# pedro-morgado/spatialaudiogen

Measured on AMD Instinct MI355X. Metric: ambisonic seconds generated/sec (0.1 s windows, 224x448 video), higher is better.
Workload: dtype f32 (fp32 in / out / accumulate; products on the 16-bit matrix cores with fp32-equivalent operand splits: two fp16 planes (3 products per multiply) for the ResNet trunk's 3x3 convs, whose operand ranges batch-norm bounds, three bf16 planes (6 products) elsewhere - measured against the fp64 oracle as

## Files before the change

### spatialaudiogen_amd/build.py

```python
import os
import subprocess
import sys
from concurrent.futures import ThreadPoolExecutor

HERE = os.path.dirname(os.path.abspath(__file__))
CSRC = os.path.join(HERE, 'csrc')
OBJ = os.path.join(CSRC, 'build')
LIB = os.path.join(HERE, 'libsagen_hip.so')
SOURCES = ['conv3p.hip', 'conv3h.hip', 'conv3g.hip', 'p3.hip', 'igemm3dw.hip', 'igemm3s2.hip', 'stempool.hip', 'stem8.hip', 'igemm.hip', 'fcm.hip', 'igemm3.hip', 'elementwise.hip', 'fft.hip', 'eval.hip', 'evalx.hip', 'render.hip', 'overlay.hip', 'train.hip', 'wgrad.hip', 'wgrad3h.hip', 'backward.hip', 'model.hip', 'train_model.hip', 'api.hip']
HEADERS = sorted(os.path.join(CSRC, h) for h in os.listdir(CSRC) if h.endswith('.h')) + \
          [os.path.join(os.path.dirname(os.path.dirname(CSRC)), 'include', 'sagen.h')]
FLAGS = ['--offload-arch=gfx950', '-O3', '-std=c++17', '-fPIC', '-Wall', '-Wno-unused-function', '-fno-slp-vectorize', '-fno-vectorize']


def _hipcc():
    for cand in (os.environ.get('HIPCC'), '/opt/rocm/bin/hipcc', 'hipcc'):
        if cand and (os.path.isabs(cand) and os.path.exists(cand) or not os.path.isabs(cand)):
            return cand
    raise RuntimeError('hipcc not found')


def flags_digest():
    import hashlib
    h = hashlib.sha256(' '.join(FLAGS).encode())
    h.update(open(os.path.abspath(__file__), 'rb').read())
    return h.hexdigest()[:16]


def source_digest():
    import hashlib
    files = sorted(f for f in os.listdir(CSRC) if f.endswith(('.hip', '.h')))
    h = hashlib.sha256()
    for f in files:
        h.update(f.encode() + b'\0' + open(os.path.join(CSRC, f), 'rb').read() + b'\0')
    h.update(b'sagen.h\0' + open(HEADERS[-1], 'rb').read())
    return h.hexdigest()[:16]


def _stale(target, deps):
    if not os.path.exists(target):
        return True
    t = os.path.getmtime(target)
    return any(os.path.getmtime(d) > t for d in deps)


def build(force=False, verbose=True):
    os.makedirs(OBJ, exist_ok=True)
    hipcc = _hipcc()
    stamp = os.path.join(OBJ, 'flags.stamp')
    if not os.path.exists(stamp) or open(stamp).read().strip() != flags_digest():
        force = True
    jobs = []
    for src in SOURCES:
        s = os.path.join(CSRC, src)
        o = os.path.join(OBJ, src.replace('.hip', '.o'))
        if force or _stale(o, [s] + HEADERS):
            jobs.append((s, o))

    def compile_one(job):
        s, o = job
        cmd = [hipcc] + FLAGS + ['-DSAGEN_BUILD_FLAGS="%s"' % ' '.join(FLAGS), '-c', s, '-o', o]
        if verbose:
# ... 50 lines not shown
```

### spatialaudiogen_amd/csrc/conv3h.hip

```cpp
#include "igemm3_common.h"
#include "h2_planes.h"

namespace sagen {

typedef _Float16 f16x8 __attribute__((ext_vector_type(8)));

constexpr int conv3h_lds(int BM, int BN, int KC, int AR = 2) { return KC * (AR * BM * 64 + 2 * 3 * 2 * BN * 32); }
constexpr int conv3h_wgs_per_cu(int BM, int BN, int KC, int AR = 2) {
    return 160 * 1024 / conv3h_lds(BM, BN, KC, AR) >= 3 ? 3 : (160 * 1024 / conv3h_lds(BM, BN, KC, AR) >= 2 ? 2 : 1);
}

template <int BM, int BN, int WM, int WN, int KC, int AR>
__device__ __forceinline__ void conv3h_body(const IgemmDesc& d) {
    static_assert(AR == 2 || AR == 3, "activation ring of two or three stages");
    constexpr int MT = WM / 32, NT = WN / 32;
    constexpr int WAVES_N = BN / WN, WAVES_M = BM / WM;
    static_assert(WAVES_N * WAVES_M == 4, "4 waves per workgroup");
    constexpr int BME = BM - 2;
    constexpr int A_INST = BM / 16;
    constexpr int B_IPT = BN / 16;
    constexpr int B_INST = 3 * B_IPT;
    constexpr int A_PW = (A_INST + 3) / 4, B_PW = (B_INST + 3) / 4;
    constexpr int A_BYTES = A_INST * 1024, B_BYTES = B_INST * 1024;
    constexpr int ST_BYTES = KC * (A_BYTES + B_BYTES);
    constexpr int NM1 = 3 * MT * NT;
    constexpr int NMG = 3 * KC * NM1;
    constexpr int SPT = A_PW + B_PW;
    constexpr int CNT_MAX = KC * SPT;
    static_assert(CNT_MAX <= NMG, "one DMA slot per MFMA slot at most");
    constexpr int NF = 2 * (MT + NT);
    constexpr int SMEM_BYTES = KC * (AR * A_BYTES + 2 * B_BYTES);
    static_assert(SMEM_BYTES == conv3h_lds(BM, BN, KC, AR), "occupancy bound uses the same footprint");
    static_assert(AR == 2 || A_INST % 4 == 0, "counted vmcnt: every wave issues the same number of activation instructions");
    auto a_stage = [&](int sa) { return AR == 2 ? sa * ST_BYTES : sa * (KC * A_BYTES); };
    auto b_stage = [&](int sb) { return AR == 2 ? sb * ST_BYTES + KC * A_BYTES : AR * KC * A_BYTES + sb * (KC * B_BYTES); };
    __shared__ __attribute__((aligned(16))) char smem[SMEM_BYTES];

    const int tid = threadIdx.x;
#ifdef SAGEN_TRACE
    const size_t trc_wg = ((size_t)blockIdx.z * gridDim.y + blockIdx.y) * gridDim.x + blockIdx.x;
    unsigned long long* const trc = (d.trace && trc_wg < 8192) ? (unsigned long long*)d.trace + trc_wg * 8 : nullptr;
#define C3H_TRC(k) do { if (trc && tid == 0) trc[k] = __builtin_amdgcn_s_memtime(); } while (0)
    if (trc && tid == 0) {
        trc[4] = __builtin_amdgcn_s_getreg((31 << 11) | 4);
        trc[5] = __builtin_amdgcn_s_getreg((31 << 11) | 20);
        trc[6] = __builtin_amdgcn_s_memrealtime();
    }
    C3H_TRC(0);
    const int gsel = (blockIdx.y | blockIdx.z) ? -1 : ((int)blockIdx.x == 8 ? 0 : ((int)blockIdx.x == (int)gridDim.x - 64 ? 1 : -1));
    unsigned long long* const gtr = (d.trace && gsel >= 0) ? (unsigned long long*)d.trace + (size_t)8192 * 8 + (size_t)gsel * 64 * 8 : nullptr;
    int g_idx = 0;
#define C3H_GTRC(k) do { if (gtr && tid == 0 && g_idx < 64) gtr[g_idx * 8 + (k)] = __builtin_amdgcn_s_memtime(); } while (0)
#else
#define C3H_TRC(k) do { } while (0)
#define C3H_GTRC(k) do { } while (0)
#endif
    const int lane = tid & 63;
    const int wave = __builtin_amdgcn_readfirstlane(tid >> 6);
    const int wm = wave / WAVES_N, wn = wave % WAVES_N;
    const int W = d.Win, H = d.Hin, Wp = W + 1, NP = d.p3_np;
    const int nchunk = d.Cin >> 4;
    const bool dhs = d.splitk == 3;
    const int dh_z = dhs ? (int)blockIdx.y : 0;
    const int G = (dhs ? 1 : 3) * nchunk / KC;
    const int nM = (NP + BME - 1) / BME, nN = (d.N + BN - 1) / BN;

    const __amdgpu_buffer_rsrc_t x_rsrc = __builtin_amdgcn_make_buffer_rsrc((void*)d.xp3, 0, d.xp3_bytes, 0x00020000);
    const __amdgpu_buffer_rsrc_t w_rsrc = __builtin_amdgcn_make_buffer_rsrc((void*)d.wh2, 0, d.wh2_bytes, 0x00020000);

    const float osc = d.h2_a_inv[0] * d.h2_w_inv[0];

    const int xcd = (blockIdx.x + blockIdx.z) & 7;
    const int per = (nM + 7) >> 3;
    const int t_run = blockIdx.x >> 3;
    const int my_tiles = max(min((xcd + 1) * per, nM) - xcd * per, 0) * nN;
    if (t_run >= my_tiles) return;
    const int tq = t_run / nN;
    const int m0 = (xcd * per + tq) * BME;
    const int n0 = (t_run - tq * nN) * BN;

    unsigned a_v0[A_PW], a_v1[A_PW], a_v2[A_PW], a_cur[A_PW];
#pragma unroll
    for (int j = 0; j < A_PW; ++j) {
        const int inst = wave + 4 * j;
        const int U = inst * 64 + lane;
        const int slot = U >> 2, v = U & 3;
        const int u = v ^ ((slot >> 2) & 3);
        const int p = m0 - 1 + slot;
        unsigned bad = 7u;
        if (inst < A_INST && p >= 0 && p < NP) {
            const unsigned row = __umulhi((unsigned)p, d.p3_magic_wp);
            const int h = (int)(row - __umulhi(row, d.p3_magic_h) * (unsigned)H);
            bad = (h == 0 ? 1u : 0u) | (h == H - 1 ? 4u : 0u);
        }
        const int base = p * 64 + u * 16;
        a_v0[j] = (bad & 1u) ? OOB : (unsigned)(base - Wp * 64);
        a_v1[j] = (bad & 2u) ? OOB : (unsigned)base;
        a_v2[j] = (bad & 4u) ? OOB : (unsigned)(base + Wp * 64);
    }
    unsigned b_voff[B_PW];
    int b_tapoff[B_PW];
#pragma unroll
    for (int j = 0; j < B_PW; ++j) {
        const int inst = wave + 4 * j;
        b_tapoff[j] = __builtin_amdgcn_readfirstlane((inst / B_IPT) * nchunk * d.N * 64);
        const int r = inst % B_IPT;
        const int L = r * 64 + lane;
        const int pl = L / (2 * BN), n = (L >> 1) % BN, half = L & 1;
        b_voff[j] = (inst < B_INST && n0 + n < d.N) ? (unsigned)((pl * d.N + n0 + n) * 32 + 16 * (half ^ ((n >> 3) & 1))) : OOB;
    }

    int qa_dh = dh_z, qa_ch = 0, cur_dh = -1, qb_dh = dh_z, qb_ch = 0;
    unsigned i_asoff = 0, i_bsoff = 0;
    char* i_astage = smem;
    char* i_bstage = smem;
    auto begin_issue_a = [&](int sa) {
        i_astage = smem + a_stage(sa);
        if (qa_dh != cur_dh) {
            cur_dh = qa_dh;
#pragma unroll
            for (int j = 0; j < A_PW; ++j) a_cur[j] = qa_dh == 0 ? a_v0[j] : (qa_dh == 1 ? a_v1[j] : a_v2[j]);
        }
        i_asoff = (unsigned)qa_ch * d.xp3_cstride;
        qa_ch += KC;
        if (qa_ch == nchunk) { qa_ch = 0; ++qa_dh; }
    };
    auto begin_issue_b = [&](int sb) {
        i_bstage = smem + b_stage(sb);
        i_bsoff = (unsigned)((qb_dh * 3) * nchunk + qb_ch) * (unsigned)(d.N * 64);
        qb_ch += KC;
        if (qb_ch == nchunk) { qb_ch = 0; ++qb_dh; }
    };
    auto issue_a = [&](int kc, int s) {
        const int inst = wave + 4 * s;
        if (A_INST % 4 == 0 || inst < A_INST)
            dma16(x_rsrc, (float*)(i_astage + kc * A_BYTES + inst * 1024), a_cur[s], i_asoff + (unsigned)kc * d.xp3_cstride);
    };
    auto issue_b = [&](int kc, int j) {
        const int inst = wave + 4 * j;
        if (4 * (j + 1) <= B_INST || inst < B_INST)
            dma16(w_rsrc, (float*)(i_bstage + kc * B_BYTES + inst * 1024), b_voff[j], i_bsoff + (unsigned)b_tapoff[j] + (unsigned)(kc * d.N * 64));
    };
    auto issue_nth = [&](int n) {
        if (AR == 2) {
            const int sg = CNT_MAX - 1 - n;
            const int kc = sg / SPT, s = sg - kc * SPT;
            if (s < A_PW) issue_a(kc, s); else issue_b(kc, s - A_PW);
        } else if (n < KC * B_PW) {
            issue_b(n / B_PW, n % B_PW);
        } else {
            const int m = n - KC * B_PW;
            issue_a(m / A_PW, m % A_PW);
        }
    };

    f32x16 acc[MT][NT];
#pragma unroll
    for (int i = 0; i < MT; ++i)
#pragma unroll
        for (int j = 0; j < NT; ++j)
#pragma unroll
            for (int e = 0; e < 16; ++e) acc[i][j][e] = 0.f;

    const int li = lane & 31, kk = lane >> 5;
    int a_foff[3][MT];
#pragma unroll
    for (int i = 0; i < MT; ++i)
#pragma unroll
        for (int dwi = 0; dwi < 3; ++dwi) {
            const int sl = wm * WM + i * 32 + li + dwi;
            a_foff[dwi][i] = sl * 64 + 16 * (kk ^ ((sl >> 2) & 3));
        }
    const int b_foff = (wn * WN + li) * 32 + 16 * (kk ^ ((li >> 3) & 1));
    constexpr int TA[3] = {1, 0, 0}, TB[3] = {0, 1, 0};

    int sa = 0, sb = 0;
    begin_issue_a(0);
    begin_issue_b(0);
#pragma unroll
    for (int n = 0; n < CNT_MAX; ++n) issue_nth(n);
    if (AR == 3) {
        begin_issue_a(1);
#pragma unroll
        for (int n = KC * B_PW; n < CNT_MAX; ++n) issue_nth(n);
    }

    auto group = [&](auto issue_tag) {
        constexpr int ISSUE = decltype(issue_tag)::value;
        constexpr int NISSUE = ISSUE == 2 ? CNT_MAX : (ISSUE == 1 ? KC * B_PW : 0);
        const char* st_a = smem + a_stage(sa);
        const char* st_b = smem + b_stage(sb);
        f16x8 fq[2][NF];
        auto load_frag = [&](int buf, int t, int f) {
            const int kc = t / 3, dwi = t - 3 * kc;
            const int pl = f / (MT + NT), r = f - pl * (MT + NT);
            if (r < MT) fq[buf][f] = *reinterpret_cast<const f16x8*>(st_a + kc * A_BYTES + (a_foff[dwi][r] ^ (pl * 32)));
            else fq[buf][f] = *reinterpret_cast<const f16x8*>(st_b + b_foff + kc * B_BYTES + (dwi * 2 + pl) * (BN * 32) + (r - MT) * 32 * 32);
        };
#pragma unroll
        for (int f = 0; f < NF; ++f) load_frag(0, 0, f);
        C3H_GTRC(3);
#pragma unroll
        for (int t = 0; t < 3 * KC; ++t) {
            const int cb = t & 1;
#pragma unroll
            for (int tt = 0; tt < 3; ++tt)
#pragma unroll
                for (int i = 0; i < MT; ++i)
#pragma unroll
                    for (int j = 0; j < NT; ++j) {
                        const int k = (tt * MT + i) * NT + j;
                        const int idx = t * NM1 + k;
                        __builtin_amdgcn_sched_barrier(0);
                        acc[i][j] = __builtin_amdgcn_mfma_f32_32x32x16_f16(fq[cb][TA[tt] * (MT + NT) + i], fq[cb][TB[tt] * (MT + NT) + MT + j],
                                                                           acc[i][j], 0, 0, 0);
                        if (t + 1 < 3 * KC) {
#pragma unroll
                            for (int f = 0; f < NF; ++f)
                                if (f * NM1 / NF == k) load_frag(cb ^ 1, t + 1, f);
                        }
#pragma unroll
                        for (int n = 0; n < NISSUE; ++n)
                            if (idx == n) issue_nth(n);
                    }
        }
        __builtin_amdgcn_sched_barrier(0);
        C3H_GTRC(4);
#ifdef SAGEN_TRACE
        ++g_idx;
#endif
        sa = sa + 1 == AR ? 0 : sa + 1;
        sb ^= 1;
    };

    C3H_TRC(1);
    if (AR == 2) {
        for (int it = 0; it + 1 < G; ++it) {
            C3H_GTRC(0);
            asm volatile("s_waitcnt vmcnt(0)" ::: "memory");
            C3H_GTRC(1);
            lds_barrier();
            C3H_GTRC(2);
            begin_issue_a(sa ^ 1);
            begin_issue_b(sb ^ 1);
            group(std::integral_constant<int, 2>{});
        }
        asm volatile("s_waitcnt vmcnt(0)" ::: "memory");
        lds_barrier();
        group(std::integral_constant<int, 0>{});
    } else {
        for (int it = 0; it + 2 < G; ++it) {
            asm volatile("s_waitcnt vmcnt(%0)" ::"n"(KC * A_PW) : "memory");
            lds_barrier();
            begin_issue_b(sb ^ 1);
            begin_issue_a(sa == 0 ? 2 : sa - 1);
            group(std::integral_constant<int, 2>{});
        }
        asm volatile("s_waitcnt vmcnt(%0)" ::"n"(KC * A_PW) : "memory");
        lds_barrier();
        begin_issue_b(sb ^ 1);
        group(std::integral_constant<int, 1>{});
        asm volatile("s_waitcnt vmcnt(0)" ::: "memory");
        lds_barrier();
        group(std::integral_constant<int, 0>{});
    }

    C3H_TRC(2);
    const int colb = n0 + wn * WN + li;
    const bool plain = d.bias == nullptr && !d.relu_out;
    const __amdgpu_buffer_rsrc_t y_rsrc = __builtin_amdgcn_make_buffer_rsrc((void*)((char*)d.y + (size_t)dh_z * d.y_bytes), 0, d.y_bytes, 0x00020000);
    const unsigned ldy4 = (unsigned)d.ldy * 4u;
    const int plim = min(NP, m0 + BME);
    float bias_j[NT], cs[NT], cq[NT];
    unsigned col4[NT];
#pragma unroll
    for (int j = 0; j < NT; ++j) {
        const bool ok = colb + 32 * j < d.N;
        col4[j] = ok ? (unsigned)(colb + 32 * j) * 4u : OOB;
        bias_j[j] = (d.bias != nullptr && ok) ? d.bias[colb + 32 * j] : 0.f;
        cs[j] = 0.f; cq[j] = 0.f;
    }
    lds_barrier();
    unsigned* const s_roff = reinterpret_cast<unsigned*>(smem);
    for (int r = tid; r < BM; r += 256) {
        const int p = m0 + r;
        const unsigned row = __umulhi((unsigned)p, d.p3_magic_wp);
        s_roff[r] = (p < plim && (unsigned)p - row * (unsigned)Wp < (unsigned)W) ? ((unsigned)p - row) * ldy4 : OOB;
    }
    lds_barrier();
    auto epilogue = [&](auto fast_tag) {
        constexpr bool FAST = decltype(fast_tag)::value;
#pragma unroll
        for (int i = 0; i < MT; ++i)
#pragma unroll
            for (int q = 0; q < 4; ++q) {
                const uint4 ro = *reinterpret_cast<const uint4*>(s_roff + wm * WM + i * 32 + 8 * q + 4 * kk);
#pragma unroll
                for (int u = 0; u < 4; ++u) {
                    const int e = 4 * q + u;
                    const unsigned rraw = u == 0 ? ro.x : (u == 1 ? ro.y : (u == 2 ? ro.z : ro.w));
                    const float sc = (rraw & OOB) ? 0.f : osc;
                    const unsigned roff = FAST ? rraw + (unsigned)(colb * 4) : rraw;
#pragma unroll
                    for (int j = 0; j < NT; ++j) {
                        float v = acc[i][j][e] * sc;
                        if (i == MT - 1 && e >= 14 && (rraw & OOB)) v = 0.f;
                        if (FAST) {
                            cs[j] += v;
                            cq[j] = __builtin_fmaf(v, v, cq[j]);
                            __builtin_amdgcn_raw_buffer_store_b32(__builtin_bit_cast(unsigned, v), y_rsrc, roff, 128 * j, 0);
                        } else {
                            const unsigned off = ((roff | col4[j]) & OOB) ? OOB : roff + col4[j];
                            if (col4[j] & OOB) v = 0.f;
                            cs[j] += v;
                            cq[j] = __builtin_fmaf(v, v, cq[j]);
                            v += bias_j[j];
                            if (d.relu_out) v = fmaxf(v, 0.f);
                            __builtin_amdgcn_raw_buffer_store_b32(__builtin_bit_cast(unsigned, v), y_rsrc, off, 0, 0);
                        }
                    }
                }
            }
    };
    if (plain && n0 + BN <= d.N) epilogue(std::true_type{});
    else epilogue(std::false_type{});
    if (d.stats != nullptr) {
        float* const red = reinterpret_cast<float*>(smem + BM * 4);
        static_assert(BM * 4 + WAVES_M * 2 * 2 * BN * 4 <= SMEM_BYTES, "statistics staging must fit the ring");
#pragma unroll
        for (int j = 0; j < NT; ++j) {
            red[((wm * 2 + kk) * 2 + 0) * BN + wn * WN + j * 32 + li] = cs[j];
            red[((wm * 2 + kk) * 2 + 1) * BN + wn * WN + j * 32 + li] = cq[j];
        }
        lds_barrier();
        for (int t = tid; t < 2 * BN; t += 256) {
            const int which = t / BN, col = t - which * BN;
            if (n0 + col < d.N) {
                float sum = 0.f;
#pragma unroll
                for (int g = 0; g < WAVES_M * 2; ++g) sum += red[(g * 2 + which) * BN + col];
                atomicAdd(&d.stats[(long)which * d.N + n0 + col], (double)sum);
            }
        }
    }
    C3H_TRC(3);
#ifdef SAGEN_TRACE
    if (trc && tid == 0) trc[7] = __builtin_amdgcn_s_memrealtime();
#endif
#undef C3H_TRC
#undef C3H_GTRC
}

template <int BM, int BN, int WM, int WN, int KC>
__global__ __launch_bounds__(256, conv3h_wgs_per_cu(BM, BN, KC, 2)) void conv3h_kernel(const IgemmDesc d_in) {
    IgemmDesc d = d_in;
    if (d.grp.G > 1) igemm_relocate(d, (int)blockIdx.z);
    conv3h_body<BM, BN, WM, WN, KC, 2>(d);
}
template <int BM, int BN, int WM, int WN, int KC>
__global__ __launch_bounds__(256, conv3h_wgs_per_cu(BM, BN, KC, 3)) void conv3hr_kernel(const IgemmDesc d_in) {
    IgemmDesc d = d_in;
    if (d.grp.G > 1) igemm_relocate(d, (int)blockIdx.z);
    conv3h_body<BM, BN, WM, WN, KC, 3>(d);
}

template <int BM, int BN, int WM, int WN, int KC, int AR = 2>
static int launch_conv3h(const IgemmDesc& d, hipStream_t s) {
    if ((d.Cin / 16) % KC) return fail(SAGEN_ERR_UNSUPPORTED, "conv3h: %d channel chunks are not a multiple of %d per group", d.Cin / 16, KC);
    const int per = (cdiv(d.p3_np, BM - 2) + 7) / 8;
    const int grid = 8 * per * cdiv(d.N, BN);
    if constexpr (AR == 3) {
        if (d.splitk != 1) return fail(SAGEN_ERR_UNSUPPORTED, "conv3hr: no dh-split (the three-deep ring needs three groups)");
        hipLaunchKernelGGL((conv3hr_kernel<BM, BN, WM, WN, KC>), dim3(grid, 1, d.grp.G), dim3(256), 0, s, d);
    } else hipLaunchKernelGGL((conv3h_kernel<BM, BN, WM, WN, KC>), dim3(grid, d.splitk, d.grp.G), dim3(256), 0, s, d);
    SAGEN_LAUNCH_CHECK();
    return SAGEN_OK;
}

#ifdef SAGEN_TRACE
static void* g_trace_buf = nullptr;
static int g_trace_nth = -1;
extern "C" void sagen_debug_trace_conv3h(void* buf, int nth) { g_trace_buf = buf; g_trace_nth = nth; }
#endif

int conv3h_dispatch(const IgemmDesc& d_in, IgemmTile tile, hipStream_t s) {
    IgemmDesc d = d_in;
#ifdef SAGEN_TRACE
    if (g_trace_nth >= 0 && g_trace_nth-- == 0) d.trace = g_trace_buf;
#endif
    if (!d.xp3 || d.p3_np <= 0 || d.xp3_fmt != 1) return fail(SAGEN_ERR_NULL, "conv3h: the fp16x2 activation planes are missing");
    if (!d.wh2 || !d.h2_a_inv || !d.h2_w_inv) return fail(SAGEN_ERR_NULL, "conv3h: the fp16x2 filter planes / scales are missing");
    if (d.splitk != 1 && d.splitk != 3) return fail(SAGEN_ERR_UNSUPPORTED, "conv3h: split-K only as the dh-split (3), got %d", d.splitk);
    if (d.splitk == 3) {
        if (!d.splitk_ws || d.bias || d.relu_out || d.stats) return fail(SAGEN_ERR_UNSUPPORTED, "conv3h: the dh-split writes raw partials (no bias / ReLU / statistics)");
        d.y = d.splitk_ws;
        d.ldy = d.N;
    }
    if ((long)(d.p3_np + 512) * (d.Win + 1) >= (1L << 32) || ((long)(d.p3_np + 512) / (d.Win + 1) + 1) * d.Hin >= (1L << 32))
        return fail(SAGEN_ERR_UNSUPPORTED, "conv3h: too many pixels for 32-bit index arithmetic");
    if ((long)d.p3_np * 64 >= (1L << 31) || (long)d.xp3_cstride * (d.Cin / 16) >= (1L << 31) || d.xp3_bytes == 0)
        return fail(SAGEN_ERR_UNSUPPORTED, "conv3h: the activation planes exceed 2 GiB buffer addressing (use a smaller batch)");
    const long y_bytes = ((long)(d.M - 1) * d.ldy + d.N) * 4;
    if (y_bytes >= (1L << 31)) return fail(SAGEN_ERR_UNSUPPORTED, "conv3h: the output exceeds 2 GiB buffer addressing (use a smaller batch)");
    d.y_bytes = (unsigned)y_bytes;
// ... 133 lines not shown
```

### spatialaudiogen_amd/csrc/igemm.hip

```cpp
#include "igemm_common.h"
#include <cstdlib>

namespace sagen {


template <int BM, int BN, int WM, int WN, int STG, int BK>
__global__ __launch_bounds__(256, (WM * WN >= 4096 ? 2 : (WM * WN >= 2048 ? (BK == 32 ? 2 : 3) : (BK == 32 ? 3 : 4)))) void igemm_kernel(const IgemmDesc d_in) {
    static_assert(BK == 16 || BK == 32, "K tile of 16 or 32");
    IgemmDesc d = d_in;
    int z = blockIdx.z;
    if (d.grp.G > 1) {
        const int g = d.splitk == 1 ? z : z / d.splitk;
        z -= g * d.splitk;
        igemm_relocate(d, g);
    }
    constexpr int CPR = BK / 4;
    constexpr int RPI = 64 / CPR;
    constexpr int RPBR = 64 / BK;
    constexpr int MT = WM / 32, NT = WN / 32;
    constexpr int WAVES_N = BN / WN;
    constexpr int WAVES_M = BM / WM;
    static_assert(WAVES_N * WAVES_M == 4, "4 waves per workgroup");
    constexpr int A_DMA = BM / RPI, B_DMA = BN / RPI;
    constexpr int A_PW = (A_DMA + 3) / 4, B_PW = (B_DMA + 3) / 4;
// ... 176 lines not shown
                        v.x = ok ? fmaxf(fmaf(v.x, sc.x, sh.x), 0.f) : 0.f;
                        v.y = ok ? fmaxf(fmaf(v.y, sc.y, sh.y), 0.f) : 0.f;
                        v.z = ok ? fmaxf(fmaf(v.z, sc.z, sh.z), 0.f) : 0.f;
                        v.w = ok ? fmaxf(fmaf(v.w, sc.w, sh.w), 0.f) : 0.f;
                        af[u][i] = v;
                    }
                }
            }
            if (hf == 0) TRC(1);
#pragma unroll
            for (int u = 0; u < 2; ++u)
#pragma unroll
                for (int r = 0; r < 4; ++r)
#pragma unroll
                    for (int i = 0; i < MT; ++i)
#pragma unroll
                        for (int j = 0; j < NT; ++j) {
                            const float a = r == 0 ? af[u][i].x : r == 1 ? af[u][i].y : r == 2 ? af[u][i].z : af[u][i].w;
                            const float b = r == 0 ? bf[u][j].x : r == 1 ? bf[u][j].y : r == 2 ? bf[u][j].z : bf[u][j].w;
#ifndef SAGEN_ABLATE_MFMA
                            acc[i][j] = __builtin_amdgcn_mfma_f32_32x32x2f32(a, b, acc[i][j], 0, 0, 0);
#else
                            asm volatile("" ::"v"(a), "v"(b));
#endif
                            const int idx = (((hf * 2 + u) * 4 + r) * MT + i) * NT + j;
#pragma unroll
                            for (int g = 0; g < PER; ++g)
                                if (idx == (g + 1) * NMFMA / (PER + 1) - 1 && more) issue_one(g);
                        }
        }
        TRC(2);
        if (uni) {
            p_c0 += BK;
            if (d.ntaps > 1 && p_c0 == d.Cin) { p_c0 = 0; ++p_tap; }
        }
        if (STAGES == 3 && more) wait_vmcnt<EVEN ? PER : 0>(); else wait_vmcnt<0>();
        TRC(3);
        lds_barrier();
        TRC(4);
        stage = stage + 1 == STAGES ? 0 : stage + 1;
    }

    igemm_epilogue<BM, BN, WM, WN>(d, acc, s_row, smem, m0, n0, z, tid);
}

template <int BM, int BN, int WM, int WN, int STG, int BK>
static int launch_cfg(const IgemmDesc& d, hipStream_t s) {
    dim3 grid(cdiv(d.M, BM), cdiv(d.N, BN), d.splitk * d.grp.G);
    hipLaunchKernelGGL((igemm_kernel<BM, BN, WM, WN, STG, BK>), grid, dim3(256), 0, s, d);
    SAGEN_LAUNCH_CHECK();
    return SAGEN_OK;
}

struct TileCfg { int bm, bn, bk; const char* name; bool split = false; bool dw3 = false; bool s2 = false; bool p3 = false; bool g = false; bool h = false; };
static const TileCfg kTiles[TILE_AUTO] = {
    {128, 128, 16, "igemm_kernel<128,128,64,64,3,16>"}, {128, 64, 16, "igemm_kernel<128,64,64,32,3,16>"},
    {256, 64, 16, "igemm_kernel<256,64,64,64,3,16>"},   {64, 64, 16, "igemm_kernel<64,64,32,32,3,16>"},
    {128, 32, 16, "igemm_kernel<128,32,32,32,2,16>"},   {32, 128, 16, "igemm_kernel<32,128,32,32,2,16>"},
    {128, 128, 16, "igemm_kernel<128,128,64,64,2,16>"}, {128, 64, 16, "igemm_kernel<128,64,64,32,2,16>"},
    {256, 64, 16, "igemm_kernel<256,64,64,64,2,16>"},   {64, 64, 16, "igemm_kernel<64,64,32,32,2,16>"},
    {64, 128, 16, "igemm_kernel<64,128,32,64,3,16>"},   {64, 128, 16, "igemm_kernel<64,128,32,64,2,16>"},
    {64, 256, 16, "igemm_kernel<64,256,64,64,3,16>"},   {64, 256, 16, "igemm_kernel<64,256,64,64,2,16>"},
    {256, 32, 16, "igemm_kernel<256,32,64,32,2,16>"},
    {64, 64, 32, "igemm_kernel<64,64,32,32,2,32>"},     {64, 128, 32, "igemm_kernel<64,128,32,64,2,32>"},
    {128, 64, 32, "igemm_kernel<128,64,64,32,2,32>"},   {128, 128, 32, "igemm_kernel<128,128,64,64,2,32>"},
    {32, 128, 32, "igemm_kernel<32,128,32,32,2,32>"},   {128, 32, 32, "igemm_kernel<128,32,32,32,2,32>"},
    {128, 128, 16, "igemm3_kernel<128,128,64,64,1>", true}, {128, 64, 16, "igemm3_kernel<128,64,64,32,1>", true},
    {256, 64, 16, "igemm3_kernel<256,64,64,64,1>", true},   {64, 64, 16, "igemm3_kernel<64,64,32,32,1>", true},
    {64, 128, 16, "igemm3_kernel<64,128,32,64,1>", true},   {64, 256, 16, "igemm3_kernel<64,256,64,64,1>", true},
    {32, 128, 16, "igemm3_kernel<32,128,32,32,1>", true},   {128, 32, 16, "igemm3_kernel<128,32,32,32,1>", true},
    {128, 64, 16, "igemm3_kernel<128,64,64,32,2>", true},   {64, 64, 16, "igemm3_kernel<64,64,32,32,2>", true},
    {64, 128, 16, "igemm3_kernel<64,128,32,64,2>", true},   {32, 128, 16, "igemm3_kernel<32,128,32,32,2>", true},
    {128, 32, 16, "igemm3_kernel<128,32,32,32,2>", true},
    {128, 128, 16, "igemm3dw_kernel<128,128,64,64,false>", true, true}, {128, 64, 16, "igemm3dw_kernel<128,64,64,32,false>", true, true},
    {256, 64, 16, "igemm3dw_kernel<256,64,64,64,false>", true, true},   {64, 128, 16, "igemm3dw_kernel<64,128,32,64,false>", true, true},
    {64, 64, 16, "igemm3dw_kernel<64,64,32,32,false>", true, true},     {64, 256, 16, "igemm3dw_kernel<64,256,64,64,false>", true, true},
    {128, 64, 16, "igemm3dw_kernel<128,64,64,32,true>", true, true},    {256, 64, 16, "igemm3dw_kernel<256,64,64,64,true>", true, true},
    {64, 64, 16, "igemm3dw_kernel<64,64,32,32,true>", true, true},      {64, 128, 16, "igemm3dw_kernel<64,128,32,64,true>", true, true},
    {256, 64, 16, "igemm3s2_kernel<256,64,64,64>", true, false, true},  {128, 64, 16, "igemm3s2_kernel<128,64,64,32>", true, false, true},
    {128, 64, 16, "conv3p_kernel<128,64,64,32>", true, true, false, true},   {128, 128, 16, "conv3p_kernel<128,128,64,64>", true, true, false, true},
    {64, 64, 16, "conv3p_kernel<64,64,32,32>", true, true, false, true},
    {128, 64, 16, "conv3pp_kernel<0>", true, true, false, true},          {128, 64, 16, "conv3pp_kernel<1>", true, true, false, true},
    {128, 64, 16, "conv3g_kernel<128,64,64,32,2,false>", true, false, false, true, true}, {64, 64, 16, "conv3g_kernel<64,64,32,32,2,false>", true, false, false, true, true},
    {64, 128, 16, "conv3g_kernel<64,128,32,64,2,false>", true, false, false, true, true}, {128, 128, 16, "conv3g_kernel<128,128,64,64,1,false>", true, false, false, true, true},
    {128, 64, 16, "conv3h_kernel<128,64,64,32,1>", true, true, false, true, false, true},   {128, 128, 16, "conv3h_kernel<128,128,64,64,1>", true, true, false, true, false, true},
    {64, 64, 16, "conv3h_kernel<64,64,32,32,1>", true, true, false, true, false, true},      {256, 64, 16, "conv3h_kernel<256,64,64,64,1>", true, true, false, true, false, true},
    {128, 64, 16, "conv3g_kernel<128,64,64,32,3,true>", true, false, false, true, true, true},   {64, 64, 16, "conv3g_kernel<64,64,32,32,4,true>", true, false, false, true, true, true},
    {128, 128, 16, "conv3g_kernel<128,128,64,64,2,true>", true, false, false, true, true, true}, {64, 128, 16, "conv3g_kernel<64,128,32,64,3,true>", true, false, false, true, true, true},
    {128, 64, 32, "conv3h_kernel<128,64,64,32,2>", true, true, false, true, false, true}, {64, 64, 32, "conv3h_kernel<64,64,32,32,2>", true, true, false, true, false, true},
    {64, 64, 64, "conv3h_kernel<64,64,32,32,4>", true, true, false, true, false, true},
    {64, 128, 16, "conv3g_kernel<64,128,32,64,2,true,1>", true, false, false, true, true, true}, {64, 128, 16, "conv3g_kernel<64,128,32,64,4,true,1>", true, false, false, true, true, true},
    {128, 128, 16, "conv3g_kernel<128,128,64,64,2,true,1>", true, false, false, true, true, true}, {128, 256, 16, "conv3g_kernel<128,256,64,128,2,true,1>", true, false, false, true, true, true},
    {256, 64, 16, "conv3hr_kernel<256,64,64,64,1>", true, true, false, true, false, true}, {128, 64, 16, "conv3hr_kernel<128,64,64,32,1>", true, true, false, true, false, true},
    {64, 64, 32, "conv3hr_kernel<64,64,32,32,2>", true, true, false, true, false, true},
    {128, 128, 16, "conv3hr_kernel<128,128,64,64,1>", true, true, false, true, false, true},
};
static bool s2_ok(const IgemmDesc& d) {
    return d.Cin == 4 && d.ldx == 4 && d.ntaps == 56 && d.TW == 8 && d.in_sh == 2 && d.in_sw == 2 && d.tap_sh == 1 && d.tap_sw == 1 &&
           d.tap_h0 == 0 && d.tap_w0 == 0 && d.dsh * d.dsw == 1 && d.g_h0 == 0 && d.g_w0 == 0 && d.K == 224 && d.Kpad == 224 &&
           d.in_scale == nullptr && d.bn_in.acc == nullptr && d.x_bstride == (long)d.Hin * d.Win * 4 && d.Wg >= 64 &&
           (d.Wg - 1) * 2 + 8 <= d.Win && (d.Hg - 1) * 2 + 7 <= d.Hin;
}
static bool dw3_ok(const IgemmDesc& d) {
    return d.ntaps == 9 && d.TW == 3 && d.tap_sh == 1 && d.tap_sw == 1 && d.tap_h0 == -1 && d.tap_w0 == -1 && d.in_sh == 1 &&
           d.in_sw == 1 && d.dsh * d.dsw == 1 && d.Hin == d.Hg && d.Win == d.Wg && d.g_h0 == 0 && d.g_w0 == 0 && d.Cin % 16 == 0 &&
           d.K == 9 * d.Cin && d.Kpad == d.K && d.x_bstride == (long)d.Hin * d.Win * d.ldx && d.Hin >= 2 && d.Win >= 8;
}
bool igemm_tile_split(IgemmTile t) { return t >= 0 && t < TILE_AUTO && kTiles[t].split; }
bool igemm_tile_p3(IgemmTile t) { return t >= 0 && t < TILE_AUTO && kTiles[t].p3; }
bool igemm_tile_dh_split(IgemmTile t) {
    return t >= 0 && t < TILE_AUTO && kTiles[t].p3 && kTiles[t].h && !kTiles[t].g && t != TILE_P3HR_256x64 && t != TILE_P3HR_128x64 && t != TILE_P3HR_64x64_C2 && t != TILE_P3HR_128x128;
}
bool igemm_p3_eligible(const IgemmDesc& d) { return dw3_ok(d) && d.w_split && d.dsh * d.dsw == 1 && d.Cin <= MAX_BN_C; }
static int tile_bm(IgemmTile t) { return (t >= 0 && t < TILE_AUTO) ? kTiles[t].bm : 0; }
static int tile_bn(IgemmTile t) { return (t >= 0 && t < TILE_AUTO) ? kTiles[t].bn : 0; }
int igemm_tile_bm(IgemmTile t) { return tile_bm(t); }
int igemm_tile_bn(IgemmTile t) { return tile_bn(t); }
int igemm_tile_bk(IgemmTile t) { return (t >= 0 && t < TILE_AUTO) ? kTiles[t].bk : 0; }
const char* igemm_tile_name(IgemmTile t) { return (t >= 0 && t < TILE_AUTO) ? kTiles[t].name : "igemm_kernel<?>"; }

static bool uniform_taps_for(const IgemmDesc& d, int bk) {
    return (d.ntaps > 1 ? (d.Cin % bk == 0) : true) && (d.K % bk == 0);
}
bool igemm_tile_grouped(IgemmTile t) {
    if (t < 0 || t >= TILE_AUTO) return false;
    const TileCfg& k = kTiles[t];
    if (k.s2 || (k.dw3 && !k.p3)) return false;
    if (k.p3 && !k.h && !k.g) return false;
    return true;
}
bool igemm_tile_ok(const IgemmDesc& d, IgemmTile t) {
    if (t < 0 || t >= TILE_AUTO) return false;
    if (cur_group().G > 1 && !igemm_tile_grouped(t)) return false;
    const int bk = kTiles[t].bk;
    if (d.Kpad % bk) return false;
    if (kTiles[t].split && !d.w_split) return false;
    const bool mm_tile = t == TILE_P3GH_MM_64x128_K2 || t == TILE_P3GH_MM_64x128_K4 || t == TILE_P3GH_MM_128x128_K2 || t == TILE_P3GH_MM_128x256_K2;
    if (mm_tile != (d.mm_out != nullptr && kTiles[t].g)) return false;
    if (mm_tile && (d.Wg % kTiles[t].bm || (d.dsw * d.Cout) % kTiles[t].bn)) return false;
    if (d.mm_out != nullptr && !mm_tile) {
        const bool b3 = kTiles[t].split && !kTiles[t].dw3 && !kTiles[t].s2 && !kTiles[t].p3;
        if (!b3 || kTiles[t].bm > 128 || kTiles[t].bn > 128 || d.Cout != 32 || d.dsh * d.dsw <= 1 || d.Wg % kTiles[t].bm ||
            (d.dsw * d.Cout) % kTiles[t].bn || d.splitk != 1 || d.in_scale || d.bn_in.acc || !d.mm_coeffs)
            return false;
    }
    if (kTiles[t].dw3 && !dw3_ok(d)) return false;
    if (kTiles[t].p3 && (d.xp3 == nullptr || (d.splitk != 1 && !(d.splitk == 3 && igemm_tile_dh_split(t))))) return false;
    if (kTiles[t].p3 && (kTiles[t].h ? (d.xp3_fmt != 1 || d.wh2 == nullptr) : d.xp3_fmt != 0)) return false;
    if (!kTiles[t].p3 && d.xp3 != nullptr && d.x == nullptr) return false;
    if (kTiles[t].g) return conv3g_ok(d);
    if (kTiles[t].p3) return true;
    if (kTiles[t].s2 && !s2_ok(d)) return false;
    if ((d.in_scale || d.bn_in.acc) && !uniform_taps_for(d, bk)) return false;
    return true;
}

IgemmTile igemm_pick_tile(const IgemmDesc& d) {
    static const char* force = getenv("SAGEN_FORCE_TILE");
    if (force && d.M > 128 && d.N >= 64 && igemm_tile_ok(d, (IgemmTile)atoi(force))) return (IgemmTile)atoi(force);
    static const bool fp32_only = getenv("SAGEN_FP32_ONLY") != nullptr;
    if (d.mm_out != nullptr) return (d.xp3 != nullptr && d.xp3_fmt == 1 && d.wh2 != nullptr && conv3g_ok(d)) ? TILE_P3GH_MM_64x128_K2 : TILE_B3_64x128;
    auto blocks = [&](IgemmTile t) { return (long)cdiv(d.M, tile_bm(t)) * cdiv(d.N, tile_bn(t)) * d.splitk; };
    const long want = 2 * 256;
    if (d.w_split && !fp32_only) {
        const bool pro = d.in_scale != nullptr || d.bn_in.acc != nullptr;
        if (s2_ok(d)) return TILE_B3S2_128x64;
        if (d.xp3 != nullptr && d.xp3_fmt == 1 && dw3_ok(d) && d.splitk == 1) {
            const long np = d.p3_np;
            if ((long)cdiv(np, 126) * cdiv(d.N, 64) >= 3 * 256) return TILE_P3H_128x64;
            return TILE_P3H_64x64;
        }
        if (d.xp3 != nullptr && dw3_ok(d) && d.splitk == 1) {
            const long np = d.p3_np;
            if (d.N <= 64) return cdiv(np, 128) >= want ? TILE_P3_128x64 : TILE_P3_64x64;
            if ((long)cdiv(np, 128) * cdiv(d.N, 64) >= want) return TILE_P3_128x64;
            return TILE_P3_64x64;
        }
        if (d.xp3 != nullptr && !dw3_ok(d) && d.splitk == 1 && conv3g_ok(d)) {
            if (d.xp3_fmt == 1) return blocks(TILE_P3GH_128x64_K3) >= 256 + 128 ? TILE_P3GH_128x64_K3 : TILE_P3GH_64x64_K4;
            return blocks(TILE_P3G_128x64_K2) >= 256 + 128 ? TILE_P3G_128x64_K2 : TILE_P3G_64x64_K2;
        }
        if (dw3_ok(d) && (!pro || uniform_taps_for(d, 16))) {
            if (d.N <= 64) return blocks(TILE_B3DW_128x64) >= want ? TILE_B3DW_128x64 : TILE_B3DWM_64x64;
            if (blocks(TILE_B3DW_128x128) >= 256 + 128) return TILE_B3DW_128x128;
            return blocks(TILE_B3DWM_128x64) >= 256 + 128 ? TILE_B3DWM_128x64 : TILE_B3DWM_64x64;
        }
        if (d.M <= 32) return TILE_B3_32x128;
        if (d.N <= 32) return TILE_B3_128x32;
        if (d.N <= 64) return blocks(TILE_B3_128x64) >= want ? TILE_B3_128x64 : TILE_B3_64x64;
        if (blocks(TILE_B3_128x128) >= 256 + 128) return TILE_B3_128x128;
        if (blocks(TILE_B3_64x128) >= want) return TILE_B3_64x128_K2;
        return TILE_B3_64x64_K2;
    }
    if (d.M <= 32) return TILE_32x128;
    if (d.N <= 32) return TILE_128x32;
    if (d.N <= 64) {
        if (blocks(TILE_256x64) >= want) return TILE_256x64;
        if (blocks(TILE_128x64) >= want) return TILE_128x64;
        return TILE_64x64;
    }
    if (blocks(TILE_128x128) >= want) return TILE_128x128;
    if (blocks(TILE_128x64) >= want) return TILE_128x64;
    return TILE_64x64;
}

int igemm_grid_m(const IgemmDesc& d, IgemmTile tile) {
    if (tile == TILE_AUTO) tile = igemm_pick_tile(d);
    return cdiv(d.M, tile_bm(tile));
}

int igemm_launch(const IgemmDesc& d_in, IgemmTile tile, hipStream_t s) {
    IgemmDesc d = d_in;
    if ((!d.x && !d.xp3) || !d.w || (!d.y && !d.splitk_ws)) return fail(SAGEN_ERR_NULL, "igemm: null operand");
    if (d.M <= 0 || d.N <= 0 || d.K <= 0) return fail(SAGEN_ERR_SHAPE, "igemm: empty problem M=%d N=%d K=%d", d.M, d.N, d.K);
    if (d.Kpad % 16 || d.Kpad < d.K) return fail(SAGEN_ERR_SHAPE, "igemm: Kpad=%d must be a multiple of 16 >= K=%d", d.Kpad, d.K);
    if (d.K % 4 || d.Cin % 4) return fail(SAGEN_ERR_UNSUPPORTED, "igemm: Cin=%d / K=%d must be multiples of 4", d.Cin, d.K);
    if (d.ntaps > 1 && (d.log2Cin < 2 || (1 << d.log2Cin) != d.Cin))
        return fail(SAGEN_ERR_UNSUPPORTED, "igemm: multi-tap conv needs power-of-two Cin (got %d)", d.Cin);
    if (d.K != d.ntaps * d.Cin) return fail(SAGEN_ERR_SHAPE, "igemm: K=%d != ntaps*Cin=%d", d.K, d.ntaps * d.Cin);
    if (d.splitk > 1 && !d.splitk_ws) return fail(SAGEN_ERR_UNSUPPORTED, "igemm: split-K needs a workspace");
    if (d.splitk_ws && (d.stats || d.dsh * d.dsw != 1))
        return fail(SAGEN_ERR_UNSUPPORTED, "igemm: partial-sum output needs a plain epilogue");
    if (d.N != d.dsh * d.dsw * d.Cout) return fail(SAGEN_ERR_SHAPE, "igemm: N=%d != dsh*dsw*Cout", d.N);
    {
        const int nb = d.M / (d.Hg * d.Wg) + (d.M % (d.Hg * d.Wg) ? 1 : 0);
        const long xb = (long)nb * d.x_bstride * 4, wb = (long)d.N * d.Kpad * 4;
        if (xb >= (1L << 31) || wb >= (1L << 31) || (d.w_split && wb / 2 * 3 >= (1L << 31)))
            return fail(SAGEN_ERR_UNSUPPORTED, "igemm: operand of %ld bytes exceeds 2 GiB buffer addressing (use a smaller batch)", xb > wb ? xb : wb);
        d.x_bytes = (unsigned)xb;
        d.w_bytes = (unsigned)wb;
        bool inside = true;
        for (int t = 0; t < d.ntaps && inside; ++t) {
            const int th = t / d.TW, dh = th * d.tap_sh + d.tap_h0, dw = (t - th * d.TW) * d.tap_sw + d.tap_w0;
            const long h_lo = (long)d.g_h0 * d.in_sh + dh, h_hi = (long)(d.g_h0 + d.Hg - 1) * d.in_sh + dh;
            const long w_lo = (long)d.g_w0 * d.in_sw + dw, w_hi = (long)(d.g_w0 + d.Wg - 1) * d.in_sw + dw;
            inside = h_lo >= 0 && h_hi < d.Hin && w_lo >= 0 && w_hi < d.Win;
        }
        d.no_bounds = inside ? 1 : 0;
        if ((d.in_scale || d.bn_in.acc) && (d.Cin % 16 || d.K % 16 || d.ntaps == 1 || d.Cin > MAX_BN_C))
            return fail(SAGEN_ERR_UNSUPPORTED, "igemm: input batch-norm needs a multi-tap conv with Cin %% 16 == 0 and Cin <= %d", MAX_BN_C);
        if (!inside && d.ntaps > 64) return fail(SAGEN_ERR_UNSUPPORTED, "igemm: padded conv with %d taps (max 64)", d.ntaps);
    }
    if (tile == TILE_AUTO) tile = igemm_pick_tile(d);
    d.grp = cur_group();
    if (d.grp.G > 1 && !igemm_tile_grouped(tile)) return fail(SAGEN_ERR_UNSUPPORTED, "igemm: %s has no grouped launch", igemm_tile_name(tile));
    if (!igemm_tile_ok(d, tile)) return fail(SAGEN_ERR_UNSUPPORTED, "igemm: %s cannot run this problem (Kpad=%d Cin=%d)", igemm_tile_name(tile), d.Kpad, d.Cin);
    d.uniform_taps = uniform_taps_for(d, kTiles[tile].bk) ? 1 : 0;
    if (d.ntaps > MAX_TAPS) return fail(SAGEN_ERR_UNSUPPORTED, "igemm: %d taps (max %d)", d.ntaps, MAX_TAPS);
    if (kTiles[tile].g) return conv3g_dispatch(d, tile, s);
    if (kTiles[tile].h) return conv3h_dispatch(d, tile, s);
    if (kTiles[tile].p3) return conv3p_dispatch(d, tile, s);
    if (kTiles[tile].s2) return igemm3s2_dispatch(d, tile, s);
    if (kTiles[tile].split) return igemm3_dispatch(d, tile, s);
    switch (tile) {
        case TILE_128x128: return launch_cfg<128, 128, 64, 64, 3, 16>(d, s);
        case TILE_128x64: return launch_cfg<128, 64, 64, 32, 3, 16>(d, s);
        case TILE_256x64: return launch_cfg<256, 64, 64, 64, 3, 16>(d, s);
        case TILE_64x64: return launch_cfg<64, 64, 32, 32, 3, 16>(d, s);
        case TILE_128x32: return launch_cfg<128, 32, 32, 32, 2, 16>(d, s);
        case TILE_32x128: return launch_cfg<32, 128, 32, 32, 2, 16>(d, s);
        case TILE_128x128_S2: return launch_cfg<128, 128, 64, 64, 2, 16>(d, s);
        case TILE_128x64_S2: return launch_cfg<128, 64, 64, 32, 2, 16>(d, s);
        case TILE_256x64_S2: return launch_cfg<256, 64, 64, 64, 2, 16>(d, s);
        case TILE_64x64_S2: return launch_cfg<64, 64, 32, 32, 2, 16>(d, s);
        case TILE_64x128: return launch_cfg<64, 128, 32, 64, 3, 16>(d, s);
        case TILE_64x128_S2: return launch_cfg<64, 128, 32, 64, 2, 16>(d, s);
        case TILE_64x256: return launch_cfg<64, 256, 64, 64, 3, 16>(d, s);
        case TILE_64x256_S2: return launch_cfg<64, 256, 64, 64, 2, 16>(d, s);
        case TILE_256x32: return launch_cfg<256, 32, 64, 32, 2, 16>(d, s);
        case TILE_64x64_K32: return launch_cfg<64, 64, 32, 32, 2, 32>(d, s);
        case TILE_64x128_K32: return launch_cfg<64, 128, 32, 64, 2, 32>(d, s);
        case TILE_128x64_K32: return launch_cfg<128, 64, 64, 32, 2, 32>(d, s);
        case TILE_128x128_K32: return launch_cfg<128, 128, 64, 64, 2, 32>(d, s);
        case TILE_32x128_K32: return launch_cfg<32, 128, 32, 32, 2, 32>(d, s);
        case TILE_128x32_K32: return launch_cfg<128, 32, 32, 32, 2, 32>(d, s);
        default: return fail(SAGEN_ERR_UNSUPPORTED, "igemm: bad tile id %d", (int)tile);
    }
}

template <int V>
__global__ __launch_bounds__(256) void splitk_reduce_kernel(const float* __restrict__ ws_, int splitk, int M, int N,
                                                            const float* __restrict__ bias, int relu,
                                                            float* __restrict__ y_, int ldy, int rep, float* __restrict__ amax_out_, const GroupInfo gi) {
    const float* __restrict__ ws = SAGEN_GRP(ws_);
    float* __restrict__ y = SAGEN_GRP(y_);
    float* __restrict__ amax_out = SAGEN_GRP(amax_out_);
    const int NV = N / V;
    const long idx = (long)blockIdx.x * 256 + threadIdx.x;
    const bool ok = idx < (long)M * NV;
    const int m = ok ? (int)(idx / NV) : 0, n = ok ? (int)(idx - (long)m * NV) * V : 0;
    float v[V];
#pragma unroll
    for (int i = 0; i < V; ++i) v[i] = 0.f;
    if (ok) {
        const long MN = (long)M * N;
        const float* p = ws + (long)m * N + n;
        int zz = 0;
        if (V == 4)
            for (; zz + 4 <= splitk; zz += 4, p += 4 * MN) {
                const float4 t0 = *reinterpret_cast<const float4*>(p), t1 = *reinterpret_cast<const float4*>(p + MN);
                const float4 t2 = *reinterpret_cast<const float4*>(p + 2 * MN), t3 = *reinterpret_cast<const float4*>(p + 3 * MN);
// ... 410 lines not shown
```

### spatialaudiogen_amd/csrc/kernels.h

```cpp
#pragma once
#include "common.h"
#include "wave_reduce.h"

namespace sagen {

struct BnRef {
    const double* acc = nullptr;
    const float* gamma = nullptr;
    const float* beta = nullptr;
    double inv_count = 0.0;
    float eps = 1e-3f;
};

constexpr int H2_AMAX_SLOTS = 64, H2_AMAX_STRIDE = 32, H2_AMAX_FLOATS = H2_AMAX_SLOTS * H2_AMAX_STRIDE;

struct IgemmDesc {
    const float* x = nullptr;
    const float* w = nullptr;
    int w_split = 0;
    float* y = nullptr;
    const float* bias = nullptr;
    const float* in_scale = nullptr;
    const float* in_shift = nullptr;
    BnRef bn_in;
    double* stats = nullptr;
    float* amax_out = nullptr;
    float* splitk_ws = nullptr;
    int* sk_ticket = nullptr;
    int sk_rep = 1;
    int M = 0, N = 0, K = 0, Kpad = 0;
    int Hg = 1, Wg = 1, g_h0 = 0, g_w0 = 0;
    int Hin = 1, Win = 1, Cin = 0, ldx = 0;
    long x_bstride = 0;
    int in_sh = 1, in_sw = 1;
    int ntaps = 1, TW = 1, tap_sh = 1, tap_sw = 1, tap_h0 = 0, tap_w0 = 0;
    int log2Cin = -1;
    int dsh = 1, dsw = 1, Cout = 0;
    int Hlim = 1, Wlim = 1;
    long y_bstride = 0;
    long y_rstride = 0;
    int ldy = 0;
    int relu_out = 0;
    int splitk = 1;
    unsigned x_bytes = 0, w_bytes = 0;
    unsigned y_bytes = 0;
    int no_bounds = 0;
    int uniform_taps = 0;
    const void* xp3 = nullptr;
    unsigned xp3_bytes = 0, xp3_cstride = 0;
    int p3_np = 0;
    int xp3_fmt = 0;
    int xp3_row0 = 0, xp3_rows = 0;
    const void* wh2 = nullptr;
    unsigned wh2_bytes = 0;
    const float* h2_a_inv = nullptr;
    const float* h2_w_inv = nullptr;
    unsigned p3_magic_wp = 0, p3_magic_h = 0;
    const float* mm_coeffs = nullptr;
    float* mm_out = nullptr;
    int mm_row0 = 0, mm_nf = 0;
    int mm_f_lo = 1;
    void* trace = nullptr;
    int trace_block = 0;
    GroupInfo grp;
};
__device__ __forceinline__ void igemm_relocate(IgemmDesc& d, int g) {
    const GroupInfo gi = d.grp;
    d.x = grp_ptr(d.x, gi, g); d.y = grp_ptr(d.y, gi, g);
    d.in_scale = grp_ptr(d.in_scale, gi, g); d.in_shift = grp_ptr(d.in_shift, gi, g);
    d.bn_in.acc = grp_ptr(d.bn_in.acc, gi, g);
    d.stats = grp_ptr(d.stats, gi, g); d.amax_out = grp_ptr(d.amax_out, gi, g);
    d.splitk_ws = grp_ptr(d.splitk_ws, gi, g); d.sk_ticket = grp_ptr(d.sk_ticket, gi, g);
    d.xp3 = grp_ptr(d.xp3, gi, g);
    d.h2_a_inv = grp_ptr(d.h2_a_inv, gi, g); d.h2_w_inv = grp_ptr(d.h2_w_inv, gi, g);
    d.mm_coeffs = grp_ptr(d.mm_coeffs, gi, g); d.mm_out = grp_ptr(d.mm_out, gi, g);
}

enum IgemmTile {
    TILE_128x128 = 0, TILE_128x64, TILE_256x64, TILE_64x64, TILE_128x32, TILE_32x128,
    TILE_128x128_S2, TILE_128x64_S2, TILE_256x64_S2, TILE_64x64_S2,
    TILE_64x128, TILE_64x128_S2, TILE_64x256, TILE_64x256_S2, TILE_256x32,
    TILE_64x64_K32, TILE_64x128_K32, TILE_128x64_K32, TILE_128x128_K32, TILE_32x128_K32, TILE_128x32_K32,
    TILE_B3_128x128, TILE_B3_128x64, TILE_B3_256x64, TILE_B3_64x64, TILE_B3_64x128, TILE_B3_64x256, TILE_B3_32x128,
    TILE_B3_128x32,
    TILE_B3_128x64_K2, TILE_B3_64x64_K2, TILE_B3_64x128_K2, TILE_B3_32x128_K2, TILE_B3_128x32_K2,
    TILE_B3DW_128x128, TILE_B3DW_128x64, TILE_B3DW_256x64, TILE_B3DW_64x128, TILE_B3DW_64x64, TILE_B3DW_64x256,
    TILE_B3DWM_128x64, TILE_B3DWM_256x64, TILE_B3DWM_64x64, TILE_B3DWM_64x128,
    TILE_B3S2_256x64, TILE_B3S2_128x64,
    TILE_P3_128x64, TILE_P3_128x128, TILE_P3_64x64,
    TILE_P3PP_PAIR, TILE_P3PP_SPLITK,
    TILE_P3G_128x64_K2, TILE_P3G_64x64_K2, TILE_P3G_64x128_K2, TILE_P3G_128x128_K1,
    TILE_P3H_128x64, TILE_P3H_128x128, TILE_P3H_64x64, TILE_P3H_256x64,
    TILE_P3GH_128x64_K3, TILE_P3GH_64x64_K4, TILE_P3GH_128x128_K2, TILE_P3GH_64x128_K3,
    TILE_P3H_128x64_C2, TILE_P3H_64x64_C2, TILE_P3H_64x64_C4,
    TILE_P3GH_MM_64x128_K2, TILE_P3GH_MM_64x128_K4, TILE_P3GH_MM_128x128_K2, TILE_P3GH_MM_128x256_K2,
    TILE_P3HR_256x64, TILE_P3HR_128x64, TILE_P3HR_64x64_C2,
    TILE_P3HR_128x128,
    TILE_AUTO
};

int igemm_launch(const IgemmDesc& d, IgemmTile tile, hipStream_t s);
int igemm_grid_m(const IgemmDesc& d, IgemmTile tile);
IgemmTile igemm_pick_tile(const IgemmDesc& d);
const char* igemm_tile_name(IgemmTile t);
int igemm_tile_bm(IgemmTile t);
int igemm_tile_bn(IgemmTile t);
int igemm_tile_bk(IgemmTile t);
bool igemm_tile_split(IgemmTile t);
int igemm3_dispatch(const IgemmDesc& d, IgemmTile tile, hipStream_t s);
int igemm3dw_dispatch(const IgemmDesc& d, IgemmTile tile, hipStream_t s);
int igemm3s2_dispatch(const IgemmDesc& d, IgemmTile tile, hipStream_t s);
int conv3p_dispatch(const IgemmDesc& d, IgemmTile tile, hipStream_t s);
int conv3g_dispatch(const IgemmDesc& d, IgemmTile tile, hipStream_t s);
int conv3h_dispatch(const IgemmDesc& d, IgemmTile tile, hipStream_t s);
int h2_filter_pack_launch(const float* wp, int N, int Kpad, void* w2, unsigned* scratch, float* w_inv, hipStream_t s);
struct H2Job {
    const float* wp = nullptr;
    void* w2 = nullptr;
    float* w_inv = nullptr;
    int N = 0, Kpad = 0, first_block = 0, pad_ = 0;
};
int h2_filter_pack_multi_launch(const H2Job* jobs_dev, int njobs, int nblocks, unsigned* amax, hipStream_t s);
bool conv3g_ok(const IgemmDesc& d);
constexpr int SK_TICKETS = 8192;
inline bool igemm_tile_fused_splitk(IgemmTile) { return true; }
bool igemm_tile_p3(IgemmTile t);
bool igemm_tile_grouped(IgemmTile t);
bool igemm_tile_dh_split(IgemmTile t);
bool igemm_p3_eligible(const IgemmDesc& d);
bool igemm_tile_ok(const IgemmDesc& d, IgemmTile t);
constexpr int SPLITK_RB = 16;
int splitk_reduce_launch(const float* ws, int splitk, int M, int N, const float* bias, int relu,
                         float* y, int ldy, int rep, double* stats, hipStream_t s, float* amax_out = nullptr);

struct DeconvGather {
    int B = 0, Hin = 0, Win = 0, kh = 1, kw = 1, sh = 1, sw = 1, Cout = 0;
    int in_row0 = 0, R = 0;
    int y0 = 0, y1 = 0;
    int relu = 0, ldy = 0;
    const float* bias = nullptr;
    float* y = nullptr;
    float* amax_out = nullptr;
};
int deconv_gather_launch(const float* ws, int splitk, const DeconvGather& g, hipStream_t s);

int pack_conv_launch(const float* w_hwio, int ntaps, int cin_src, int cin_pad, int cout,
                     float* wp, int Npad, int Kpad, hipStream_t s, int tw_src = 0, int tw_pad = 0);
int pack_split_launch(float* wp, int N, int Kpad, hipStream_t s);
inline size_t packed_split_floats(size_t n_fp32) { return n_fp32 + (3 * n_fp32 + 1) / 2; }
enum PackKind { PACK_CONV = 0, PACK_DECONV, PACK_FLIPT, PACK_ROWS, PACK_DECONV_PHASE };
struct PackJob {
    const float* src = nullptr;
    float* dst = nullptr;
    int kind = 0, N = 0, Kpad = 0;
    int p[7] = {0, 0, 0, 0, 0, 0, 0};
    int first_block = 0;
};
inline int pack_job_blocks(int kind, long N, long Kpad) {
    return kind == PACK_CONV ? (int)(((N + 31) / 32) * ((Kpad + 31) / 32)) : (int)((N * Kpad + 1023) / 1024);
}
int pack_multi_launch(const PackJob* jobs_dev, int njobs, int nblocks, hipStream_t s, int block0 = 0);
int pack_deconv_launch(const float* w_hwoi, int kh, int kw, int cout, int cin, int sh, int sw,
                       float* wp, int Npad, int Kpad, hipStream_t s);

int bn_finalize_launch(const double* stats, long count, int C, const float* gamma,
                       const float* beta, float eps, float* scale, float* shift, hipStream_t s);
int bn_apply_relu_launch(const float* x, const float* scale, const float* shift, const BnRef& bn, const float* residual,
                         float* y, long n_pixels, int C, hipStream_t s);
int maxpool3x3s2_launch(const float* x, const float* scale, const float* shift, const BnRef& bn, float* y,
                        int B, int H, int W, int C, hipStream_t s);
int pad_nhwc3to4_launch(const float* x, float* y, int B, int H, int W, int pt, int pb, int pl, int pr,
                        hipStream_t s);
int pad_u8_nhwc3to4_launch(const unsigned char* x, float* y, int B, int H, int W, int pt, int pb, int pl, int pr, hipStream_t s);
int stempool_launch(const float* xpad, const float* wp, const float* gamma, float* pooled, double* stats, int B, hipStream_t s);
size_t stem8_plane_bytes(int B);
int stem8_prep_launch(const unsigned char* x, void* plane, int B, hipStream_t s, float* zero_ptr = nullptr, long zero_n = 0, int half = 0);
int stem8pool_h2_launch(const void* plane, const float* wp, const void* wh2, const float* w_inv, const float* gamma, float* pooled, double* stats, int B,
                        hipStream_t s);
int stem8pool_launch(const void* plane, const float* wp, const float* gamma, float* pooled, double* stats, int B, hipStream_t s);
int stem16_prep_launch(const float* x, void* planes, float* part, float* a_inv, int B, hipStream_t s, float* zero_ptr = nullptr, long zero_n = 0);
int stem16pool_launch(const void* planes, const void* wh2, const float* gamma, float* pooled, double* stats, const float* a_inv, const float* w_inv,
                      int B, hipStream_t s);
constexpr int STEM16_PARTS = 1024;
int stem8raw_launch(const void* plane, const float* wp, float* y0, double* stats, int B, hipStream_t s);
int stem8rawpool_launch(const void* plane, const float* wp, const float* gamma, float* y0, float* pooled, double* stats, int B, hipStream_t s);
int assemble_wyzx_launch(const float* audio, const float* yzx, float* out, int B, int snd_size,
                         int snd_contx, int snd_dur, hipStream_t s);
int power_map_launch(const float* ambi, long T, const float* sh, int P, float* rms, hipStream_t s);
int power_map_batched_launch(const float* ambi, int nchunks, long T, const float* sh, int P, float* rms, double* moments, hipStream_t s);
int nosep_mix_launch(const float* audio, const float* coeffs, float* out, int B, int snd_size,
                     int snd_contx, int snd_dur, int num_out, hipStream_t s);
int nosep_mix_multi_launch(const float* audio, const float* coeffs, float* out, int B, int snd_size, int snd_contx,
                           int snd_dur, int nin, int num_out, hipStream_t s);

size_t p3_bytes(int B, int H, int W, int C);
constexpr int H2S_FILTER_FIRST = 8;
constexpr int H2S_FIXED_FIRST = 232;
constexpr int H2S_A_INV_X = 232;
constexpr int H2S_A_INV_B = 236;
constexpr int H2S_S16_A_INV = 238;
constexpr int H2_RIG_OFF = 240;
struct P3hScale {
    float* a_inv = nullptr;
    const float* res_bound = nullptr;
    const double* res_acc = nullptr;
    double res_inv_count = 0.0;
    float* bound_out = nullptr;
    unsigned* sat_count = nullptr;
    unsigned char* relu_bits = nullptr;
    const void* res_planes = nullptr;
    const float* res_a_inv = nullptr;
};
int p3_pack_launch(const float* x, const float* scale, const float* shift, const BnRef& bn, const float* residual, int relu,
                   float* y, void* p3, int B, int H, int W, int C, hipStream_t s, int fmt = 0, const P3hScale* h2 = nullptr);
size_t p3h_bytes(int B, int H, int W, int C);
int h2_pack_rows_launch(const float* x, long x_bstride, long x_rstride, int ldx, int row0, int B, int R, int W, int C, const float* amax0,
                        const float* amax1, void* planes, float* a_inv, unsigned* sat_count, hipStream_t s);
int p3_maxpool_launch(const float* x, const float* scale, const float* shift, const BnRef& bn, float* y, void* p3, int B, int H,
                      int W, int C, hipStream_t s, int fmt = 0, const P3hScale* h2 = nullptr);

int fft_tables_ensure(hipStream_t s);
int stft_launch(const float* audio, int B, int n_samples, int f0, int f1, float* mag,
                int c0, int c1, float* spec, hipStream_t s, float* zero_ptr = nullptr, int zero_n = 0);
size_t mask_istft_scratch_bytes(int B);
int mask_istft_mix_launch(const float* dmask, long dmask_bstride, int dmask_f0, const float* spec,
                          const float* coeffs, int B, int ntracks, float* out, float* scratch,
                          hipStream_t s, const float* ebuf = nullptr);
int stft_multi_launch(const float* audio, int B, int n_samples, int nin, int f0, int f1, float* mag, int c0, int c1, float* spec,
                      hipStream_t s, float* zero_ptr = nullptr, int zero_n = 0);
size_t mask_istft_hoa_scratch_bytes(int B, int nout);
int mask_istft_hoa_launch(const float* dmask, long dmask_bstride, int dmask_f0, const float* spec, const float* coeffs, int B,
                          int ntracks, int nin, int nout, float* out, float* scratch, hipStream_t s);

size_t eval_scratch_floats(int B);
int eval_init_launch(float* scratch, hipStream_t s);
int eval_metrics_launch(const float* pred, const float* gt, int B, float* ps, double* pw, float* scratch, hipStream_t s);
size_t eval_scratch_floats_c(int B, int C);
int eval_metrics_c_launch(const float* pred, const float* gt, int B, int C, float* ps, double* pw, float* scratch, hipStream_t s);
size_t evalx_scratch_floats(int B, int C);
int evalx_mel_env_launch(const float* pred, const float* gt, int B, int C, float* mel_lsd, float* env_mse, float* scratch,
                         hipStream_t s);
int evalx_emd_launch(const float* p, const float* q, int n_maps, int nodes, const double* cost, double* out, unsigned int* not_converged,
                     hipStream_t s);

int render_fir_launch(const float* x, long long n_hist, long long n, int channels, const float* taps, int outputs, int ntaps,
                      const float* rot, int n_rot, int rot_hop, long long pos0, long long zero_before, float* y, hipStream_t s);

int power_map_windows_launch(const float* ambi, int channels, int stride, long long window, int n_maps, const float* sh, int P, float* rms,
                             double* moments, hipStream_t s);
size_t overlay_blend_grid_bytes(int mh, int mw, int n_frames);
int overlay_blend_launch(const float* maps, long long map0, int mh, int mw, const double* lut, const uint8_t* frames, int n_frames,
                         long long frame0, int h, int w, int frames_per_map, uint8_t* out, void* scratch, hipStream_t s);

int stft_loss_grad_launch(const float* pred, const float* gt, const float* mask, int B, float* grad, double* loss, hipStream_t s);
int adam_update_launch(float* p, const float* g, float* m, float* v, long n, float lr_t, float beta1, float beta2, float eps,
                       float gscale, hipStream_t s);

struct WgradDesc {
    const float* g = nullptr;
    const float* d = nullptr;
    float* out = nullptr;
    float* ws = nullptr;
    int B = 1, Hd = 1, Wd = 1;
    int HG = 1, WG = 1, ldg = 0, Cg = 0;
    int ldd = 0, Cd = 0;
    unsigned g_bstride = 0, g_rstride = 0, d_bstride = 0, d_rstride = 0;
    int sh = 1, sw = 1, TH = 1, TW = 1, h0 = 0, w0 = 0;
    int tsh = 1, tsw = 1;
// ... 53 lines not shown
```

### spatialaudiogen_amd/csrc/model.h

```cpp
#pragma once
#include "kernels.h"
#include "fcm.h"
#include <algorithm>
#include <cstdlib>
#include <functional>
#include <map>
#include <string>
#include <vector>

namespace sagen {

struct VarSpec {
    std::string name;
    int ndim;
    int64_t shape[4];
    long numel() const {
        long n = 1;
        for (int i = 0; i < ndim; ++i) n *= shape[i];
        return n;
    }
};

struct Buf {
    size_t off = 0, n = 0;
// ... 53 lines not shown
    int nsep = 32;
    int nin = 1, nout = 3;
    bool has_video = false, has_flow = false, freq_mask = true;

    std::vector<VarSpec> vars;
    std::map<std::string, int> var_index;
    std::vector<const float*> var_ptr;
    bool bound = false;

    int G = 1;
    int tune_groups = 0;
    int inter_group = 0;
    size_t grp_off = 0, grp_floats = 0;
    GroupInfo group_info() const {
        GroupInfo gi;
        if (G > 1 && ws) {
            gi.lo = reinterpret_cast<const char*>(ws + grp_off);
            gi.span = (unsigned long long)grp_floats * sizeof(float);
            gi.stride = gi.span;
            gi.G = G;
        }
        return gi;
    }
    size_t ws_floats = 0;
    float* ws = nullptr;
    std::map<std::string, Buf> bufs;
    std::map<std::string, Named> named;
    std::vector<PackJob> pack_jobs, pack_jobs_bwd;
    int pack_blocks = 0, pack_blocks_bwd = 0;
    bool train_mode = false;
    bool train_ready = false;
    bool stem_fused = true;
    bool materialize_mask = false;
    bool mask_fused_last = false;
    bool video_u8 = false;
    bool train_h2 = true;
    bool use_h2 = true;
    bool train_h2d = true;
    bool no_aud_planes = false;
    bool no_dh_split = false;
    bool sk_fused = false;
    bool train_h2w = true;
    std::map<std::string, int> h2d_slot;
    std::vector<H2Job> h2d_jobs;
    int h2d_blocks = 0;
    std::map<std::string, int> h2_slot;
    std::vector<H2Job> h2_jobs;
    int h2_blocks = 0;
    bool use_p3g = true;
    bool rawpool_last = false;
    bool train_rawpool = true;
    bool train_bands = true;
    int dec_lo[7] = {0, 0, 0, 0, 0, 0, 0}, dec_hi[7] = {0, 0, 0, 0, 0, 0, 0};
    bool no_scatter = false, no_d1_planes = false, no_lean_trunk = false;
    int dec_planes_min_batch = 16;
    bool use_fcm = false;
    std::map<std::string, int> fcm_slices;
    bool stem8h = true;
    bool stem16 = true;
    bool stem8 = true;
    size_t tws_floats = 0;
    float* tws = nullptr;
    std::map<std::string, Buf> tbufs;
    std::vector<float*> grad_ptr;
    std::vector<int> ms_bucket;
    std::vector<int> ms_count, ms_left;
    std::vector<hipEvent_t> ms_event;
    std::vector<char> ms_done;
    std::vector<int> ms_touched;
    hipEvent_t ms_tmp = nullptr;
    std::vector<float*> mov_ptr;
    Buf talloc(const std::string& name, size_t n) {
        Buf b;
        b.off = tws_floats;
        b.n = n;
        tws_floats += (n + 63) / 64 * 64;
        tbufs[name] = b;
        return b;
    }
    size_t cap(const std::string& name) const { auto it = bufs.find(name); return it != bufs.end() ? it->second.n : tbufs.at(name).n; }

    Buf alloc(const std::string& name, size_t n) {
        Buf b;
        b.off = ws_floats;
        b.n = n;
        ws_floats += (n + 63) / 64 * 64;
        bufs[name] = b;
        return b;
    }
    float* p(const std::string& name) const {
        auto it = bufs.find(name);
        if (it != bufs.end()) return ws + it->second.off;
        return tws + tbufs.at(name).off;
    }
    const float* v(const std::string& name) const { return var_ptr[var_index.at(name)]; }
    void add_var(const std::string& name, std::initializer_list<int64_t> shape) {
        VarSpec s;
        s.name = name;
        s.ndim = (int)shape.size();
        int i = 0;
        for (auto d : shape) s.shape[i++] = d;
        for (; i < 4; ++i) s.shape[i] = 1;
        var_index[name] = (int)vars.size();
        vars.push_back(s);
    }
    void expose(const std::string& name, const std::string& buf, size_t extra, std::initializer_list<int64_t> shape,
// ... 325 lines not shown
        d.M = c->B * R * Win; d.N = gd.kh * gd.kw * gd.Cout; d.K = Cin; d.Kpad = Cin;
        d.Hg = R; d.Wg = Win; d.Hin = Hin - in_row0; d.Win = Win; d.Cin = Cin; d.ldx = Cin; d.x_bstride = (long)Hin * Win * Cin;
        d.ntaps = 1; d.Cout = d.N; d.Hlim = R; d.Wlim = Win; d.ldy = d.N; d.y_rstride = (long)Win * d.N; d.y_bstride = (long)R * Win * d.N;
        d.y = c->ws + c->bufs.at(wsname).off;
        if (x_planes && !c->tuning) {
            auto it = c->plan.find(name);
            if (it != c->plan.end() && !igemm_tile_p3((IgemmTile)it->second.tile)) x_planes = false;
        }
        if (x_planes) {
            const int lx = l + 1;
            void* planes = c->p("catp");
            timed("h2_pack_rows_kernel", 0.0, [&] {
                return h2_pack_rows_launch(x, (long)Hin * Win * Cin, (long)Win * Cin, Cin, in_row0, c->B, R, Win, Cin, cat_amax(lx, 0), cat_amax(lx, 1), planes,
                                           cat_a_inv(lx), reinterpret_cast<unsigned*>(c->p("h2s") + 7), s); });
            d.xp3 = planes; d.xp3_fmt = 1; d.xp3_row0 = 0; d.xp3_rows = R;
            d.p3_np = c->B * R * (Win + 1);
            d.xp3_cstride = (unsigned)((size_t)d.p3_np * 64);
            d.xp3_bytes = (unsigned)((size_t)d.xp3_cstride * (Cin / 16));
            d.wh2 = c->p("pkhs:" + name + "/weights"); d.wh2_bytes = (unsigned)((size_t)d.N * d.Kpad * 4);
            d.h2_a_inv = cat_a_inv(lx); d.h2_w_inv = c->p("h2s") + c->h2_slot.at("pks:" + name);
        }
        custom_reduce_name = "deconv_gather_kernel";
        custom_reduce = [gd](const float* ws, int sk, hipStream_t st) { return deconv_gather_launch(ws, sk, gd, st); };
        gemm(d);
        custom_reduce = nullptr;
    }

    bool h2() const { return c->use_h2 && c->use_p3 && !c->fp32_only && (!c->train_mode || c->train_h2); }
    int p3_fmt() const { return h2() ? 1 : 0; }
    float* h2_a_inv() { return c->p("h2s") + (sfx.empty() ? 0 : 1); }
    float* h2_a_inv_x(int parity) { return c->p("h2s") + H2S_A_INV_X + 2 * (parity & 1) + (sfx.empty() ? 0 : 1); }
    float* h2_a_inv_b() { return c->p("h2s") + H2S_A_INV_B + (sfx.empty() ? 0 : 1); }
    float* h2_xbound(int parity) { return c->p("h2s") + 2 + 2 * (parity & 1) + (sfx.empty() ? 0 : 1); }
    P3hScale h2_scale(float* bound_out = nullptr, const float* res_bound = nullptr, const double* res_acc = nullptr, double res_inv_count = 0.0) {
        P3hScale h;
        h.a_inv = h2_a_inv(); h.bound_out = bound_out; h.res_bound = res_bound; h.res_acc = res_acc; h.res_inv_count = res_inv_count;
        h.sat_count = reinterpret_cast<unsigned*>(c->p("h2s") + 7);
        return h;
    }

    double* bn_acc(int layer_index) { return reinterpret_cast<double*>(c->p("bnacc" + sfx)) + (size_t)layer_index * 2 * 512; }
    BnRef bn_ref(int layer_index, const std::string& bn_name, long count) {
        BnRef r;
        r.acc = bn_acc(layer_index);
        r.gamma = c->v(bn_name + "/bn/gamma");
        r.beta = c->v(bn_name + "/bn/beta");
        r.inv_count = 1.0 / (double)count;
        r.eps = 1e-3f;
        return r;
    }

    void conv_bn(const float* x, int Hin, int Win, int Cin, const std::string& name, int k, int stride, int Cout,
                 const BnRef& bn_in, float* y, int& Hout, int& Wout, int bn_index, const std::string& plan_key = "",
                 const void* planes = nullptr, const float* planes_a_inv = nullptr) {
        if (rc) return;
        IgemmDesc d = conv_desc(x, Hin, Win, Cin, Cin, c->p("pk:" + name + "/weights"), k, k, stride, stride, true, Cout, y,
                                Cout, Hout, Wout);
        if (planes) {
            d.xp3 = planes;
            d.p3_np = c->B * Hin * (Win + 1);
            auto hs = c->h2_slot.find(name);
            if (h2() && (stride == 1 || c->use_p3g) && k == 3 && hs != c->h2_slot.end()) {
                d.xp3_fmt = 1;
                d.xp3_cstride = (unsigned)((size_t)d.p3_np * 64);
                d.xp3_bytes = (unsigned)p3h_bytes(c->B, Hin, Win, Cin);
                d.wh2 = c->p("pkh:" + name + "/weights");
                d.wh2_bytes = (unsigned)((size_t)d.N * d.Kpad * 4);
                d.h2_a_inv = planes_a_inv ? planes_a_inv : h2_a_inv();
                d.h2_w_inv = c->p("h2s") + hs->second;
            } else {
                d.xp3_cstride = (unsigned)((size_t)d.p3_np * 96);
                d.xp3_bytes = (unsigned)p3_bytes(c->B, Hin, Win, Cin);
            }
        }
        d.bn_in = bn_in;
        d.stats = bn_acc(bn_index);
        layer = plan_key.empty() ? name : plan_key;
        contract(d);
    }

    const float* resnet(const float* img, const std::string& scope) {
        const int B = c->B;
        int li = 0;
        const bool tune_general = c->tuning && c->G == 1;
        const bool fast8 = c->video_u8 && scope == "video_encoder" && c->stem8 && !tune_general && !c->fp32_only && !c->train_mode;
        const bool fast8h = fast8 && c->stem8h && h2() && c->h2_slot.count(scope + "/conv1/conv") != 0;
        const bool fast16 = !fast8 && !(c->video_u8 && scope == "video_encoder") && c->stem16 && !tune_general && !c->fp32_only && !c->train_mode && h2() &&
                            c->use_p3 && c->p3_from_stage <= 2 && c->bufs.count("s16:part" + sfx) != 0 && c->h2_slot.count(scope + "/conv1/conv") != 0;
        if (!fast8 && !fast16 && !rc && hipMemsetAsync(c->p("bnacc" + sfx), 0, c->bufs.at("bnacc" + sfx).n * sizeof(float), s) != hipSuccess)
            rc = fail(SAGEN_ERR_HIP, "hipMemsetAsync(bn accumulators) failed");
        layer = scope + "/pad";
        const bool pool_planes = c->use_p3 && c->p3_from_stage <= 2;
        const bool no_lean = c->no_lean_trunk;
        const bool lean = !no_lean && h2() && pool_planes && c->use_p3g && c->bufs.count("p3b" + sfx) != 0 && !c->train_mode;
        float* const s16_a_inv = c->p("h2s") + H2S_S16_A_INV + (sfx.empty() ? 0 : 1);
        if (fast16)
            timed("stem16_amax_kernel+stem16_prep_kernel", 0.0, [&] { return stem16_prep_launch(img, c->p("xpad" + sfx), c->p("s16:part" + sfx), s16_a_inv, B, s,
                                                                                               c->p("bnacc" + sfx), (long)c->bufs.at("bnacc" + sfx).n); });
        else if (fast8)
            timed("stem8_prep_kernel", 0.0, [&] { return stem8_prep_launch(reinterpret_cast<const unsigned char*>(img), c->p("xpad" + sfx), B, s,
                                                                          c->p("bnacc" + sfx), (long)c->bufs.at("bnacc" + sfx).n, fast8h ? 1 : 0); });
        else if (c->video_u8 && scope == "video_encoder")
            timed("pad_u8_nhwc3to4_kernel", 0.0, [&] { return pad_u8_nhwc3to4_launch(reinterpret_cast<const unsigned char*>(img), c->p("xpad" + sfx), B, 224, 448, 2, 3, 2, 4, s); });
        else
            timed("pad_nhwc3to4_kernel", 0.0, [&] { return pad_nhwc3to4_launch(img, c->p("xpad" + sfx), B, 224, 448, 2, 3, 2, 4, s); });
        int H = 0, W = 0;
        if (!rc && wait_before_mfma) {
            if (hipStreamWaitEvent(s, wait_before_mfma, 0) != hipSuccess) rc = fail(SAGEN_ERR_HIP, "hipStreamWaitEvent failed");
            wait_before_mfma = nullptr;
        }
        {
            const std::string name = scope + "/conv1/conv";
            const bool fused = c->stem_fused && !c->tuning && !c->fp32_only && !(c->use_p3 && c->p3_from_stage <= 2);
            if (fast8 || fast16) {
                H = 112; W = 224;
                layer = name + "+pool";
                if (fast16)
                    timed("stem8pool_kernel<f16>", 2.0 * B * H * W * 64 * 224, [&] {
                        return stem16pool_launch(c->p("xpad" + sfx), c->p("pkh:" + name + "/weights"), c->v(name + "/bn/gamma"), c->p("rx0" + sfx), bn_acc(li),
                                                 s16_a_inv, c->p("h2s") + c->h2_slot.at(name), B, s); });
                else if (fast8h)
                    timed("stem8pool_kernel<h2>", 2.0 * B * H * W * 64 * 224, [&] {
                        return stem8pool_h2_launch(c->p("xpad" + sfx), c->p("pk:" + name + "/weights"), c->p("pkh:" + name + "/weights"), c->p("h2s") + c->h2_slot.at(name),
                                                   c->v(name + "/bn/gamma"), c->p("rx0" + sfx), bn_acc(li), B, s); });
                else
                timed("stem8pool_kernel", 2.0 * B * H * W * 64 * 224, [&] {
                    return stem8pool_launch(c->p("xpad" + sfx), c->p("pk:" + name + "/weights"), c->v(name + "/bn/gamma"), c->p("rx0" + sfx), bn_acc(li), B, s); });
                const BnRef bnf = bn_ref(li, name, (long)B * H * W);
                layer = name + "/bn-relu";
                P3hScale hs0 = h2_scale(h2_xbound(0));
                if (lean) hs0.a_inv = h2_a_inv_x(0);
                if (pool_planes)
                    timed("p3_pack_kernel", 0.0, [&] { return p3_pack_launch(c->p("rx0" + sfx), nullptr, nullptr, bnf, nullptr, 1, lean ? nullptr : c->p("rx0" + sfx), c->p("p3" + sfx), B, 56, 112, 64, s, p3_fmt(), &hs0); });
                else
                    timed("bn_apply_relu_kernel", 0.0, [&] { return bn_apply_relu_launch(c->p("rx0" + sfx), nullptr, nullptr, bnf, nullptr, c->p("rx0" + sfx), (long)B * 56 * 112, 64, s); });
            } else if (fused) {
                H = 112; W = 224;
                layer = name + "+pool";
                timed("stempool_kernel", 2.0 * B * H * W * 64 * 224, [&] {
                    return stempool_launch(c->p("xpad" + sfx), c->p("pk:" + name + "/weights"), c->v(name + "/bn/gamma"), c->p("rx0" + sfx), bn_acc(li), B, s); });
                const BnRef bnf = bn_ref(li, name, (long)B * H * W);
                layer = name + "/bn-relu";
                timed("bn_apply_relu_kernel", 0.0, [&] { return bn_apply_relu_launch(c->p("rx0" + sfx), nullptr, nullptr, bnf, nullptr, c->p("rx0" + sfx), (long)B * 56 * 112, 64, s); });
            } else {
            IgemmDesc d = conv_desc(c->p("xpad" + sfx), 229, 454, 4, 4, c->p("pk:" + name + "/weights"), 7, 8, 2, 2, false, 64,
                                    c->p("y0" + sfx), 64, H, W);
            d.stats = bn_acc(li);
            layer = name;
            contract(d);
            const BnRef bn = bn_ref(li, name, (long)B * H * W);
            if (c->use_p3 && c->p3_from_stage <= 2)
            {
                P3hScale hs0 = h2_scale(h2_xbound(0));
                if (lean) hs0.a_inv = h2_a_inv_x(0);
                timed("p3_maxpool_kernel", 0.0, [&] { return p3_maxpool_launch(c->p("y0" + sfx), nullptr, nullptr, bn, lean ? nullptr : c->p("rx0" + sfx), c->p("p3" + sfx), B, H, W, 64, s, p3_fmt(), &hs0); });
            }
            else
                timed("maxpool3x3s2_kernel", 0.0, [&] { return maxpool3x3s2_launch(c->p("y0" + sfx), nullptr, nullptr, bn, c->p("rx0" + sfx), B, H, W, 64, s); });
            }
            ++li;
            H = (H + 1) / 2; W = (W + 1) / 2;
        }
        float* xin = c->p("rx0" + sfx);
        float* xout = c->p("rx1" + sfx);
        int cin = 64;
        const int couts[4] = {64, 128, 256, 512};
        bool x_in_planes = pool_planes;
        int xb_par = 0;
        bool x_fp32_valid = !lean;
        for (int st = 0; st < 4; ++st) {
            const int cout = couts[st];
            for (int unit = 1; unit <= 2; ++unit) {
                const std::string pfx = scope + "/conv" + std::to_string(st + 2) + "_" + std::to_string(unit);
                const bool first = unit == 1 && cin != cout;
                const int stride = first ? 2 : 1;
                int Ho = 0, Wo = 0;
                const float* shortcut = xin;
                const bool p3_here = c->use_p3 && st + 2 >= c->p3_from_stage;
                void* planes = p3_here ? (void*)c->p((lean ? "p3b" : "p3") + sfx) : nullptr;
                void* const xplanes = p3_here ? (void*)c->p("p3" + sfx) : nullptr;
                const float* const x_ai = lean ? h2_a_inv_x(xb_par) : nullptr;
                const void* in_planes = (p3_here && x_in_planes) ? xplanes : nullptr;
                if (first) {
                    IgemmDesc d = conv_desc(xin, H, W, cin, cin, c->p("pk:" + pfx + "/shortcut/weights"), 1, 1, 2, 2, true,
                                            cout, c->p("rsc" + sfx), cout, Ho, Wo);
                    if (!x_fp32_valid) d.x = nullptr;
                    if (in_planes) {
                        d.xp3 = in_planes;
                        d.p3_np = B * H * (W + 1);
                        auto hs = c->h2_slot.find(pfx + "/shortcut");
                        if (h2() && hs != c->h2_slot.end()) {
                            d.xp3_fmt = 1;
                            d.xp3_cstride = (unsigned)((size_t)d.p3_np * 64);
                            d.xp3_bytes = (unsigned)p3h_bytes(B, H, W, cin);
                            d.wh2 = c->p("pkh:" + pfx + "/shortcut/weights");
                            d.wh2_bytes = (unsigned)((size_t)d.N * d.Kpad * 4);
                            d.h2_a_inv = x_ai ? x_ai : h2_a_inv();
                            d.h2_w_inv = c->p("h2s") + hs->second;
                        } else {
                            d.xp3_cstride = (unsigned)((size_t)d.p3_np * 96);
                            d.xp3_bytes = (unsigned)p3_bytes(B, H, W, cin);
                        }
                    }
                    if (h2() && p3_here) d.stats = bn_acc(20 + st);
                    layer = pfx + "/shortcut";
                    gemm(d, 1, false);
                    shortcut = c->p("rsc" + sfx);
                }
                conv_bn(x_fp32_valid ? xin : nullptr, H, W, cin, pfx + "/conv_1", 3, stride, cout, BnRef(), c->p("ry1" + sfx), Ho, Wo, li, "", in_planes, x_ai);
                const BnRef bn1 = bn_ref(li, pfx + "/conv_1", (long)B * Ho * Wo);
                ++li;
                int H2, W2;
                if (p3_here) {
                    layer = pfx + "/bn1-relu";
                    P3hScale hs1 = h2_scale();
                    if (lean) hs1.a_inv = h2_a_inv_b();
                    timed("p3_pack_kernel", 0.0, [&] { return p3_pack_launch(c->p("ry1" + sfx), nullptr, nullptr, bn1, nullptr, 1, nullptr, planes, B, Ho, Wo, cout, s, p3_fmt(), &hs1); });
                    conv_bn(nullptr, Ho, Wo, cout, pfx + "/conv_2", 3, 1, cout, BnRef(), c->p("ry2" + sfx), H2, W2, li, "", planes, lean ? h2_a_inv_b() : nullptr);
                    const BnRef bn2 = bn_ref(li, pfx + "/conv_2", (long)B * Ho * Wo);
                    layer = pfx + "/merge";
                    const bool to_next_stage = unit == 2 && c->use_p3g && st < 3;
                    const bool next_p3 = unit == 1 || to_next_stage;
                    P3hScale hs2 = first ? h2_scale(h2_xbound(xb_par ^ 1), nullptr, bn_acc(20 + st), 1.0 / ((double)B * Ho * Wo))
                                         : h2_scale(h2_xbound(xb_par ^ 1), h2_xbound(xb_par));
                    const bool res_planes = lean && !first;
                    const bool y_fp32 = lean ? !next_p3 : !to_next_stage;
                    if (lean) {
                        hs2.a_inv = h2_a_inv_x(xb_par ^ 1);
                        if (res_planes) { hs2.res_planes = xplanes; hs2.res_a_inv = h2_a_inv_x(xb_par); }
                    }
                    xb_par ^= 1;
                    timed("p3_pack_kernel", 0.0, [&] { return p3_pack_launch(c->p("ry2" + sfx), nullptr, nullptr, bn2, res_planes ? nullptr : shortcut, 1, y_fp32 ? xout : nullptr, next_p3 ? xplanes : nullptr, B, Ho, Wo, cout, s, p3_fmt(), &hs2); });
                    x_in_planes = next_p3;
                    x_fp32_valid = y_fp32;
                    ++li;
                    std::swap(xin, xout);
                    H = Ho; W = Wo; cin = cout;
                    continue;
                }
                const std::string l2 = pfx + "/conv_2";
                auto run_prologue = [&] { conv_bn(c->p("ry1" + sfx), Ho, Wo, cout, l2, 3, 1, cout, bn1, c->p("ry2" + sfx), H2, W2, li); };
                auto run_materialized = [&](const std::string& key) {
                    layer = pfx + "/bn1-relu";
                    timed("bn_apply_relu_kernel", 0.0, [&] { return bn_apply_relu_launch(c->p("ry1" + sfx), nullptr, nullptr, bn1, nullptr, c->p("ry1n" + sfx), (long)B * Ho * Wo, cout, s); });
                    conv_bn(c->p("ry1n" + sfx), Ho, Wo, cout, l2, 3, 1, cout, BnRef(), c->p("ry2" + sfx), H2, W2, li, key);
                };
                if (c->tuning && !rc) {
                    run_prologue();
                    const float t_pro = c->plan[l2].us;
                    (void)hipEventRecord(c->tune_e0, s);
                    (void)bn_apply_relu_launch(c->p("ry1" + sfx), nullptr, nullptr, bn1, nullptr, c->p("ry1n" + sfx), (long)B * Ho * Wo, cout, s);
                    (void)hipEventRecord(c->tune_e1, s);
                    (void)hipEventSynchronize(c->tune_e1);
                    float ms = 0.f;
                    (void)hipEventElapsedTime(&ms, c->tune_e0, c->tune_e1);
                    if (!rc && hipMemsetAsync(bn_acc(li), 0, (size_t)2 * cout * sizeof(double), s) != hipSuccess) rc = fail(SAGEN_ERR_HIP, "memset failed");
                    run_materialized(l2 + "#mat");
                    const float t_mat = c->plan[l2 + "#mat"].us + ms * 1e3f;
                    c->materialize[l2] = t_mat < t_pro;
                    if (!c->materialize[l2] && !rc) {
                        if (hipMemsetAsync(bn_acc(li), 0, (size_t)2 * cout * sizeof(double), s) != hipSuccess) rc = fail(SAGEN_ERR_HIP, "memset failed");
                        c->tuning = false; run_prologue(); c->tuning = true;
                    }
                } else if (c->materialize.count(l2) && c->materialize[l2]) {
                    run_materialized(l2 + "#mat");
                } else {
                    run_prologue();
                }
                const BnRef bn2 = bn_ref(li, pfx + "/conv_2", (long)B * Ho * Wo);
                layer = pfx + "/merge";
                const bool planes_out = unit == 2 && st < 3 && c->use_p3g && c->use_p3 && st + 3 >= c->p3_from_stage;
                if (planes_out)
                    timed("p3_pack_kernel", 0.0, [&] { return p3_pack_launch(c->p("ry2" + sfx), nullptr, nullptr, bn2, shortcut, 1, nullptr, c->p("p3" + sfx), B, Ho, Wo, cout, s); });
                else
                    timed("bn_apply_relu_kernel", 0.0, [&] { return bn_apply_relu_launch(c->p("ry2" + sfx), nullptr, nullptr, bn2, shortcut, xout, (long)B * Ho * Wo, cout, s); });
                x_in_planes = planes_out;
                x_fp32_valid = !planes_out;
                ++li;
                std::swap(xin, xout);
                H = Ho; W = Wo; cin = cout;
            }
        }
        return xin;
    }

// ... 143 lines not shown
```

### spatialaudiogen_amd/csrc/model.hip

```cpp
#include "model.h"

void sagen_destroy_impl(sagen_ctx* c);
int sagen_groups_impl(const sagen_ctx* c) { return c->G; }
int sagen_create_impl(sagen_ctx** out, const sagen_config* cfg, int groups) {
    if (!out || !cfg) return fail(SAGEN_ERR_NULL, "sagen_create: null argument");
    if (groups < 1 || groups > SAGEN_MAX_GROUPS) return fail(SAGEN_ERR_SHAPE, "sagen_create_grouped: groups=%d (1..%d)", groups, SAGEN_MAX_GROUPS);
    if (groups > 1 && cfg->separation != SAGEN_SEP_FREQ_MASK)
        return fail(SAGEN_ERR_UNSUPPORTED, "sagen_create_grouped: the grouped launch covers the FREQ_MASK path only");
    if (cfg->batch <= 0) return fail(SAGEN_ERR_SHAPE, "sagen_create: batch=%d", cfg->batch);
    if (!(cfg->encoders & SAGEN_ENC_AUDIO))
        return fail(SAGEN_ERR_UNSUPPORTED, "the audio encoder is mandatory (reference model.py:207)");
    if (cfg->audio_rate != 48000 || cfg->video_rate != 10 || cfg->context != 1.0f || cfg->sample_duration != 0.1f ||
        cfg->fft_window != 0.025f)
        return fail(SAGEN_ERR_UNSUPPORTED,
                    "HIP path implements audio_rate=48000 video_rate=10 context=1.0 sample_duration=0.1 "
                    "fft_window=0.025 (the geometry of every BASELINE config)");
    if (cfg->ambi_order != 1 && cfg->ambi_order != 2)
        return fail(SAGEN_ERR_UNSUPPORTED, "ambi_order=%d (supported: 1, 2; order 3 would need audio_encoder/conv1 with cin = 9, "
                    "which the contraction kernels do not take)", cfg->ambi_order);
    if (cfg->separation != SAGEN_SEP_NONE && cfg->separation != SAGEN_SEP_FREQ_MASK)
        return fail(SAGEN_ERR_UNSUPPORTED, "unknown separation mode %d", cfg->separation);
    if (cfg->separation == SAGEN_SEP_NONE && cfg->num_sep_tracks > 1)
        return fail(SAGEN_ERR_UNSUPPORTED, "separation 'none' decodes the mono track only: num_sep_tracks must be 1 (got %d); the reference's fc3 "
                    "would be [.., 3*(num_sep_tracks+1)] (model.py:254) against a single separated track (model.py:274-280)", cfg->num_sep_tracks);
    if (cfg->separation == SAGEN_SEP_FREQ_MASK && cfg->num_sep_tracks != 16 && cfg->num_sep_tracks != 32 &&
        cfg->num_sep_tracks != 64)
        return fail(SAGEN_ERR_UNSUPPORTED, "num_sep_tracks=%d (supported 16/32/64)", cfg->num_sep_tracks);
    if (cfg->n_loc_units < 0 || cfg->n_loc_units > 4) return fail(SAGEN_ERR_SHAPE, "n_loc_units=%d", cfg->n_loc_units);
    for (int i = 0; i < cfg->n_loc_units; ++i)
        if (cfg->loc_units[i] <= 0 || cfg->loc_units[i] % 4) return fail(SAGEN_ERR_UNSUPPORTED, "loc_units[%d]=%d must be a positive multiple of 4", i, cfg->loc_units[i]);

    sagen_ctx* c = new sagen_ctx();
    c->G = groups;

    c->fp32_only = getenv("SAGEN_FP32_ONLY") != nullptr;
    c->use_p3 = !c->fp32_only && getenv("SAGEN_NO_P3") == nullptr;
    if (const char* e = getenv("SAGEN_P3_FROM_STAGE")) c->p3_from_stage = atoi(e);
    c->stem_fused = getenv("SAGEN_NO_STEMPOOL") == nullptr && (getenv("SAGEN_ONE_STREAM") == nullptr || getenv("SAGEN_STEMPOOL") != nullptr);
    c->stem8 = getenv("SAGEN_NO_STEM8") == nullptr;
    c->stem16 = getenv("SAGEN_NO_STEM16") == nullptr;
    c->stem8h = getenv("SAGEN_NO_STEM8_H2") == nullptr;
    c->use_h2 = getenv("SAGEN_NO_H2") == nullptr;
    c->train_h2 = getenv("SAGEN_TRAIN_NO_H2") == nullptr;
    c->train_h2d = getenv("SAGEN_TRAIN_NO_H2D") == nullptr;
    c->train_h2w = getenv("SAGEN_TRAIN_NO_H2W") == nullptr;
    c->sk_fused = getenv("SAGEN_SK_FUSED") != nullptr;
    c->no_dh_split = getenv("SAGEN_NO_DH_SPLIT") != nullptr;
    c->no_aud_planes = getenv("SAGEN_NO_AUDIO_PLANES") != nullptr;
    if (const char* e = getenv("SAGEN_TUNE_GROUPS")) c->tune_groups = atoi(e);
    c->no_scatter = getenv("SAGEN_NO_DECONV_SCATTER") != nullptr;
    c->train_bands = getenv("SAGEN_TRAIN_NO_BANDS") == nullptr;
    c->train_rawpool = getenv("SAGEN_TRAIN_NO_RAWPOOL") == nullptr;
    c->no_d1_planes = getenv("SAGEN_NO_DECONV1_PLANES") != nullptr;
    c->no_lean_trunk = getenv("SAGEN_NO_LEAN_TRUNK") != nullptr;
    if (getenv("SAGEN_NO_DECODER_PLANES") != nullptr) c->dec_planes_min_batch = 1 << 30;
    if (getenv("SAGEN_P3_FROM_STAGE") == nullptr) c->p3_from_stage = (c->use_h2 && c->use_p3) ? 2 : 3;
    c->use_p3g = c->use_p3 && (getenv("SAGEN_P3G") != nullptr || (c->use_h2 && getenv("SAGEN_NO_P3G") == nullptr));
    c->cfg = *cfg;
    c->B = cfg->batch;
    c->has_video = cfg->encoders & SAGEN_ENC_VIDEO;
    c->has_flow = cfg->encoders & SAGEN_ENC_FLOW;
    c->freq_mask = cfg->separation == SAGEN_SEP_FREQ_MASK;
    c->nsep = c->freq_mask ? cfg->num_sep_tracks : 1;
    c->nin = cfg->ambi_order * cfg->ambi_order;
    c->nout = (cfg->ambi_order + 1) * (cfg->ambi_order + 1) - cfg->ambi_order * cfg->ambi_order;
    const int B = c->B;

    c->enc_h[0] = 127; c->enc_w[0] = 1024; c->enc_c[0] = c->nin;
    for (int l = 0; l < 5; ++l) {
        c->enc_h[l + 1] = (c->enc_h[l] - AENC_K[l][0]) / AENC_S[l][0] + 1;
        c->enc_w[l + 1] = (c->enc_w[l] - AENC_K[l][1]) / AENC_S[l][1] + 1;
        c->enc_c[l + 1] = AENC_F[l];
    }
    c->Cb = 1024 + (c->has_video ? 512 : 0) + (c->has_flow ? 512 : 0);

    {
        int cin = c->nin;
        for (int l = 0; l < 5; ++l) {
            const std::string n = "audio_encoder/conv" + std::to_string(l + 1);
            c->add_var(n + "/weights", {AENC_K[l][0], AENC_K[l][1], cin, AENC_F[l]});
            c->add_var(n + "/biases", {AENC_F[l]});
            cin = AENC_F[l];
        }
        if (c->has_video) add_resnet_vars(c, "video_encoder");
        if (c->has_flow) add_resnet_vars(c, "flow_encoder");
        c->add_var("bottleneck/audio-fc/weights", {c->enc_w[5] * c->enc_c[5], 1024});
        c->add_var("bottleneck/audio-fc/biases", {1024});
        for (const char* e : {"video", "flow"}) {
            if ((std::string(e) == "video" && !c->has_video) || (std::string(e) == "flow" && !c->has_flow)) continue;
            c->add_var(std::string("bottleneck/") + e + "-fc-red/weights", {512, 128});
            c->add_var(std::string("bottleneck/") + e + "-fc-red/biases", {128});
            c->add_var(std::string("bottleneck/") + e + "-fc/weights", {7 * 14 * 128, 512});
            c->add_var(std::string("bottleneck/") + e + "-fc/biases", {512});
        }
        int fin = c->Cb;
        for (int i = 0; i < cfg->n_loc_units; ++i) {
            const std::string n = "localization/fc" + std::to_string(i + 1);
            c->add_var(n + "/weights", {fin, cfg->loc_units[i]});
            c->add_var(n + "/biases", {cfg->loc_units[i]});
            fin = cfg->loc_units[i];
        }
        const int nlast = c->nout * c->nin * (c->nsep + 1);
        const std::string n = "localization/fc" + std::to_string(cfg->n_loc_units + 1);
        c->add_var(n + "/weights", {fin, nlast});
        c->add_var(n + "/biases", {nlast});
        if (c->freq_mask) {
            c->add_var("separation/fc-feats/weights", {c->Cb, 512});
// ... 67 lines not shown
    c->alloc("bott", (size_t)B * 3 * c->Cb);
    for (int i = 0; i < cfg->n_loc_units; ++i) c->alloc("loc" + std::to_string(i + 1), (size_t)B * 3 * cfg->loc_units[i]);
    c->alloc("coeffs", (size_t)B * 3 * c->nout * c->nin * (c->nsep + 1));
    {
        struct L { std::string name; int rows, K, N; };
        std::vector<L> ls;
        ls.push_back({"bottleneck/audio-fc", 3 * B, c->enc_w[5] * c->enc_c[5], 1024});
        if (c->has_video) ls.push_back({"bottleneck/video-fc", B, 7 * 14 * 128, 512});
        if (c->has_flow) ls.push_back({"bottleneck/flow-fc", B, 7 * 14 * 128, 512});
        int fin = c->Cb;
        for (int i = 0; i < cfg->n_loc_units; ++i) { ls.push_back({"localization/fc" + std::to_string(i + 1), 3 * B, fin, cfg->loc_units[i]}); fin = cfg->loc_units[i]; }
        ls.push_back({"localization/fc" + std::to_string(cfg->n_loc_units + 1), 3 * B, fin, c->nout * c->nin * (c->nsep + 1)});
        if (c->freq_mask) ls.push_back({"separation/fc-feats", 3 * B, c->Cb, 512});
        bool ok = getenv("SAGEN_FCM") != nullptr && !c->sk_fused && 3 * B <= FCM_MAX_M;
        for (const L& l : ls) ok = ok && fcm_pick_slices(l.K, (long)l.K * l.N) > 0;
        c->use_fcm = ok;
        if (ok)
            for (const L& l : ls) {
                int ns = fcm_pick_slices(l.K, (long)l.K * l.N);
                if (l.name == "separation/fc-feats") ns = c->fcm_slices.at("localization/fc1");
                c->fcm_slices[l.name] = ns;
                c->alloc("fcm:" + l.name, (size_t)ns * l.rows * l.N);
            }
    }
    c->alloc("splitk", std::max<size_t>((size_t)16 << 20, (size_t)B * 56 * 112 * 64 * 2));
    if (c->freq_mask) {
        c->alloc("cat1p", (p3h_bytes(B, 7, c->enc_w[1], 2 * c->enc_c[1]) + 3) / 4 + 64);
        {
            size_t mx = 0;
            for (int l = 2; l <= 5; ++l) mx = std::max(mx, p3h_bytes(B, c->enc_h[l], c->enc_w[l], 2 * c->enc_c[l]));
            c->alloc("catp", (mx + 3) / 4 + 64);
        }
        {
            size_t mx = 0;
            for (int l = 1; l <= 4; ++l) mx = std::max(mx, p3h_bytes(B, c->enc_h[l], c->enc_w[l], c->enc_c[l]));
            c->alloc("aencp", (mx + 3) / 4 + 64);
        }
        c->alloc("amax", 10 * H2_AMAX_FLOATS + 64);
        c->alloc("dmask", (size_t)B * 23 * 1024 * c->nsep * c->nin);
        c->alloc("frames", (c->nin == 1 ? mask_istft_scratch_bytes(B) : mask_istft_hoa_scratch_bytes(B, c->nout)) / sizeof(float));
    }
    c->alloc("splitk_aux", (size_t)8 << 20);
    c->alloc("splitk:tk", SK_TICKETS);
    c->alloc("splitk_aux:tk", SK_TICKETS);
    for (int set = 0; set < 2; ++set) {
        const std::string x = set ? "_b" : "";
        if (set == 0 ? !(c->has_video || c->has_flow) : !(c->has_video && c->has_flow)) continue;
        c->alloc("xpad" + x, (size_t)B * 229 * 456 * 4);
        c->alloc("s16:part" + x, STEM16_PARTS + 64);
        c->alloc("y0" + x, (size_t)B * 112 * 224 * 64);
        const size_t stage = (size_t)B * 56 * 112 * 64;
        for (const char* nm : {"rx0", "rx1", "ry1", "ry2", "rsc", "ry1n"}) c->alloc(nm + x, stage);
        c->alloc("p3" + x, (p3_bytes(B, 56, 112, 64) + 3) / 4 + 64);
        c->alloc("p3b" + x, (p3h_bytes(B, 56, 112, 64) + 3) / 4 + 64);
        c->alloc("bnacc" + x, (size_t)24 * 2 * 512 * 2);
        c->alloc("fcred" + x, (size_t)B * 98 * 128);
        const std::string enc = (set == 1 || !c->has_video) ? "flow_encoder" : "video_encoder";
        c->expose(enc + "/conv5_2", "rx0" + x, 0, {B, 7, 14, 512}, 512);
    }
    c->bufs["dmask_or_scratch_flush"] = c->freq_mask ? c->bufs.at("dmask") : c->bufs.at("splitk_aux");
    c->expose("mag", "mag", 0, {B, 127, 1024, c->nin}, c->nin);
    c->expose("stft", "spec", 0, {B, c->nin * 28, 513, 2}, 2);
    for (int l = 1; l <= 5; ++l) {
        const int ce = c->enc_c[l];
        c->expose("audio_encoder/conv" + std::to_string(l), "cat" + std::to_string(l), l == 5 ? 0 : ce,
                  {B, c->enc_h[l], c->enc_w[l], ce}, 2 * ce);
    }
    c->expose("bottleneck", "bott", 0, {B, 3, c->Cb}, c->Cb);
    c->expose("localization/coeffs", "coeffs", 0, {B, 3, c->nout * c->nin, c->nsep + 1}, c->nsep + 1);
    if (c->freq_mask) c->expose("separation/deconv1", "dmask", 0, {B, 23, 1024, c->nsep * c->nin}, c->nsep * c->nin);
    int prio_lo = 0, prio_hi = 0;
    (void)hipDeviceGetStreamPriorityRange(&prio_lo, &prio_hi);
    const char* aux_prio = getenv("SAGEN_AUX_PRIO");
    const int prio = aux_prio && aux_prio[0] == 'l' ? prio_lo : (aux_prio && aux_prio[0] == 'h' ? prio_hi : 0);
    if ((aux_prio ? hipStreamCreateWithPriority(&c->aux, hipStreamNonBlocking, prio) : hipStreamCreateWithFlags(&c->aux, hipStreamNonBlocking)) != hipSuccess ||
        hipEventCreateWithFlags(&c->ev_fork, hipEventDisableTiming) != hipSuccess ||
        hipEventCreateWithFlags(&c->ev_stft, hipEventDisableTiming) != hipSuccess ||
        hipEventCreateWithFlags(&c->ev_pack, hipEventDisableTiming) != hipSuccess ||
        hipEventCreateWithFlags(&c->ev_join, hipEventDisableTiming) != hipSuccess) {
        (void)hipGetLastError();
        c->aux = nullptr;
    }
    c->grp_floats = c->ws_floats - c->grp_off;
    c->ws_floats = c->grp_off + (size_t)c->G * c->grp_floats;
    if (c->G > 1 && (c->use_fcm || c->sk_fused || c->fp32_only || !c->use_h2 || !c->use_p3 || !c->use_p3g || c->p3_from_stage > 2 || c->no_lean_trunk)) {
        sagen_destroy_impl(c);
        return fail(SAGEN_ERR_UNSUPPORTED, "sagen_create_grouped: the grouped launch runs the default kernels only (an environment switch selected others)");
    }
    *out = c;
    return SAGEN_OK;
}

int sagen_bind_impl(sagen_ctx* c, const sagen_tensor* tensors, int n, void* workspace, size_t workspace_bytes,
                    hipStream_t s) {
    if (!c || !tensors || !workspace) return fail(SAGEN_ERR_NULL, "sagen_bind_weights: null argument");
    if (workspace_bytes < c->ws_floats * sizeof(float))
        return fail(SAGEN_ERR_WORKSPACE, "workspace has %zu bytes, need %zu", workspace_bytes, c->ws_floats * sizeof(float));
    if (((uintptr_t)workspace) % 256) return fail(SAGEN_ERR_WORKSPACE, "workspace must be 256-byte aligned");
    c->ws = (float*)workspace;
    std::vector<const float*> ptr(c->vars.size(), nullptr);
    for (int i = 0; i < n; ++i) {
        const sagen_tensor& t = tensors[i];
        if (!t.name || !t.data) return fail(SAGEN_ERR_NULL, "tensor %d has a null name or data pointer", i);
        auto it = c->var_index.find(t.name);
        if (it == c->var_index.end()) continue;
        const VarSpec& vs = c->vars[it->second];
        bool ok = t.ndim == vs.ndim;
// ... 519 lines not shown
    if (out.size() + 1 > buflen) return fail(SAGEN_ERR_WORKSPACE, "plan description needs %zu bytes", out.size() + 1);
    memcpy(buf, out.c_str(), out.size() + 1);
    return n;
}

int sagen_profile_enable_impl(sagen_ctx* c, int on) {
    c->profiling = on != 0;
    c->prof.clear();
    c->events_used = 0;
    return SAGEN_OK;
}

int sagen_profile_report_impl(sagen_ctx* c, char* buf, size_t buflen) {
    std::string out;
    for (const ProfRec& r : c->prof) {
        float ms = 0.f;
        hipError_t e = hipEventSynchronize(r.e1);
        if (e == hipSuccess) e = hipEventElapsedTime(&ms, r.e0, r.e1);
        if (e != hipSuccess) return fail(SAGEN_ERR_HIP, "profile: %s", hipGetErrorString(e));
        char line[512];
        snprintf(line, sizeof line, "%s\t%s\t%.3f\t%.6g\n", r.kernel.c_str(), r.layer.c_str(), ms * 1e3, r.flops);
        out += line;
    }
    if (out.size() + 1 > buflen) return fail(SAGEN_ERR_WORKSPACE, "profile report needs %zu bytes", out.size() + 1);
    memcpy(buf, out.c_str(), out.size() + 1);
    return (int)c->prof.size();
}
size_t sagen_workspace_bytes_impl(const sagen_ctx* c) { return c->ws_floats * sizeof(float); }
int sagen_num_variables_impl(const sagen_ctx* c) { return (int)c->vars.size(); }
int sagen_variable_spec_impl(const sagen_ctx* c, int i, const char** name, int32_t* ndim, int64_t shape[4]) {
    if (i < 0 || i >= (int)c->vars.size()) return fail(SAGEN_ERR_SHAPE, "variable index %d out of range", i);
    *name = c->vars[i].name.c_str();
    *ndim = c->vars[i].ndim;
    for (int k = 0; k < 4; ++k) shape[k] = c->vars[i].shape[k];
    return SAGEN_OK;
}
int sagen_set_option_impl(sagen_ctx* c, const char* name, int value) {
    const std::string n = name;
    if (n == "materialize_mask") { c->materialize_mask = value != 0; return SAGEN_OK; }
    if (n == "intermediate_group") {
        if (value < 0 || value >= c->G) return fail(SAGEN_ERR_SHAPE, "intermediate_group=%d of %d groups", value, c->G);
        c->inter_group = value;
        return SAGEN_OK;
    }
    if (n == "u8_fast_stem") { c->stem8 = value != 0; return SAGEN_OK; }
    if (n == "f16_fast_stem") { c->stem16 = value != 0; return SAGEN_OK; }
    if (n == "u8_stem_h2") { c->stem8h = value != 0; return SAGEN_OK; }
    if (n == "train_bands") { c->train_bands = value != 0; return SAGEN_OK; }
    if (n == "train_rawpool") { c->train_rawpool = value != 0; return SAGEN_OK; }
    if (n == "fp16x2") { c->use_h2 = value != 0; return SAGEN_OK; }
    if (n == "planes_from_stage") { if (value < 2 || value > 6) return fail(SAGEN_ERR_SHAPE, "planes_from_stage in 2..6"); c->p3_from_stage = value; return SAGEN_OK; }
    if (n == "decoder_planes") { c->dec_planes_min_batch = value ? 1 : (1 << 30); return SAGEN_OK; }
    if (n == "plane_gather") { c->use_p3g = c->use_p3 && value != 0; return SAGEN_OK; }
    return fail(SAGEN_ERR_UNSUPPORTED, "sagen_set_option: unknown option %s", name);
}

int sagen_counter_impl(sagen_ctx* c, const char* name, uint64_t* value, hipStream_t s) {
    if (!c->ws) return fail(SAGEN_ERR_WORKSPACE, "no workspace bound");
    if (std::string(name) != "fp16x2_saturations") return fail(SAGEN_ERR_UNSUPPORTED, "sagen_counter: unknown counter %s", name);
    unsigned v[SAGEN_MAX_GROUPS] = {0};
    for (int g = 0; g < c->G; ++g)
        SAGEN_HIP_CHECK(hipMemcpyAsync(&v[g], c->p("h2s") + (size_t)g * c->grp_floats + 7, sizeof(unsigned), hipMemcpyDeviceToHost, s));
    SAGEN_HIP_CHECK(hipStreamSynchronize(s));
    uint64_t tot = 0;
    for (int g = 0; g < c->G; ++g) tot += v[g];
    *value = tot;
    return SAGEN_OK;
}

int sagen_get_intermediate_impl(const sagen_ctx* c, const char* name, const float** data, int32_t* ndim, int64_t shape[4],
                                int64_t* pixel_stride) {
    if (!c->ws) return fail(SAGEN_ERR_WORKSPACE, "no workspace bound");
    auto it = c->named.find(name);
    if (it == c->named.end()) return fail(SAGEN_ERR_SHAPE, "unknown intermediate %s", name);
    const Named& nm = it->second;
    if (c->mask_fused_last && std::string(name) == "separation/deconv1")
        return fail(SAGEN_ERR_UNSUPPORTED, "separation/deconv1: the last forward fused the mask into the deconvolution's epilogue - "
                    "sagen_set_option(ctx, \"materialize_mask\", 1) keeps the logits");
    *data = c->ws + nm.buf.off + nm.extra_off + (size_t)c->inter_group * c->grp_floats;
    *ndim = nm.ndim;
    for (int k = 0; k < 4; ++k) shape[k] = nm.shape[k];
    *pixel_stride = nm.pixel_stride;
    return SAGEN_OK;
}
```

### spatialaudiogen_amd/csrc/p3.hip

```cpp
#include "igemm3_common.h"
#include "h2_planes.h"

namespace sagen {

size_t p3_bytes(int B, int H, int W, int C) { return (size_t)(C / 16) * B * H * (W + 1) * 96; }

constexpr int P3_MAX_C = 512;
__device__ __forceinline__ void p3_bn_table(const float* scale, const float* shift, const BnRef& bn, int C, float (*tab)[P3_MAX_C]) {
    for (int c = threadIdx.x; c < C; c += blockDim.x) {
        float sc = 1.f, sh = 0.f;
        if (bn.acc != nullptr) {
            const double mean = bn.acc[c] * bn.inv_count;
            double var = bn.acc[C + c] * bn.inv_count - mean * mean;
            var = var < 0.0 ? 0.0 : var;
            const double a = (double)bn.gamma[c] / sqrt(var + (double)bn.eps);
            sc = (float)a;
            sh = (float)((double)bn.beta[c] - mean * a);
        } else if (scale != nullptr) {
            sc = scale[c];
            sh = shift[c];
        }
        tab[0][c] = sc;
        tab[1][c] = sh;
    }
    __syncthreads();
}

__device__ __forceinline__ void p3_split8(float (&v)[8], u32x4& hi, u32x4& mid, u32x4& lo) {
#pragma unroll
    for (int k = 0; k < 4; ++k) hi[k] = split_pair(v[2 * k], v[2 * k + 1]);
#pragma unroll
    for (int k = 0; k < 4; ++k) mid[k] = split_pair(v[2 * k], v[2 * k + 1]);
#pragma unroll
    for (int k = 0; k < 4; ++k) lo[k] = split_pair(v[2 * k], v[2 * k + 1]);
}

__device__ __forceinline__ void p3_store(char* p3, long cstride, long pp, int c8, const u32x4& hi, const u32x4& mid, const u32x4& lo) {
    char* dst = p3 + (long)(c8 >> 1) * cstride + pp * 96 + (c8 & 1) * 16;
    *reinterpret_cast<u32x4*>(dst) = hi;
    *reinterpret_cast<u32x4*>(dst + 32) = mid;
    *reinterpret_cast<u32x4*>(dst + 64) = lo;
}

size_t p3h_bytes(int B, int H, int W, int C) { return (size_t)(C / 16) * B * H * (W + 1) * 64; }


template <bool H2>
__device__ __forceinline__ float p3_tables(const float* scale, const float* shift, const BnRef& bn, const P3hScale& h, bool has_res, int C,
                                           float (*tab)[P3_MAX_C], unsigned* s_bits) {
    if (H2 && threadIdx.x < 4) s_bits[threadIdx.x] = 0u;
    if (H2) __syncthreads();
    float m = 0.f, mr = 0.f, mg = 0.f, mrg = 0.f;
    const float sqn = H2 && bn.acc != nullptr ? (float)sqrt(1.0 / bn.inv_count) : 0.f;
    const float sqn_r = H2 && has_res && h.res_acc != nullptr ? (float)sqrt(1.0 / h.res_inv_count) : 0.f;
    for (int c = threadIdx.x; c < C; c += blockDim.x) {
        float sc = 1.f, sh = 0.f;
        if (bn.acc != nullptr) {
            const double mean = bn.acc[c] * bn.inv_count;
            double var = bn.acc[C + c] * bn.inv_count - mean * mean;
            var = var < 0.0 ? 0.0 : var;
            const double inv = 1.0 / sqrt(var + (double)bn.eps);
            const double a = (double)bn.gamma[c] * inv;
            sc = (float)a;
            sh = (float)((double)bn.beta[c] - mean * a);
            if (H2) {
                const float gs = fabsf(bn.gamma[c]) * (float)(sqrt(var) * inv);
                m = fmaxf(m, fabsf(bn.beta[c]) + 8.f * gs);
                mg = fmaxf(mg, fabsf(bn.beta[c]) + sqn * gs);
                if (has_res && h.res_acc != nullptr) {
                    const double rm = h.res_acc[c] * h.res_inv_count;
                    double rv = h.res_acc[C + c] * h.res_inv_count - rm * rm;
                    rv = rv < 0.0 ? 0.0 : rv;
                    mr = fmaxf(mr, (float)(fabs(rm) + 8.0 * sqrt(rv)));
                    mrg = fmaxf(mrg, (float)(fabs(rm) + (double)sqn_r * sqrt(rv)));
                }
            }
        } else if (scale != nullptr) {
            sc = scale[c];
            sh = shift[c];
        }
        tab[0][c] = sc;
        tab[1][c] = sh;
    }
    if (H2 && bn.acc != nullptr) {
        m = wave_max_f(m); mr = wave_max_f(mr); mg = wave_max_f(mg); mrg = wave_max_f(mrg);
        if ((threadIdx.x & 63) == 0) {
            atomicMax(&s_bits[0], __builtin_bit_cast(unsigned, m));
            atomicMax(&s_bits[1], __builtin_bit_cast(unsigned, mr));
            atomicMax(&s_bits[2], __builtin_bit_cast(unsigned, mg));
            atomicMax(&s_bits[3], __builtin_bit_cast(unsigned, mrg));
        }
    }
    __syncthreads();
    if (!H2) return 1.f;
    float bound = __builtin_bit_cast(float, s_bits[0]) + __builtin_bit_cast(float, s_bits[1]);
    float rig = __builtin_bit_cast(float, s_bits[2]) + __builtin_bit_cast(float, s_bits[3]);
    if (has_res && h.res_acc == nullptr && h.res_bound != nullptr) { bound += h.res_bound[0]; rig += h.res_bound[H2_RIG_OFF]; }
    if (blockIdx.x == 0 && threadIdx.x == 0 && h.bound_out != nullptr) { h.bound_out[0] = bound; h.bound_out[H2_RIG_OFF] = rig; }
    const unsigned b = __builtin_bit_cast(unsigned, bound);
    const int e = (int)((b >> 23) & 0xff);
    float sa = 1.f;
    if (bn.acc != nullptr && e != 0 && e != 255) {
        int k = 127 + 9 - e;
        const float q = 64000.f / rig;
        const int eq = (int)((__builtin_bit_cast(unsigned, q) >> 23) & 0xff);
        if (eq != 0 && eq != 255) k = min(k, eq - 127);
        sa = __builtin_bit_cast(float, (unsigned)(127 + max(-60, min(60, k))) << 23);
    }
    if (blockIdx.x == 0 && threadIdx.x == 0 && h.a_inv) h.a_inv[0] = 1.f / sa;
    return sa;
}

template <bool H2>
__global__ __launch_bounds__(256) void p3_pack_kernel(const float* __restrict__ x_, const float* __restrict__ scale_,
                                                      const float* __restrict__ shift_, const BnRef bn_,
                                                      const float* __restrict__ res_, int relu, float* __restrict__ y_,
                                                      char* p3_, long nrows, int W, int C, const P3hScale h2_, const GroupInfo gi) {
    const float* __restrict__ x = SAGEN_GRP(x_);
    const float* __restrict__ scale = SAGEN_GRP(scale_);
    const float* __restrict__ shift = SAGEN_GRP(shift_);
    const float* __restrict__ res = SAGEN_GRP(res_);
    float* __restrict__ y = SAGEN_GRP(y_);
    char* p3 = SAGEN_GRP(p3_);
    BnRef bn = bn_;
    bn.acc = SAGEN_GRP(bn.acc);
    P3hScale h2 = h2_;
    h2.a_inv = SAGEN_GRP(h2.a_inv); h2.res_bound = SAGEN_GRP(h2.res_bound); h2.res_acc = SAGEN_GRP(h2.res_acc);
    h2.bound_out = SAGEN_GRP(h2.bound_out); h2.sat_count = SAGEN_GRP(h2.sat_count); h2.relu_bits = SAGEN_GRP(h2.relu_bits);
    h2.res_planes = SAGEN_GRP(h2.res_planes); h2.res_a_inv = SAGEN_GRP(h2.res_a_inv);
    const int C8 = C >> 3;
    const long total = nrows * (W + 1) * C8;
    const long cstride = nrows * (W + 1) * (H2 ? 64 : 96);
    __shared__ unsigned s_bits[4];
    const long t0 = (long)blockIdx.x * 256 + threadIdx.x;
    const int c8 = (int)(t0 % C8);
    __shared__ __attribute__((aligned(16))) float tab[2][P3_MAX_C];
    const char* const resp = H2 ? reinterpret_cast<const char*>(h2.res_planes) : nullptr;
    const float sa = p3_tables<H2>(scale, shift, bn, h2, res != nullptr || resp != nullptr, C, tab, s_bits);
    const float r_inv = resp ? h2.res_a_inv[0] : 0.f;
    const float4 sc0 = *reinterpret_cast<const float4*>(&tab[0][8 * c8]), sc1 = *reinterpret_cast<const float4*>(&tab[0][8 * c8 + 4]);
    const float4 sh0 = *reinterpret_cast<const float4*>(&tab[1][8 * c8]), sh1 = *reinterpret_cast<const float4*>(&tab[1][8 * c8 + 4]);
    for (long i = t0; i < total; i += (long)gridDim.x * 256) {
        const long pp = i / C8;
        const long row = pp / (W + 1);
        const int w = (int)(pp - row * (W + 1));
        float v[8];
        if (w < W) {
            const long e = (row * W + w) * C + 8 * c8;
            const float4 a = *reinterpret_cast<const float4*>(x + e), b = *reinterpret_cast<const float4*>(x + e + 4);
            v[0] = fmaf(a.x, sc0.x, sh0.x); v[1] = fmaf(a.y, sc0.y, sh0.y); v[2] = fmaf(a.z, sc0.z, sh0.z); v[3] = fmaf(a.w, sc0.w, sh0.w);
            v[4] = fmaf(b.x, sc1.x, sh1.x); v[5] = fmaf(b.y, sc1.y, sh1.y); v[6] = fmaf(b.z, sc1.z, sh1.z); v[7] = fmaf(b.w, sc1.w, sh1.w);
            if (res) {
                const float4 ra = *reinterpret_cast<const float4*>(res + e), rb = *reinterpret_cast<const float4*>(res + e + 4);
                v[0] += ra.x; v[1] += ra.y; v[2] += ra.z; v[3] += ra.w; v[4] += rb.x; v[5] += rb.y; v[6] += rb.z; v[7] += rb.w;
            }
            if (H2 && resp) {
                typedef _Float16 h8 __attribute__((ext_vector_type(8)));
                const char* src = resp + (long)(c8 >> 1) * cstride + pp * 64 + (c8 & 1) * 16;
                const h8 rh = *reinterpret_cast<const h8*>(src), rl = *reinterpret_cast<const h8*>(src + 32);
#pragma unroll
                for (int k = 0; k < 8; ++k) v[k] += ((float)rh[k] + (float)rl[k]) * r_inv;
            }
            if (relu) {
#pragma unroll
                for (int k = 0; k < 8; ++k) v[k] = fmaxf(v[k], 0.f);
            }
            if (y) {
                *reinterpret_cast<float4*>(y + e) = make_float4(v[0], v[1], v[2], v[3]);
                *reinterpret_cast<float4*>(y + e + 4) = make_float4(v[4], v[5], v[6], v[7]);
            }
            if (h2.relu_bits) {
                unsigned bits = 0u;
#pragma unroll
                for (int k = 0; k < 8; ++k) bits |= (v[k] > 0.f ? 1u : 0u) << k;
                h2.relu_bits[e >> 3] = (unsigned char)bits;
            }
        } else {
#pragma unroll
            for (int k = 0; k < 8; ++k) v[k] = 0.f;
        }
        if (p3) {
            if (H2) {
                p3h_store(p3, cstride, pp, c8, v, sa, h2.sat_count);
            } else {
                u32x4 hi, mid, lo;
                p3_split8(v, hi, mid, lo);
                p3_store(p3, cstride, pp, c8, hi, mid, lo);
            }
        }
    }
}

static int aligned_grid(long total, int unit_threads, int amort = 1) {
    long g = std::min<long>(cdiv(total, 256L * amort), 256L * 8);
    long a = 256, b = unit_threads;
    while (b) { const long t = a % b; a = b; b = t; }
    const long unit = unit_threads / a;
    g = std::max<long>(unit, g / unit * unit);
    return (int)g;
}

int p3_pack_launch(const float* x, const float* scale, const float* shift, const BnRef& bn, const float* residual, int relu,
                   float* y, void* p3, int B, int H, int W, int C, hipStream_t s, int fmt, const P3hScale* h2) {
    if (C % 16 || C > P3_MAX_C) return fail(SAGEN_ERR_UNSUPPORTED, "p3_pack: C=%d must be a multiple of 16, at most %d", C, P3_MAX_C);
    if (!y && !p3) return fail(SAGEN_ERR_NULL, "p3_pack: no output");
    const long nrows = (long)B * H;
    if (p3_bytes(B, H, W, C) >= (1UL << 31)) return fail(SAGEN_ERR_UNSUPPORTED, "p3_pack: tensor exceeds 2 GiB buffer addressing");
    const long total = nrows * (W + 1) * (C / 8);
    if (fmt == 1 && p3 && !(h2 && h2->a_inv)) return fail(SAGEN_ERR_NULL, "p3_pack: the fp16x2 format needs a slot for its scale");
    static const int amort_env = getenv("SAGEN_P3_AMORT") ? atoi(getenv("SAGEN_P3_AMORT")) : 0;
    const int amort = amort_env > 0 ? amort_env : 4;
    const GroupInfo gi = cur_group();
    if (fmt == 1)
        hipLaunchKernelGGL(p3_pack_kernel<true>, dim3(aligned_grid(total, C / 8, amort), 1, gi.G), dim3(256), 0, s, x, scale, shift, bn, residual, relu, y,
                           (char*)p3, nrows, W, C, *h2, gi);
    else
        hipLaunchKernelGGL(p3_pack_kernel<false>, dim3(aligned_grid(total, C / 8, amort), 1, gi.G), dim3(256), 0, s, x, scale, shift, bn, residual, relu, y,
                           (char*)p3, nrows, W, C, P3hScale(), gi);
    SAGEN_LAUNCH_CHECK();
    return SAGEN_OK;
}

__global__ __launch_bounds__(256) void h2_pack_rows_kernel(const float* __restrict__ x_, long x_bstride, long x_rstride, int ldx, int row0, int B, int R,
                                                           int W, int C, const float* __restrict__ amax0_, const float* __restrict__ amax1_,
                                                           char* __restrict__ planes_, float* __restrict__ a_inv_, unsigned* __restrict__ sat_count_, const GroupInfo gi) {
    const float* __restrict__ x = SAGEN_GRP(x_);
    const float* __restrict__ amax0 = SAGEN_GRP(amax0_);
    const float* __restrict__ amax1 = SAGEN_GRP(amax1_);
    char* __restrict__ planes = SAGEN_GRP(planes_);
    float* __restrict__ a_inv = SAGEN_GRP(a_inv_);
    unsigned* __restrict__ sat_count = SAGEN_GRP(sat_count_);
    const int C8 = C >> 3;
    const long NP = (long)B * R * (W + 1);
    const long total = NP * C8;
    float bound = amax0[H2_AMAX_STRIDE * (threadIdx.x & (H2_AMAX_SLOTS - 1))];
    if (amax1) bound = fmaxf(bound, amax1[H2_AMAX_STRIDE * (threadIdx.x & (H2_AMAX_SLOTS - 1))]);
    bound = wave_max_f(bound);
    const float sa = h2_scale_of_bound(bound);
    if (blockIdx.x == 0 && threadIdx.x == 0) a_inv[0] = 1.f / sa;
    for (long i = (long)blockIdx.x * 256 + threadIdx.x; i < total; i += (long)gridDim.x * 256) {
        const long pp = i / C8;
        const int c8 = (int)(i - pp * C8);
        const long row = pp / (W + 1);
        const int w = (int)(pp - row * (W + 1));
        float v[8];
        if (w < W) {
            const long b = row / R;
            const int r = (int)(row - b * R);
            const float* src = x + b * x_bstride + (long)(row0 + r) * x_rstride + (long)w * ldx + 8 * c8;
            const float4 a = *reinterpret_cast<const float4*>(src), bq = *reinterpret_cast<const float4*>(src + 4);
            v[0] = a.x; v[1] = a.y; v[2] = a.z; v[3] = a.w; v[4] = bq.x; v[5] = bq.y; v[6] = bq.z; v[7] = bq.w;
        } else {
#pragma unroll
            for (int k = 0; k < 8; ++k) v[k] = 0.f;
        }
        p3h_store(planes, NP * 64, pp, c8, v, sa, sat_count);
    }
}

int h2_pack_rows_launch(const float* x, long x_bstride, long x_rstride, int ldx, int row0, int B, int R, int W, int C, const float* amax0,
                        const float* amax1, void* planes, float* a_inv, unsigned* sat_count, hipStream_t s) {
    if (!x || !amax0 || !planes || !a_inv) return fail(SAGEN_ERR_NULL, "h2_pack_rows: null argument");
    if (C % 16 || ldx % 4 || ((uintptr_t)x % 16)) return fail(SAGEN_ERR_UNSUPPORTED, "h2_pack_rows: C %% 16, ldx %% 4 and a 16-byte aligned tensor are required");
    const long total = (long)B * R * (W + 1) * (C / 8);
    const GroupInfo gi = cur_group();
    hipLaunchKernelGGL(h2_pack_rows_kernel, dim3((int)std::min<long>(cdiv(total, 256), 2048), 1, gi.G), dim3(256), 0, s, x, x_bstride, x_rstride, ldx, row0,
                       B, R, W, C, amax0, amax1, (char*)planes, a_inv, sat_count, gi);
    SAGEN_LAUNCH_CHECK();
    return SAGEN_OK;
}

// ... 88 lines not shown
```

Measured before the change: 3251.

## Add space-to-depth fp16x2 plane layout for stride-2 trunk convs

Adds a space-to-depth packed plane format written by the pack kernel at stage boundaries, plus a new conv3s kernel (with the shared conv3h body moved into a header) that consumes it for the stride-2 first conv and shortcut of the next stage. The aim is to let stride-2 3x3 convs run as dense stride-1 style loads on phase-split planes instead of the slower strided path. This costs a second pack pass when tuning or when both layouts are needed, a larger staging buffer, and new tile plan choices. Enabled by default, with an env var and an option to turn it off.

```diff
diff --git a/spatialaudiogen_amd/build.py b/spatialaudiogen_amd/build.py
--- a/spatialaudiogen_amd/build.py
+++ b/spatialaudiogen_amd/build.py
@@ -7,7 +7,7 @@
 CSRC = os.path.join(HERE, 'csrc')
 OBJ = os.path.join(CSRC, 'build')
 LIB = os.path.join(HERE, 'libsagen_hip.so')
-SOURCES = ['conv3p.hip', 'conv3h.hip', 'conv3g.hip', 'p3.hip', 'igemm3dw.hip', 'igemm3s2.hip', 'stempool.hip', 'stem8.hip', 'igemm.hip', 'fcm.hip', 'igemm3.hip', 'elementwise.hip', 'fft.hip', 'eval.hip', 'evalx.hip', 'render.hip', 'overlay.hip', 'train.hip', 'wgrad.hip', 'wgrad3h.hip', 'backward.hip', 'model.hip', 'train_model.hip', 'api.hip']
+SOURCES = ['conv3p.hip', 'conv3h.hip', 'conv3s.hip', 'conv3g.hip', 'p3.hip', 'igemm3dw.hip', 'igemm3s2.hip', 'stempool.hip', 'stem8.hip', 'igemm.hip', 'fcm.hip', 'igemm3.hip', 'elementwise.hip', 'fft.hip', 'eval.hip', 'evalx.hip', 'render.hip', 'overlay.hip', 'train.hip', 'wgrad.hip', 'wgrad3h.hip', 'backward.hip', 'model.hip', 'train_model.hip', 'api.hip']
 HEADERS = sorted(os.path.join(CSRC, h) for h in os.listdir(CSRC) if h.endswith('.h')) + \
           [os.path.join(os.path.dirname(os.path.dirname(CSRC)), 'include', 'sagen.h')]
 FLAGS = ['--offload-arch=gfx950', '-O3', '-std=c++17', '-fPIC', '-Wall', '-Wno-unused-function', '-fno-slp-vectorize', '-fno-vectorize']
diff --git a/spatialaudiogen_amd/csrc/conv3h.hip b/spatialaudiogen_amd/csrc/conv3h.hip
--- a/spatialaudiogen_amd/csrc/conv3h.hip
+++ b/spatialaudiogen_amd/csrc/conv3h.hip
@@ -1,355 +1,6 @@
-#include "igemm3_common.h"
-#include "h2_planes.h"
+#include "conv3h_body.h"
 
 namespace sagen {
-
-typedef _Float16 f16x8 __attribute__((ext_vector_type(8)));
-
-constexpr int conv3h_lds(int BM, int BN, int KC, int AR = 2) { return KC * (AR * BM * 64 + 2 * 3 * 2 * BN * 32); }
-constexpr int conv3h_wgs_per_cu(int BM, int BN, int KC, int AR = 2) {
-    return 160 * 1024 / conv3h_lds(BM, BN, KC, AR) >= 3 ? 3 : (160 * 1024 / conv3h_lds(BM, BN, KC, AR) >= 2 ? 2 : 1);
-}
-
-template <int BM, int BN, int WM, int WN, int KC, int AR>
-__device__ __forceinline__ void conv3h_body(const IgemmDesc& d) {
-    static_assert(AR == 2 || AR == 3, "activation ring of two or three stages");
-    constexpr int MT = WM / 32, NT = WN / 32;
-    constexpr int WAVES_N = BN / WN, WAVES_M = BM / WM;
-    static_assert(WAVES_N * WAVES_M == 4, "4 waves per workgroup");
-    constexpr int BME = BM - 2;
-    constexpr int A_INST = BM / 16;
-    constexpr int B_IPT = BN / 16;
-    constexpr int B_INST = 3 * B_IPT;
-    constexpr int A_PW = (A_INST + 3) / 4, B_PW = (B_INST + 3) / 4;
-    constexpr int A_BYTES = A_INST * 1024, B_BYTES = B_INST * 1024;
-    constexpr int ST_BYTES = KC * (A_BYTES + B_BYTES);
-    constexpr int NM1 = 3 * MT * NT;
-    constexpr int NMG = 3 * KC * NM1;
-    constexpr int SPT = A_PW + B_PW;
-    constexpr int CNT_MAX = KC * SPT;
-    static_assert(CNT_MAX <= NMG, "one DMA slot per MFMA slot at most");
-    constexpr int NF = 2 * (MT + NT);
-    constexpr int SMEM_BYTES = KC * (AR * A_BYTES + 2 * B_BYTES);
-    static_assert(SMEM_BYTES == conv3h_lds(BM, BN, KC, AR), "occupancy bound uses the same footprint");
-    static_assert(AR == 2 || A_INST % 4 == 0, "counted vmcnt: every wave issues the same number of activation instructions");
-    auto a_stage = [&](int sa) { return AR == 2 ? sa * ST_BYTES : sa * (KC * A_BYTES); };
-    auto b_stage = [&](int sb) { return AR == 2 ? sb * ST_BYTES + KC * A_BYTES : AR * KC * A_BYTES + sb * (KC * B_BYTES); };
-    __shared__ __attribute__((aligned(16))) char smem[SMEM_BYTES];
-
-    const int tid = threadIdx.x;
-#ifdef SAGEN_TRACE
-    const size_t trc_wg = ((size_t)blockIdx.z * gridDim.y + blockIdx.y) * gridDim.x + blockIdx.x;
-    unsigned long long* const trc = (d.trace && trc_wg < 8192) ? (unsigned long long*)d.trace + trc_wg * 8 : nullptr;
-#define C3H_TRC(k) do { if (trc && tid == 0) trc[k] = __builtin_amdgcn_s_memtime(); } while (0)
-    if (trc && tid == 0) {
-        trc[4] = __builtin_amdgcn_s_getreg((31 << 11) | 4);
-        trc[5] = __builtin_amdgcn_s_getreg((31 << 11) | 20);
-        trc[6] = __builtin_amdgcn_s_memrealtime();
-    }
-    C3H_TRC(0);
-    const int gsel = (blockIdx.y | blockIdx.z) ? -1 : ((int)blockIdx.x == 8 ? 0 : ((int)blockIdx.x == (int)gridDim.x - 64 ? 1 : -1));
-    unsigned long long* const gtr = (d.trace && gsel >= 0) ? (unsigned long long*)d.trace + (size_t)8192 * 8 + (size_t)gsel * 64 * 8 : nullptr;
-    int g_idx = 0;
-#define C3H_GTRC(k) do { if (gtr && tid == 0 && g_idx < 64) gtr[g_idx * 8 + (k)] = __builtin_amdgcn_s_memtime(); } while (0)
-#else
-#define C3H_TRC(k) do { } while (0)
-#define C3H_GTRC(k) do { } while (0)
-#endif
-    const int lane = tid & 63;
-    const int wave = __builtin_amdgcn_readfirstlane(tid >> 6);
-    const int wm = wave / WAVES_N, wn = wave % WAVES_N;
-    const int W = d.Win, H = d.Hin, Wp = W + 1, NP = d.p3_np;
-    const int nchunk = d.Cin >> 4;
-    const bool dhs = d.splitk == 3;
-    const int dh_z = dhs ? (int)blockIdx.y : 0;
-    const int G = (dhs ? 1 : 3) * nchunk / KC;
-    const int nM = (NP + BME - 1) / BME, nN = (d.N + BN - 1) / BN;
-
-    const __amdgpu_buffer_rsrc_t x_rsrc = __builtin_amdgcn_make_buffer_rsrc((void*)d.xp3, 0, d.xp3_bytes, 0x00020000);
-    const __amdgpu_buffer_rsrc_t w_rsrc = __builtin_amdgcn_make_buffer_rsrc((void*)d.wh2, 0, d.wh2_bytes, 0x00020000);
-
-    const float osc = d.h2_a_inv[0] * d.h2_w_inv[0];
-
-    const int xcd = (blockIdx.x + blockIdx.z) & 7;
-    const int per = (nM + 7) >> 3;
-    const int t_run = blockIdx.x >> 3;
-    const int my_tiles = max(min((xcd + 1) * per, nM) - xcd * per, 0) * nN;
-    if (t_run >= my_tiles) return;
-    const int tq = t_run / nN;
-    const int m0 = (xcd * per + tq) * BME;
-    const int n0 = (t_run - tq * nN) * BN;
-
-    unsigned a_v0[A_PW], a_v1[A_PW], a_v2[A_PW], a_cur[A_PW];
-#pragma unroll
-    for (int j = 0; j < A_PW; ++j) {
-        const int inst = wave + 4 * j;
-        const int U = inst * 64 + lane;
-        const int slot = U >> 2, v = U & 3;
-        const int u = v ^ ((slot >> 2) & 3);
-        const int p = m0 - 1 + slot;
-        unsigned bad = 7u;
-        if (inst < A_INST && p >= 0 && p < NP) {
-            const unsigned row = __umulhi((unsigned)p, d.p3_magic_wp);
-            const int h = (int)(row - __umulhi(row, d.p3_magic_h) * (unsigned)H);
-            bad = (h == 0 ? 1u : 0u) | (h == H - 1 ? 4u : 0u);
-        }
-        const int base = p * 64 + u * 16;
-        a_v0[j] = (bad & 1u) ? OOB : (unsigned)(base - Wp * 64);
-        a_v1[j] = (bad & 2u) ? OOB : (unsigned)base;
-        a_v2[j] = (bad & 4u) ? OOB : (unsigned)(base + Wp * 64);
-    }
-    unsigned b_voff[B_PW];
-    int b_tapoff[B_PW];
-#pragma unroll
-    for (int j = 0; j < B_PW; ++j) {
-        const int inst = wave + 4 * j;
-        b_tapoff[j] = __builtin_amdgcn_readfirstlane((inst / B_IPT) * nchunk * d.N * 64);
-        const int r = inst % B_IPT;
-        const int L = r * 64 + lane;
-        const int pl = L / (2 * BN), n = (L >> 1) % BN, half = L & 1;
-        b_voff[j] = (inst < B_INST && n0 + n < d.N) ? (unsigned)((pl * d.N + n0 + n) * 32 + 16 * (half ^ ((n >> 3) & 1))) : OOB;
-    }
-
-    int qa_dh = dh_z, qa_ch = 0, cur_dh = -1, qb_dh = dh_z, qb_ch = 0;
-    unsigned i_asoff = 0, i_bsoff = 0;
-    char* i_astage = smem;
-    char* i_bstage = smem;
-    auto begin_issue_a = [&](int sa) {
-        i_astage = smem + a_stage(sa);
-        if (qa_dh != cur_dh) {
-            cur_dh = qa_dh;
-#pragma unroll
-            for (int j = 0; j < A_PW; ++j) a_cur[j] = qa_dh == 0 ? a_v0[j] : (qa_dh == 1 ? a_v1[j] : a_v2[j]);
-        }
-        i_asoff = (unsigned)qa_ch * d.xp3_cstride;
-        qa_ch += KC;
-        if (qa_ch == nchunk) { qa_ch = 0; ++qa_dh; }
-    };
-    auto begin_issue_b = [&](int sb) {
-        i_bstage = smem + b_stage(sb);
-        i_bsoff = (unsigned)((qb_dh * 3) * nchunk + qb_ch) * (unsigned)(d.N * 64);
-        qb_ch += KC;
-        if (qb_ch == nchunk) { qb_ch = 0; ++qb_dh; }
-    };
-    auto issue_a = [&](int kc, int s) {
-        const int inst = wave + 4 * s;
-        if (A_INST % 4 == 0 || inst < A_INST)
-            dma16(x_rsrc, (float*)(i_astage + kc * A_BYTES + inst * 1024), a_cur[s], i_asoff + (unsigned)kc * d.xp3_cstride);
-    };
-    auto issue_b = [&](int kc, int j) {
-        const int inst = wave + 4 * j;
-        if (4 * (j + 1) <= B_INST || inst < B_INST)
-            dma16(w_rsrc, (float*)(i_bstage + kc * B_BYTES + inst * 1024), b_voff[j], i_bsoff + (unsigned)b_tapoff[j] + (unsigned)(kc * d.N * 64));
-    };
-    auto issue_nth = [&](int n) {
-        if (AR == 2) {
-            const int sg = CNT_MAX - 1 - n;
-            const int kc = sg / SPT, s = sg - kc * SPT;
-            if (s < A_PW) issue_a(kc, s); else issue_b(kc, s - A_PW);
-        } else if (n < KC * B_PW) {
-            issue_b(n / B_PW, n % B_PW);
-        } else {
-            const int m = n - KC * B_PW;
-            issue_a(m / A_PW, m % A_PW);
-        }
-    };
-
-    f32x16 acc[MT][NT];
-#pragma unroll
-    for (int i = 0; i < MT; ++i)
-#pragma unroll
-        for (int j = 0; j < NT; ++j)
-#pragma unroll
-            for (int e = 0; e < 16; ++e) acc[i][j][e] = 0.f;
-
-    const int li = lane & 31, kk = lane >> 5;
-    int a_foff[3][MT];
-#pragma unroll
-    for (int i = 0; i < MT; ++i)
-#pragma unroll
-        for (int dwi = 0; dwi < 3; ++dwi) {
-            const int sl = wm * WM + i * 32 + li + dwi;
-            a_foff[dwi][i] = sl * 64 + 16 * (kk ^ ((sl >> 2) & 3));
-        }
-    const int b_foff = (wn * WN + li) * 32 + 16 * (kk ^ ((li >> 3) & 1));
-    constexpr int TA[3] = {1, 0, 0}, TB[3] = {0, 1, 0};
-
-    int sa = 0, sb = 0;
-    begin_issue_a(0);
-    begin_issue_b(0);
-#pragma unroll
-    for (int n = 0; n < CNT_MAX; ++n) issue_nth(n);
-    if (AR == 3) {
-        begin_issue_a(1);
-#pragma unroll
-        for (int n = KC * B_PW; n < CNT_MAX; ++n) issue_nth(n);
-    }
-
-    auto group = [&](auto issue_tag) {
-        constexpr int ISSUE = decltype(issue_tag)::value;
-        constexpr int NISSUE = ISSUE == 2 ? CNT_MAX : (ISSUE == 1 ? KC * B_PW : 0);
-        const char* st_a = smem + a_stage(sa);
-        const char* st_b = smem + b_stage(sb);
-        f16x8 fq[2][NF];
-        auto load_frag = [&](int buf, int t, int f) {
-            const int kc = t / 3, dwi = t - 3 * kc;
-            const int pl = f / (MT + NT), r = f - pl * (MT + NT);
-            if (r < MT) fq[buf][f] = *reinterpret_cast<const f16x8*>(st_a + kc * A_BYTES + (a_foff[dwi][r] ^ (pl * 32)));
-            else fq[buf][f] = *reinterpret_cast<const f16x8*>(st_b + b_foff + kc * B_BYTES + (dwi * 2 + pl) * (BN * 32) + (r - MT) * 32 * 32);
-        };
-#pragma unroll
-        for (int f = 0; f < NF; ++f) load_frag(0, 0, f);
-        C3H_GTRC(3);
-#pragma unroll
-        for (int t = 0; t < 3 * KC; ++t) {
-            const int cb = t & 1;
-#pragma unroll
-            for (int tt = 0; tt < 3; ++tt)
-#pragma unroll
-                for (int i = 0; i < MT; ++i)
-#pragma unroll
-                    for (int j = 0; j < NT; ++j) {
-                        const int k = (tt * MT + i) * NT + j;
-                        const int idx = t * NM1 + k;
-                        __builtin_amdgcn_sched_barrier(0);
-                        acc[i][j] = __builtin_amdgcn_mfma_f32_32x32x16_f16(fq[cb][TA[tt] * (MT + NT) + i], fq[cb][TB[tt] * (MT + NT) + MT + j],
-                                                                           acc[i][j], 0, 0, 0);
-                        if (t + 1 < 3 * KC) {
-#pragma unroll
-                            for (int f = 0; f < NF; ++f)
-                                if (f * NM1 / NF == k) load_frag(cb ^ 1, t + 1, f);
-                        }
-#pragma unroll
-                        for (int n = 0; n < NISSUE; ++n)
-                            if (idx == n) issue_nth(n);
-                    }
-        }
-        __builtin_amdgcn_sched_barrier(0);
-        C3H_GTRC(4);
-#ifdef SAGEN_TRACE
-        ++g_idx;
-#endif
-        sa = sa + 1 == AR ? 0 : sa + 1;
-        sb ^= 1;
-    };
-
-    C3H_TRC(1);
-    if (AR == 2) {
-        for (int it = 0; it + 1 < G; ++it) {
-            C3H_GTRC(0);
-            asm volatile("s_waitcnt vmcnt(0)" ::: "memory");
-            C3H_GTRC(1);
-            lds_barrier();
-            C3H_GTRC(2);
-            begin_issue_a(sa ^ 1);
-            begin_issue_b(sb ^ 1);
-            group(std::integral_constant<int, 2>{});
-        }
-        asm volatile("s_waitcnt vmcnt(0)" ::: "memory");
-        lds_barrier();
-        group(std::integral_constant<int, 0>{});
-    } else {
-        for (int it = 0; it + 2 < G; ++it) {
-            asm volatile("s_waitcnt vmcnt(%0)" ::"n"(KC * A_PW) : "memory");
-            lds_barrier();
-            begin_issue_b(sb ^ 1);
-            begin_issue_a(sa == 0 ? 2 : sa - 1);
-            group(std::integral_constant<int, 2>{});
-        }
-        asm volatile("s_waitcnt vmcnt(%0)" ::"n"(KC * A_PW) : "memory");
-        lds_barrier();
-        begin_issue_b(sb ^ 1);
-        group(std::integral_constant<int, 1>{});
-        asm volatile("s_waitcnt vmcnt(0)" ::: "memory");
-        lds_barrier();
-        group(std::integral_constant<int, 0>{});
-    }
-
-    C3H_TRC(2);
-    const int colb = n0 + wn * WN + li;
-    const bool plain = d.bias == nullptr && !d.relu_out;
-    const __amdgpu_buffer_rsrc_t y_rsrc = __builtin_amdgcn_make_buffer_rsrc((void*)((char*)d.y + (size_t)dh_z * d.y_bytes), 0, d.y_bytes, 0x00020000);
-    const unsigned ldy4 = (unsigned)d.ldy * 4u;
-    const int plim = min(NP, m0 + BME);
-    float bias_j[NT], cs[NT], cq[NT];
-    unsigned col4[NT];
-#pragma unroll
-    for (int j = 0; j < NT; ++j) {
-        const bool ok = colb + 32 * j < d.N;
-        col4[j] = ok ? (unsigned)(colb + 32 * j) * 4u : OOB;
-        bias_j[j] = (d.bias != nullptr && ok) ? d.bias[colb + 32 * j] : 0.f;
-        cs[j] = 0.f; cq[j] = 0.f;
-    }
-    lds_barrier();
-    unsigned* const s_roff = reinterpret_cast<unsigned*>(smem);
-    for (int r = tid; r < BM; r += 256) {
-        const int p = m0 + r;
-        const unsigned row = __umulhi((unsigned)p, d.p3_magic_wp);
-        s_roff[r] = (p < plim && (unsigned)p - row * (unsigned)Wp < (unsigned)W) ? ((unsigned)p - row) * ldy4 : OOB;
-    }
-    lds_barrier();
-    auto epilogue = [&](auto fast_tag) {
-        constexpr bool FAST = decltype(fast_tag)::value;
-#pragma unroll
-        for (int i = 0; i < MT; ++i)
-#pragma unroll
-            for (int q = 0; q < 4; ++q) {
-                const uint4 ro = *reinterpret_cast<const uint4*>(s_roff + wm * WM + i * 32 + 8 * q + 4 * kk);
-#pragma unroll
-                for (int u = 0; u < 4; ++u) {
-                    const int e = 4 * q + u;
-                    const unsigned rraw = u == 0 ? ro.x : (u == 1 ? ro.y : (u == 2 ? ro.z : ro.w));
-                    const float sc = (rraw & OOB) ? 0.f : osc;
-                    const unsigned roff = FAST ? rraw + (unsigned)(colb * 4) : rraw;
-#pragma unroll
-                    for (int j = 0; j < NT; ++j) {
-                        float v = acc[i][j][e] * sc;
-                        if (i == MT - 1 && e >= 14 && (rraw & OOB)) v = 0.f;
-                        if (FAST) {
-                            cs[j] += v;
-                            cq[j] = __builtin_fmaf(v, v, cq[j]);
-                            __builtin_amdgcn_raw_buffer_store_b32(__builtin_bit_cast(unsigned, v), y_rsrc, roff, 128 * j, 0);
-                        } else {
-                            const unsigned off = ((roff | col4[j]) & OOB) ? OOB : roff + col4[j];
-                            if (col4[j] & OOB) v = 0.f;
-                            cs[j] += v;
-                            cq[j] = __builtin_fmaf(v, v, cq[j]);
-                            v += bias_j[j];
-                            if (d.relu_out) v = fmaxf(v, 0.f);
-                            __builtin_amdgcn_raw_buffer_store_b32(__builtin_bit_cast(unsigned, v), y_rsrc, off, 0, 0);
-                        }
-                    }
-                }
-            }
-    };
-    if (plain && n0 + BN <= d.N) epilogue(std::true_type{});
-    else epilogue(std::false_type{});
-    if (d.stats != nullptr) {
-        float* const red = reinterpret_cast<float*>(smem + BM * 4);
-        static_assert(BM * 4 + WAVES_M * 2 * 2 * BN * 4 <= SMEM_BYTES, "statistics staging must fit the ring");
-#pragma unroll
-        for (int j = 0; j < NT; ++j) {
-            red[((wm * 2 + kk) * 2 + 0) * BN + wn * WN + j * 32 + li] = cs[j];
-            red[((wm * 2 + kk) * 2 + 1) * BN + wn * WN + j * 32 + li] = cq[j];
-        }
-        lds_barrier();
-        for (int t = tid; t < 2 * BN; t += 256) {
-            const int which = t / BN, col = t - which * BN;
-            if (n0 + col < d.N) {
-                float sum = 0.f;
-#pragma unroll
-                for (int g = 0; g < WAVES_M * 2; ++g) sum += red[(g * 2 + which) * BN + col];
-                atomicAdd(&d.stats[(long)which * d.N + n0 + col], (double)sum);
-            }
-        }
-    }
-    C3H_TRC(3);
-#ifdef SAGEN_TRACE
-    if (trc && tid == 0) trc[7] = __builtin_amdgcn_s_memrealtime();
-#endif
-#undef C3H_TRC
-#undef C3H_GTRC
-}
 
 template <int BM, int BN, int WM, int WN, int KC>
 __global__ __launch_bounds__(256, conv3h_wgs_per_cu(BM, BN, KC, 2)) void conv3h_kernel(const IgemmDesc d_in) {
diff --git a/spatialaudiogen_amd/csrc/conv3h_body.h b/spatialaudiogen_amd/csrc/conv3h_body.h
--- /dev/null
+++ b/spatialaudiogen_amd/csrc/conv3h_body.h
@@ -0,0 +1,360 @@
+#pragma once
+#include "igemm3_common.h"
+#include "h2_planes.h"
+
+namespace sagen {
+
+typedef _Float16 f16x8 __attribute__((ext_vector_type(8)));
+
+constexpr int conv3h_lds(int BM, int BN, int KC, int AR = 2, bool S2D = false) { return KC * (AR * (S2D ? 2 : 1) * BM * 64 + 2 * 3 * 2 * BN * 32); }
+constexpr int conv3h_wgs_per_cu(int BM, int BN, int KC, int AR = 2, bool S2D = false) {
+    return 160 * 1024 / conv3h_lds(BM, BN, KC, AR, S2D) >= 3 ? 3 : (160 * 1024 / conv3h_lds(BM, BN, KC, AR, S2D) >= 2 ? 2 : 1);
+}
+
+template <int BM, int BN, int WM, int WN, int KC, int AR, bool S2D = false>
+__device__ __forceinline__ void conv3h_body(const IgemmDesc& d) {
+    static_assert(AR == 2 || AR == 3, "activation ring of two or three stages");
+    constexpr int MT = WM / 32, NT = WN / 32;
+    constexpr int WAVES_N = BN / WN, WAVES_M = BM / WM;
+    static_assert(WAVES_N * WAVES_M == 4, "4 waves per workgroup");
+    constexpr int BME = S2D ? BM - 1 : BM - 2;
+    constexpr int A_IMG = BM / 16;
+    constexpr int A_INST = (S2D ? 2 : 1) * A_IMG;
+    static_assert(!S2D || A_IMG % 4 == 0, "S2D: a wave's DMA slot j belongs to image j / (A_IMG / 4)");
+    constexpr int B_IPT = BN / 16;
+    constexpr int B_INST = 3 * B_IPT;
+    constexpr int A_PW = (A_INST + 3) / 4, B_PW = (B_INST + 3) / 4;
+    constexpr int A_BYTES = A_INST * 1024, B_BYTES = B_INST * 1024;
+    constexpr int ST_BYTES = KC * (A_BYTES + B_BYTES);
+    constexpr int NM1 = 3 * MT * NT;
+    constexpr int NMG = 3 * KC * NM1;
+    constexpr int SPT = A_PW + B_PW;
+    constexpr int CNT_MAX = KC * SPT;
+    static_assert(CNT_MAX <= NMG, "one DMA slot per MFMA slot at most");
+    constexpr int NF = 2 * (MT + NT);
+    constexpr int SMEM_BYTES = KC * (AR * A_BYTES + 2 * B_BYTES);
+    static_assert(SMEM_BYTES == conv3h_lds(BM, BN, KC, AR, S2D), "occupancy bound uses the same footprint");
+    static_assert(AR == 2 || A_INST % 4 == 0, "counted vmcnt: every wave issues the same number of activation instructions");
+    auto a_stage = [&](int sa) { return AR == 2 ? sa * ST_BYTES : sa * (KC * A_BYTES); };
+    auto b_stage = [&](int sb) { return AR == 2 ? sb * ST_BYTES + KC * A_BYTES : AR * KC * A_BYTES + sb * (KC * B_BYTES); };
+    __shared__ __attribute__((aligned(16))) char smem[SMEM_BYTES];
+
+    const int tid = threadIdx.x;
+#ifdef SAGEN_TRACE
+    const size_t trc_wg = ((size_t)blockIdx.z * gridDim.y + blockIdx.y) * gridDim.x + blockIdx.x;
+    unsigned long long* const trc = (d.trace && trc_wg < 8192) ? (unsigned long long*)d.trace + trc_wg * 8 : nullptr;
+#define C3H_TRC(k) do { if (trc && tid == 0) trc[k] = __builtin_amdgcn_s_memtime(); } while (0)
+    if (trc && tid == 0) {
+        trc[4] = __builtin_amdgcn_s_getreg((31 << 11) | 4);
+        trc[5] = __builtin_amdgcn_s_getreg((31 << 11) | 20);
+        trc[6] = __builtin_amdgcn_s_memrealtime();
+    }
+    C3H_TRC(0);
+    const int gsel = (blockIdx.y | blockIdx.z) ? -1 : ((int)blockIdx.x == 8 ? 0 : ((int)blockIdx.x == (int)gridDim.x - 64 ? 1 : -1));
+    unsigned long long* const gtr = (d.trace && gsel >= 0) ? (unsigned long long*)d.trace + (size_t)8192 * 8 + (size_t)gsel * 64 * 8 : nullptr;
+    int g_idx = 0;
+#define C3H_GTRC(k) do { if (gtr && tid == 0 && g_idx < 64) gtr[g_idx * 8 + (k)] = __builtin_amdgcn_s_memtime(); } while (0)
+#else
+#define C3H_TRC(k) do { } while (0)
+#define C3H_GTRC(k) do { } while (0)
+#endif
+    const int lane = tid & 63;
+    const int wave = __builtin_amdgcn_readfirstlane(tid >> 6);
+    const int wm = wave / WAVES_N, wn = wave % WAVES_N;
+    const int W = S2D ? d.Wg : d.Win, H = S2D ? d.Hg : d.Hin, Wp = W + 1, NP = S2D ? d.xs2d_np : d.p3_np;
+    const unsigned xcs = S2D ? (unsigned)NP * 64u : d.xp3_cstride;
+    const int nchunk = d.Cin >> 4;
+    const bool dhs = d.splitk == 3;
+    const int dh_z = dhs ? (int)blockIdx.y : 0;
+    const int G = (dhs ? 1 : 3) * nchunk / KC;
+    const int nM = (NP + BME - 1) / BME, nN = (d.N + BN - 1) / BN;
+
+    const __amdgpu_buffer_rsrc_t x_rsrc = __builtin_amdgcn_make_buffer_rsrc((void*)(S2D ? d.xs2d : d.xp3), 0, S2D ? d.xs2d_bytes : d.xp3_bytes, 0x00020000);
+    const __amdgpu_buffer_rsrc_t w_rsrc = __builtin_amdgcn_make_buffer_rsrc((void*)d.wh2, 0, d.wh2_bytes, 0x00020000);
+
+    const float osc = d.h2_a_inv[0] * d.h2_w_inv[0];
+
+    const int xcd = (blockIdx.x + blockIdx.z) & 7;
+    const int per = (nM + 7) >> 3;
+    const int t_run = blockIdx.x >> 3;
+    const int my_tiles = max(min((xcd + 1) * per, nM) - xcd * per, 0) * nN;
+    if (t_run >= my_tiles) return;
+    const int tq = t_run / nN;
+    const int m0 = (xcd * per + tq) * BME;
+    const int n0 = (t_run - tq * nN) * BN;
+
+    unsigned a_v0[A_PW], a_v1[A_PW], a_v2[A_PW], a_cur[A_PW];
+#pragma unroll
+    for (int j = 0; j < A_PW; ++j) {
+        const int inst = wave + 4 * j;
+        const int U = inst * 64 + lane;
+        const int slot = U >> 2, v = U & 3;
+        const int u = v ^ ((slot >> 2) & 3);
+        const int p = S2D ? m0 + (slot & (BM - 1)) : m0 - 1 + slot;
+        unsigned bad = 7u;
+        if (inst < A_INST && p >= 0 && p < NP) {
+            const unsigned row = __umulhi((unsigned)p, d.p3_magic_wp);
+            const int h = (int)(row - __umulhi(row, d.p3_magic_h) * (unsigned)H);
+            bad = (h == 0 && !S2D ? 1u : 0u) | (h == H - 1 ? 4u : 0u);
+        }
+        const int base = p * 64 + u * 16;
+        a_v0[j] = (bad & 1u) ? OOB : (unsigned)(S2D ? base : base - Wp * 64);
+        a_v1[j] = (bad & 2u) ? OOB : (unsigned)base;
+        a_v2[j] = (bad & 4u) ? OOB : (unsigned)(base + Wp * 64);
+    }
+    unsigned b_voff[B_PW];
+    int b_tapoff[B_PW];
+#pragma unroll
+    for (int j = 0; j < B_PW; ++j) {
+        const int inst = wave + 4 * j;
+        b_tapoff[j] = __builtin_amdgcn_readfirstlane((inst / B_IPT) * nchunk * d.N * 64);
+        const int r = inst % B_IPT;
+        const int L = r * 64 + lane;
+        const int pl = L / (2 * BN), n = (L >> 1) % BN, half = L & 1;
+        b_voff[j] = (inst < B_INST && n0 + n < d.N) ? (unsigned)((pl * d.N + n0 + n) * 32 + 16 * (half ^ ((n >> 3) & 1))) : OOB;
+    }
+
+    int qa_dh = dh_z, qa_ch = 0, cur_dh = -1, qb_dh = dh_z, qb_ch = 0;
+    unsigned i_asoff = 0, i_bsoff = 0;
+    char* i_astage = smem;
+    char* i_bstage = smem;
+    auto begin_issue_a = [&](int sa) {
+        i_astage = smem + a_stage(sa);
+        if (qa_dh != cur_dh) {
+            cur_dh = qa_dh;
+#pragma unroll
+            for (int j = 0; j < A_PW; ++j) a_cur[j] = qa_dh == 0 ? a_v0[j] : (qa_dh == 1 ? a_v1[j] : a_v2[j]);
+        }
+        i_asoff = (unsigned)qa_ch * xcs;
+        if (S2D) i_asoff += (unsigned)((qa_dh & 1) * 2) * ((unsigned)nchunk * xcs);
+        qa_ch += KC;
+        if (qa_ch == nchunk) { qa_ch = 0; ++qa_dh; }
+    };
+    auto begin_issue_b = [&](int sb) {
+        i_bstage = smem + b_stage(sb);
+        i_bsoff = (unsigned)((qb_dh * 3) * nchunk + qb_ch) * (unsigned)(d.N * 64);
+        qb_ch += KC;
+        if (qb_ch == nchunk) { qb_ch = 0; ++qb_dh; }
+    };
+    auto issue_a = [&](int kc, int s) {
+        const int inst = wave + 4 * s;
+        if (A_INST % 4 == 0 || inst < A_INST)
+            dma16(x_rsrc, (float*)(i_astage + kc * A_BYTES + inst * 1024), a_cur[s],
+                  i_asoff + (unsigned)kc * xcs + (S2D && 4 * s >= A_IMG ? (unsigned)nchunk * xcs : 0u));
+    };
+    auto issue_b = [&](int kc, int j) {
+        const int inst = wave + 4 * j;
+        if (4 * (j + 1) <= B_INST || inst < B_INST)
+            dma16(w_rsrc, (float*)(i_bstage + kc * B_BYTES + inst * 1024), b_voff[j], i_bsoff + (unsigned)b_tapoff[j] + (unsigned)(kc * d.N * 64));
+    };
+    auto issue_nth = [&](int n) {
+        if (AR == 2) {
+            const int sg = CNT_MAX - 1 - n;
+            const int kc = sg / SPT, s = sg - kc * SPT;
+            if (s < A_PW) issue_a(kc, s); else issue_b(kc, s - A_PW);
+        } else if (n < KC * B_PW) {
+            issue_b(n / B_PW, n % B_PW);
+        } else {
+            const int m = n - KC * B_PW;
+            issue_a(m / A_PW, m % A_PW);
+        }
+    };
+
+    f32x16 acc[MT][NT];
+#pragma unroll
+    for (int i = 0; i < MT; ++i)
+#pragma unroll
+        for (int j = 0; j < NT; ++j)
+#pragma unroll
+            for (int e = 0; e < 16; ++e) acc[i][j][e] = 0.f;
+
+    const int li = lane & 31, kk = lane >> 5;
+    int a_foff[3][MT];
+#pragma unroll
+    for (int i = 0; i < MT; ++i)
+#pragma unroll
+        for (int dwi = 0; dwi < 3; ++dwi) {
+            const int sl = wm * WM + i * 32 + li + (S2D ? (dwi == 1 ? BM : dwi >> 1) : dwi);
+            a_foff[dwi][i] = sl * 64 + 16 * (kk ^ ((sl >> 2) & 3));
+        }
+    const int b_foff = (wn * WN + li) * 32 + 16 * (kk ^ ((li >> 3) & 1));
+    constexpr int TA[3] = {1, 0, 0}, TB[3] = {0, 1, 0};
+
+    int sa = 0, sb = 0;
+    begin_issue_a(0);
+    begin_issue_b(0);
+#pragma unroll
+    for (int n = 0; n < CNT_MAX; ++n) issue_nth(n);
+    if (AR == 3) {
+        begin_issue_a(1);
+#pragma unroll
+        for (int n = KC * B_PW; n < CNT_MAX; ++n) issue_nth(n);
+    }
+
+    auto group = [&](auto issue_tag) {
+        constexpr int ISSUE = decltype(issue_tag)::value;
+        constexpr int NISSUE = ISSUE == 2 ? CNT_MAX : (ISSUE == 1 ? KC * B_PW : 0);
+        const char* st_a = smem + a_stage(sa);
+        const char* st_b = smem + b_stage(sb);
+        f16x8 fq[2][NF];
+        auto load_frag = [&](int buf, int t, int f) {
+            const int kc = t / 3, dwi = t - 3 * kc;
+            const int pl = f / (MT + NT), r = f - pl * (MT + NT);
+            if (r < MT) fq[buf][f] = *reinterpret_cast<const f16x8*>(st_a + kc * A_BYTES + (a_foff[dwi][r] ^ (pl * 32)));
+            else fq[buf][f] = *reinterpret_cast<const f16x8*>(st_b + b_foff + kc * B_BYTES + (dwi * 2 + pl) * (BN * 32) + (r - MT) * 32 * 32);
+        };
+#pragma unroll
+        for (int f = 0; f < NF; ++f) load_frag(0, 0, f);
+        C3H_GTRC(3);
+#pragma unroll
+        for (int t = 0; t < 3 * KC; ++t) {
+            const int cb = t & 1;
+#pragma unroll
+            for (int tt = 0; tt < 3; ++tt)
+#pragma unroll
+                for (int i = 0; i < MT; ++i)
+#pragma unroll
+                    for (int j = 0; j < NT; ++j) {
+                        const int k = (tt * MT + i) * NT + j;
+                        const int idx = t * NM1 + k;
+                        __builtin_amdgcn_sched_barrier(0);
+                        acc[i][j] = __builtin_amdgcn_mfma_f32_32x32x16_f16(fq[cb][TA[tt] * (MT + NT) + i], fq[cb][TB[tt] * (MT + NT) + MT + j],
+                                                                           acc[i][j], 0, 0, 0);
+                        if (t + 1 < 3 * KC) {
+#pragma unroll
+                            for (int f = 0; f < NF; ++f)
+                                if (f * NM1 / NF == k) load_frag(cb ^ 1, t + 1, f);
+                        }
+#pragma unroll
+                        for (int n = 0; n < NISSUE; ++n)
+                            if (idx == n) issue_nth(n);
+                    }
+        }
+        __builtin_amdgcn_sched_barrier(0);
+        C3H_GTRC(4);
+#ifdef SAGEN_TRACE
+        ++g_idx;
+#endif
+        sa = sa + 1 == AR ? 0 : sa + 1;
+        sb ^= 1;
+    };
+
+    C3H_TRC(1);
+    if (AR == 2) {
+        for (int it = 0; it + 1 < G; ++it) {
+            C3H_GTRC(0);
+            asm volatile("s_waitcnt vmcnt(0)" ::: "memory");
+            C3H_GTRC(1);
+            lds_barrier();
+            C3H_GTRC(2);
+            begin_issue_a(sa ^ 1);
+            begin_issue_b(sb ^ 1);
+            group(std::integral_constant<int, 2>{});
+        }
+        asm volatile("s_waitcnt vmcnt(0)" ::: "memory");
+        lds_barrier();
+        group(std::integral_constant<int, 0>{});
+    } else {
+        for (int it = 0; it + 2 < G; ++it) {
+            asm volatile("s_waitcnt vmcnt(%0)" ::"n"(KC * A_PW) : "memory");
+            lds_barrier();
+            begin_issue_b(sb ^ 1);
+            begin_issue_a(sa == 0 ? 2 : sa - 1);
+            group(std::integral_constant<int, 2>{});
+        }
+        asm volatile("s_waitcnt vmcnt(%0)" ::"n"(KC * A_PW) : "memory");
+        lds_barrier();
+        begin_issue_b(sb ^ 1);
+        group(std::integral_constant<int, 1>{});
+        asm volatile("s_waitcnt vmcnt(0)" ::: "memory");
+        lds_barrier();
+        group(std::integral_constant<int, 0>{});
+    }
+
+    C3H_TRC(2);
+    const int colb = n0 + wn * WN + li;
+    const bool plain = d.bias == nullptr && !d.relu_out;
+    const __amdgpu_buffer_rsrc_t y_rsrc = __builtin_amdgcn_make_buffer_rsrc((void*)((char*)d.y + (size_t)dh_z * d.y_bytes), 0, d.y_bytes, 0x00020000);
+    const unsigned ldy4 = (unsigned)d.ldy * 4u;
+    const int plim = min(NP, m0 + BME);
+    float bias_j[NT], cs[NT], cq[NT];
+    unsigned col4[NT];
+#pragma unroll
+    for (int j = 0; j < NT; ++j) {
+        const bool ok = colb + 32 * j < d.N;
+        col4[j] = ok ? (unsigned)(colb + 32 * j) * 4u : OOB;
+        bias_j[j] = (d.bias != nullptr && ok) ? d.bias[colb + 32 * j] : 0.f;
+        cs[j] = 0.f; cq[j] = 0.f;
+    }
+    lds_barrier();
+    unsigned* const s_roff = reinterpret_cast<unsigned*>(smem);
+    for (int r = tid; r < BM; r += 256) {
+        const int p = m0 + r;
+        const unsigned row = __umulhi((unsigned)p, d.p3_magic_wp);
+        s_roff[r] = (p < plim && (unsigned)p - row * (unsigned)Wp < (unsigned)W) ? ((unsigned)p - row) * ldy4 : OOB;
+    }
+    lds_barrier();
+    auto epilogue = [&](auto fast_tag) {
+        constexpr bool FAST = decltype(fast_tag)::value;
+#pragma unroll
+        for (int i = 0; i < MT; ++i)
+#pragma unroll
+            for (int q = 0; q < 4; ++q) {
+                const uint4 ro = *reinterpret_cast<const uint4*>(s_roff + wm * WM + i * 32 + 8 * q + 4 * kk);
+#pragma unroll
+                for (int u = 0; u < 4; ++u) {
+                    const int e = 4 * q + u;
+                    const unsigned rraw = u == 0 ? ro.x : (u == 1 ? ro.y : (u == 2 ? ro.z : ro.w));
+                    const float sc = (rraw & OOB) ? 0.f : osc;
+                    const unsigned roff = FAST ? rraw + (unsigned)(colb * 4) : rraw;
+#pragma unroll
+                    for (int j = 0; j < NT; ++j) {
+                        float v = acc[i][j][e] * sc;
+                        if (i == MT - 1 && e >= 14 && (rraw & OOB)) v = 0.f;
+                        if (FAST) {
+                            cs[j] += v;
+                            cq[j] = __builtin_fmaf(v, v, cq[j]);
+                            __builtin_amdgcn_raw_buffer_store_b32(__builtin_bit_cast(unsigned, v), y_rsrc, roff, 128 * j, 0);
+                        } else {
+                            const unsigned off = ((roff | col4[j]) & OOB) ? OOB : roff + col4[j];
+                            if (col4[j] & OOB) v = 0.f;
+                            cs[j] += v;
+                            cq[j] = __builtin_fmaf(v, v, cq[j]);
+                            v += bias_j[j];
+                            if (d.relu_out) v = fmaxf(v, 0.f);
+                            __builtin_amdgcn_raw_buffer_store_b32(__builtin_bit_cast(unsigned, v), y_rsrc, off, 0, 0);
+                        }
+                    }
+                }
+            }
+    };
+    if (plain && n0 + BN <= d.N) epilogue(std::true_type{});
+    else epilogue(std::false_type{});
+    if (d.stats != nullptr) {
+        float* const red = reinterpret_cast<float*>(smem + BM * 4);
+        static_assert(BM * 4 + WAVES_M * 2 * 2 * BN * 4 <= SMEM_BYTES, "statistics staging must fit the ring");
+#pragma unroll
+        for (int j = 0; j < NT; ++j) {
+            red[((wm * 2 + kk) * 2 + 0) * BN + wn * WN + j * 32 + li] = cs[j];
+            red[((wm * 2 + kk) * 2 + 1) * BN + wn * WN + j * 32 + li] = cq[j];
+        }
+        lds_barrier();
+        for (int t = tid; t < 2 * BN; t += 256) {
+            const int which = t / BN, col = t - which * BN;
+            if (n0 + col < d.N) {
+                float sum = 0.f;
+#pragma unroll
+                for (int g = 0; g < WAVES_M * 2; ++g) sum += red[(g * 2 + which) * BN + col];
+                atomicAdd(&d.stats[(long)which * d.N + n0 + col], (double)sum);
+            }
+        }
+    }
+    C3H_TRC(3);
+#ifdef SAGEN_TRACE
+    if (trc && tid == 0) trc[7] = __builtin_amdgcn_s_memrealtime();
+#endif
+#undef C3H_TRC
+#undef C3H_GTRC
+}
+
+}
diff --git a/spatialaudiogen_amd/csrc/conv3s.hip b/spatialaudiogen_amd/csrc/conv3s.hip
--- /dev/null
+++ b/spatialaudiogen_amd/csrc/conv3s.hip
@@ -0,0 +1,54 @@
+#include "conv3h_body.h"
+
+namespace sagen {
+
+template <int BM, int BN, int WM, int WN, int KC, int AR, bool S2D>
+__global__ __launch_bounds__(256, conv3h_wgs_per_cu(BM, BN, KC, AR, true)) void conv3h_kernel(const IgemmDesc d_in) {
+    IgemmDesc d = d_in;
+    if (d.grp.G > 1) igemm_relocate(d, (int)blockIdx.z);
+    static_assert(S2D, "the space-to-depth instantiations only");
+    conv3h_body<BM, BN, WM, WN, KC, AR, true>(d);
+}
+
+template <int BM, int BN, int WM, int WN, int KC, int AR>
+static int launch_conv3s(const IgemmDesc& d, hipStream_t s) {
+    if ((d.Cin / 16) % KC) return fail(SAGEN_ERR_UNSUPPORTED, "conv3s: %d channel chunks are not a multiple of %d per group", d.Cin / 16, KC);
+    const int per = (cdiv(d.xs2d_np, BM - 1) + 7) / 8;
+    const int grid = 8 * per * cdiv(d.N, BN);
+    hipLaunchKernelGGL((conv3h_kernel<BM, BN, WM, WN, KC, AR, true>), dim3(grid, 1, d.grp.G), dim3(256), 0, s, d);
+    SAGEN_LAUNCH_CHECK();
+    return SAGEN_OK;
+}
+
+bool conv3s_ok(const IgemmDesc& d) {
+    if (!d.xs2d || d.xs2d_np <= 0 || !d.wh2 || !d.h2_a_inv || !d.h2_w_inv) return false;
+    if (d.ntaps != 9 || d.TW != 3 || d.tap_sh != 1 || d.tap_sw != 1 || d.tap_h0 != 0 || d.tap_w0 != 0 || d.in_sh != 2 || d.in_sw != 2) return false;
+    if ((d.Hin & 1) || (d.Win & 1) || d.Hg * 2 != d.Hin || d.Wg * 2 != d.Win || d.g_h0 != 0 || d.g_w0 != 0 || d.dsh * d.dsw != 1) return false;
+    if (d.Cin % 16 || d.K != 9 * d.Cin || d.Kpad != d.K || d.in_scale != nullptr || d.bn_in.acc != nullptr) return false;
+    if (d.M % (d.Hg * d.Wg) || d.xs2d_np != d.M / d.Wg * (d.Wg + 1)) return false;
+    return d.y_rstride == (long)d.Wg * d.ldy && d.y_bstride == (long)d.Hg * d.Wg * d.ldy;
+}
+
+int conv3s_dispatch(const IgemmDesc& d_in, IgemmTile tile, hipStream_t s) {
+    IgemmDesc d = d_in;
+    if (!conv3s_ok(d)) return fail(SAGEN_ERR_UNSUPPORTED, "conv3s: not a 3x3 stride-2 SAME conv over even sizes with its space-to-depth planes");
+    if (d.splitk != 1) return fail(SAGEN_ERR_UNSUPPORTED, "conv3s: no split-K");
+    if ((long)(d.xs2d_np + 512) * (d.Wg + 1) >= (1L << 32) || ((long)(d.xs2d_np + 512) / (d.Wg + 1) + 1) * d.Hg >= (1L << 32))
+        return fail(SAGEN_ERR_UNSUPPORTED, "conv3s: too many pixels for 32-bit index arithmetic");
+    const long x_bytes = 4L * (d.Cin / 16) * d.xs2d_np * 64;
+    if (x_bytes >= (1L << 31) || d.xs2d_bytes != (unsigned)x_bytes)
+        return fail(SAGEN_ERR_UNSUPPORTED, "conv3s: the activation planes exceed 2 GiB buffer addressing (use a smaller batch) or their extent is wrong");
+    const long y_bytes = ((long)(d.M - 1) * d.ldy + d.N) * 4;
+    if (y_bytes >= (1L << 31)) return fail(SAGEN_ERR_UNSUPPORTED, "conv3s: the output exceeds 2 GiB buffer addressing (use a smaller batch)");
+    d.y_bytes = (unsigned)y_bytes;
+    d.p3_magic_wp = (unsigned)((1UL << 32) / (unsigned)(d.Wg + 1)) + 1u;
+    d.p3_magic_h = (unsigned)((1UL << 32) / (unsigned)d.Hg) + 1u;
+    switch (tile) {
+        case TILE_P3S_128x128: return launch_conv3s<128, 128, 64, 64, 1, 2>(d, s);
+        case TILE_P3SR_128x64: return launch_conv3s<128, 64, 64, 32, 1, 3>(d, s);
+        case TILE_P3SR_256x64: return launch_conv3s<256, 64, 64, 64, 1, 3>(d, s);
+        default: return fail(SAGEN_ERR_UNSUPPORTED, "conv3s: bad tile id %d", (int)tile);
+    }
+}
+
+}
diff --git a/spatialaudiogen_amd/csrc/igemm.hip b/spatialaudiogen_amd/csrc/igemm.hip
--- a/spatialaudiogen_amd/csrc/igemm.hip
+++ b/spatialaudiogen_amd/csrc/igemm.hip
@@ -252,7 +252,7 @@
     return SAGEN_OK;
 }
 
-struct TileCfg { int bm, bn, bk; const char* name; bool split = false; bool dw3 = false; bool s2 = false; bool p3 = false; bool g = false; bool h = false; };
+struct TileCfg { int bm, bn, bk; const char* name; bool split = false; bool dw3 = false; bool s2 = false; bool p3 = false; bool g = false; bool h = false; bool s2d = false; };
 static const TileCfg kTiles[TILE_AUTO] = {
     {128, 128, 16, "igemm_kernel<128,128,64,64,3,16>"}, {128, 64, 16, "igemm_kernel<128,64,64,32,3,16>"},
     {256, 64, 16, "igemm_kernel<256,64,64,64,3,16>"},   {64, 64, 16, "igemm_kernel<64,64,32,32,3,16>"},
@@ -294,6 +294,8 @@
     {256, 64, 16, "conv3hr_kernel<256,64,64,64,1>", true, true, false, true, false, true}, {128, 64, 16, "conv3hr_kernel<128,64,64,32,1>", true, true, false, true, false, true},
     {64, 64, 32, "conv3hr_kernel<64,64,32,32,2>", true, true, false, true, false, true},
     {128, 128, 16, "conv3hr_kernel<128,128,64,64,1>", true, true, false, true, false, true},
+    {128, 128, 16, "conv3h_kernel<128,128,64,64,1,2,true>", true, false, false, true, false, true, true}, {128, 64, 16, "conv3h_kernel<128,64,64,32,1,3,true>", true, false, false, true, false, true, true},
+    {256, 64, 16, "conv3h_kernel<256,64,64,64,1,3,true>", true, false, false, true, false, true, true},
 };
 static bool s2_ok(const IgemmDesc& d) {
     return d.Cin == 4 && d.ldx == 4 && d.ntaps == 56 && d.TW == 8 && d.in_sh == 2 && d.in_sw == 2 && d.tap_sh == 1 && d.tap_sw == 1 &&
@@ -308,8 +310,9 @@
 }
 bool igemm_tile_split(IgemmTile t) { return t >= 0 && t < TILE_AUTO && kTiles[t].split; }
 bool igemm_tile_p3(IgemmTile t) { return t >= 0 && t < TILE_AUTO && kTiles[t].p3; }
+bool igemm_tile_s2d(IgemmTile t) { return t >= 0 && t < TILE_AUTO && kTiles[t].s2d; }
 bool igemm_tile_dh_split(IgemmTile t) {
-    return t >= 0 && t < TILE_AUTO && kTiles[t].p3 && kTiles[t].h && !kTiles[t].g && t != TILE_P3HR_256x64 && t != TILE_P3HR_128x64 && t != TILE_P3HR_64x64_C2 && t != TILE_P3HR_128x128;
+    return t >= 0 && t < TILE_AUTO && kTiles[t].p3 && kTiles[t].h && !kTiles[t].g && !kTiles[t].s2d && t != TILE_P3HR_256x64 && t != TILE_P3HR_128x64 && t != TILE_P3HR_64x64_C2 && t != TILE_P3HR_128x128;
 }
 bool igemm_p3_eligible(const IgemmDesc& d) { return dw3_ok(d) && d.w_split && d.dsh * d.dsw == 1 && d.Cin <= MAX_BN_C; }
 static int tile_bm(IgemmTile t) { return (t >= 0 && t < TILE_AUTO) ? kTiles[t].bm : 0; }
@@ -345,6 +348,7 @@
             return false;
     }
     if (kTiles[t].dw3 && !dw3_ok(d)) return false;
+    if (kTiles[t].s2d) return d.splitk == 1 && d.mm_out == nullptr && conv3s_ok(d);
     if (kTiles[t].p3 && (d.xp3 == nullptr || (d.splitk != 1 && !(d.splitk == 3 && igemm_tile_dh_split(t))))) return false;
     if (kTiles[t].p3 && (kTiles[t].h ? (d.xp3_fmt != 1 || d.wh2 == nullptr) : d.xp3_fmt != 0)) return false;
     if (!kTiles[t].p3 && d.xp3 != nullptr && d.x == nullptr) return false;
@@ -359,6 +363,7 @@
     static const char* force = getenv("SAGEN_FORCE_TILE");
     if (force && d.M > 128 && d.N >= 64 && igemm_tile_ok(d, (IgemmTile)atoi(force))) return (IgemmTile)atoi(force);
     static const bool fp32_only = getenv("SAGEN_FP32_ONLY") != nullptr;
+    if (d.xp3 == nullptr && d.x == nullptr && conv3s_ok(d)) return TILE_P3S_128x128;
     if (d.mm_out != nullptr) return (d.xp3 != nullptr && d.xp3_fmt == 1 && d.wh2 != nullptr && conv3g_ok(d)) ? TILE_P3GH_MM_64x128_K2 : TILE_B3_64x128;
     auto blocks = [&](IgemmTile t) { return (long)cdiv(d.M, tile_bm(t)) * cdiv(d.N, tile_bn(t)) * d.splitk; };
     const long want = 2 * 256;
@@ -411,7 +416,7 @@
 
 int igemm_launch(const IgemmDesc& d_in, IgemmTile tile, hipStream_t s) {
     IgemmDesc d = d_in;
-    if ((!d.x && !d.xp3) || !d.w || (!d.y && !d.splitk_ws)) return fail(SAGEN_ERR_NULL, "igemm: null operand");
+    if ((!d.x && !d.xp3 && !d.xs2d) || !d.w || (!d.y && !d.splitk_ws)) return fail(SAGEN_ERR_NULL, "igemm: null operand");
     if (d.M <= 0 || d.N <= 0 || d.K <= 0) return fail(SAGEN_ERR_SHAPE, "igemm: empty problem M=%d N=%d K=%d", d.M, d.N, d.K);
     if (d.Kpad % 16 || d.Kpad < d.K) return fail(SAGEN_ERR_SHAPE, "igemm: Kpad=%d must be a multiple of 16 >= K=%d", d.Kpad, d.K);
     if (d.K % 4 || d.Cin % 4) return fail(SAGEN_ERR_UNSUPPORTED, "igemm: Cin=%d / K=%d must be multiples of 4", d.Cin, d.K);
@@ -447,6 +452,7 @@
     if (!igemm_tile_ok(d, tile)) return fail(SAGEN_ERR_UNSUPPORTED, "igemm: %s cannot run this problem (Kpad=%d Cin=%d)", igemm_tile_name(tile), d.Kpad, d.Cin);
     d.uniform_taps = uniform_taps_for(d, kTiles[tile].bk) ? 1 : 0;
     if (d.ntaps > MAX_TAPS) return fail(SAGEN_ERR_UNSUPPORTED, "igemm: %d taps (max %d)", d.ntaps, MAX_TAPS);
+    if (kTiles[tile].s2d) return conv3s_dispatch(d, tile, s);
     if (kTiles[tile].g) return conv3g_dispatch(d, tile, s);
     if (kTiles[tile].h) return conv3h_dispatch(d, tile, s);
     if (kTiles[tile].p3) return conv3p_dispatch(d, tile, s);
diff --git a/spatialaudiogen_amd/csrc/kernels.h b/spatialaudiogen_amd/csrc/kernels.h
--- a/spatialaudiogen_amd/csrc/kernels.h
+++ b/spatialaudiogen_amd/csrc/kernels.h
@@ -51,6 +51,9 @@
     int p3_np = 0;
     int xp3_fmt = 0;
     int xp3_row0 = 0, xp3_rows = 0;
+    const void* xs2d = nullptr;
+    unsigned xs2d_bytes = 0;
+    int xs2d_np = 0;
     const void* wh2 = nullptr;
     unsigned wh2_bytes = 0;
     const float* h2_a_inv = nullptr;
@@ -71,7 +74,7 @@
     d.bn_in.acc = grp_ptr(d.bn_in.acc, gi, g);
     d.stats = grp_ptr(d.stats, gi, g); d.amax_out = grp_ptr(d.amax_out, gi, g);
     d.splitk_ws = grp_ptr(d.splitk_ws, gi, g); d.sk_ticket = grp_ptr(d.sk_ticket, gi, g);
-    d.xp3 = grp_ptr(d.xp3, gi, g);
+    d.xp3 = grp_ptr(d.xp3, gi, g); d.xs2d = grp_ptr(d.xs2d, gi, g);
     d.h2_a_inv = grp_ptr(d.h2_a_inv, gi, g); d.h2_w_inv = grp_ptr(d.h2_w_inv, gi, g);
     d.mm_coeffs = grp_ptr(d.mm_coeffs, gi, g); d.mm_out = grp_ptr(d.mm_out, gi, g);
 }
@@ -96,6 +99,7 @@
     TILE_P3GH_MM_64x128_K2, TILE_P3GH_MM_64x128_K4, TILE_P3GH_MM_128x128_K2, TILE_P3GH_MM_128x256_K2,
     TILE_P3HR_256x64, TILE_P3HR_128x64, TILE_P3HR_64x64_C2,
     TILE_P3HR_128x128,
+    TILE_P3S_128x128, TILE_P3SR_128x64, TILE_P3SR_256x64,
     TILE_AUTO
 };
 
@@ -113,6 +117,8 @@
 int conv3p_dispatch(const IgemmDesc& d, IgemmTile tile, hipStream_t s);
 int conv3g_dispatch(const IgemmDesc& d, IgemmTile tile, hipStream_t s);
 int conv3h_dispatch(const IgemmDesc& d, IgemmTile tile, hipStream_t s);
+int conv3s_dispatch(const IgemmDesc& d, IgemmTile tile, hipStream_t s);
+bool conv3s_ok(const IgemmDesc& d);
 int h2_filter_pack_launch(const float* wp, int N, int Kpad, void* w2, unsigned* scratch, float* w_inv, hipStream_t s);
 struct H2Job {
     const float* wp = nullptr;
@@ -126,6 +132,7 @@
 inline bool igemm_tile_fused_splitk(IgemmTile) { return true; }
 bool igemm_tile_p3(IgemmTile t);
 bool igemm_tile_grouped(IgemmTile t);
+bool igemm_tile_s2d(IgemmTile t);
 bool igemm_tile_dh_split(IgemmTile t);
 bool igemm_p3_eligible(const IgemmDesc& d);
 bool igemm_tile_ok(const IgemmDesc& d, IgemmTile t);
@@ -212,8 +219,10 @@
     const float* res_a_inv = nullptr;
 };
 int p3_pack_launch(const float* x, const float* scale, const float* shift, const BnRef& bn, const float* residual, int relu,
-                   float* y, void* p3, int B, int H, int W, int C, hipStream_t s, int fmt = 0, const P3hScale* h2 = nullptr);
+                   float* y, void* p3, int B, int H, int W, int C, hipStream_t s, int fmt = 0, const P3hScale* h2 = nullptr,
+                   int s2d = 0);
 size_t p3h_bytes(int B, int H, int W, int C);
+size_t p3s_bytes(int B, int H, int W, int C);
 int h2_pack_rows_launch(const float* x, long x_bstride, long x_rstride, int ldx, int row0, int B, int R, int W, int C, const float* amax0,
                         const float* amax1, void* planes, float* a_inv, unsigned* sat_count, hipStream_t s);
 int p3_maxpool_launch(const float* x, const float* scale, const float* shift, const BnRef& bn, float* y, void* p3, int B, int H,
diff --git a/spatialaudiogen_amd/csrc/model.h b/spatialaudiogen_amd/csrc/model.h
--- a/spatialaudiogen_amd/csrc/model.h
+++ b/spatialaudiogen_amd/csrc/model.h
@@ -129,6 +129,7 @@
     bool train_rawpool = true;
     bool train_bands = true;
     int dec_lo[7] = {0, 0, 0, 0, 0, 0, 0}, dec_hi[7] = {0, 0, 0, 0, 0, 0, 0};
+    bool use_s2d = true;
     bool no_scatter = false, no_d1_planes = false, no_lean_trunk = false;
     int dec_planes_min_batch = 16;
     bool use_fcm = false;
@@ -560,22 +561,27 @@
 
     void conv_bn(const float* x, int Hin, int Win, int Cin, const std::string& name, int k, int stride, int Cout,
                  const BnRef& bn_in, float* y, int& Hout, int& Wout, int bn_index, const std::string& plan_key = "",
-                 const void* planes = nullptr, const float* planes_a_inv = nullptr) {
+                 const void* planes = nullptr, const float* planes_a_inv = nullptr, const void* s2d_planes = nullptr) {
         if (rc) return;
         IgemmDesc d = conv_desc(x, Hin, Win, Cin, Cin, c->p("pk:" + name + "/weights"), k, k, stride, stride, true, Cout, y,
                                 Cout, Hout, Wout);
-        if (planes) {
+        if (planes || s2d_planes) {
             d.xp3 = planes;
-            d.p3_np = c->B * Hin * (Win + 1);
+            d.p3_np = planes ? c->B * Hin * (Win + 1) : 0;
             auto hs = c->h2_slot.find(name);
             if (h2() && (stride == 1 || c->use_p3g) && k == 3 && hs != c->h2_slot.end()) {
                 d.xp3_fmt = 1;
                 d.xp3_cstride = (unsigned)((size_t)d.p3_np * 64);
-                d.xp3_bytes = (unsigned)p3h_bytes(c->B, Hin, Win, Cin);
+                d.xp3_bytes = planes ? (unsigned)p3h_bytes(c->B, Hin, Win, Cin) : 0u;
                 d.wh2 = c->p("pkh:" + name + "/weights");
                 d.wh2_bytes = (unsigned)((size_t)d.N * d.Kpad * 4);
                 d.h2_a_inv = planes_a_inv ? planes_a_inv : h2_a_inv();
                 d.h2_w_inv = c->p("h2s") + hs->second;
+                if (s2d_planes) {
+                    d.xs2d = s2d_planes;
+                    d.xs2d_np = c->B * (Hin / 2) * (Win / 2 + 1);
+                    d.xs2d_bytes = (unsigned)p3s_bytes(c->B, Hin, Win, Cin);
+                }
             } else {
                 d.xp3_cstride = (unsigned)((size_t)d.p3_np * 96);
                 d.xp3_bytes = (unsigned)p3_bytes(c->B, Hin, Win, Cin);
@@ -675,6 +681,7 @@
         const int couts[4] = {64, 128, 256, 512};
         bool x_in_planes = pool_planes;
         int xb_par = 0;
+        bool x_in_s2d = false, x_in_rows = true;
         bool x_fp32_valid = !lean;
         for (int st = 0; st < 4; ++st) {
             const int cout = couts[st];
@@ -688,8 +695,28 @@
                 void* planes = p3_here ? (void*)c->p((lean ? "p3b" : "p3") + sfx) : nullptr;
                 void* const xplanes = p3_here ? (void*)c->p("p3" + sfx) : nullptr;
                 const float* const x_ai = lean ? h2_a_inv_x(xb_par) : nullptr;
-                const void* in_planes = (p3_here && x_in_planes) ? xplanes : nullptr;
-                if (first) {
+                const void* in_planes = (p3_here && x_in_planes && x_in_rows) ? xplanes : nullptr;
+                const void* const in_s2d = (first && p3_here && x_in_planes && x_in_s2d) ? (void*)c->p("p3b" + sfx) : nullptr;
+                auto shortcut_s2d = [&] {
+                    IgemmDesc d = conv_desc(nullptr, H / 2, W / 2, cin, cin, c->p("pk:" + pfx + "/shortcut/weights"), 1, 1, 1, 1, true,
+                                            cout, c->p("rsc" + sfx), cout, Ho, Wo);
+                    d.xp3 = in_s2d;
+                    d.p3_np = B * (H / 2) * (W / 2 + 1);
+                    d.xp3_fmt = 1;
+                    d.xp3_cstride = (unsigned)((size_t)d.p3_np * 64);
+                    d.xp3_bytes = (unsigned)p3h_bytes(B, H / 2, W / 2, cin);
+                    d.wh2 = c->p("pkh:" + pfx + "/shortcut/weights");
+                    d.wh2_bytes = (unsigned)((size_t)d.N * d.Kpad * 4);
+                    d.h2_a_inv = x_ai;
+                    d.h2_w_inv = c->p("h2s") + c->h2_slot.at(pfx + "/shortcut");
+                    d.stats = bn_acc(20 + st);
+                    layer = pfx + "/shortcut#s2d";
+                    gemm(d, 1, false);
+                };
+                if (first && in_s2d && !in_planes) {
+                    shortcut_s2d();
+                    shortcut = c->p("rsc" + sfx);
+                } else if (first) {
                     IgemmDesc d = conv_desc(xin, H, W, cin, cin, c->p("pk:" + pfx + "/shortcut/weights"), 1, 1, 2, 2, true,
                                             cout, c->p("rsc" + sfx), cout, Ho, Wo);
                     if (!x_fp32_valid) d.x = nullptr;
@@ -713,9 +740,13 @@
                     if (h2() && p3_here) d.stats = bn_acc(20 + st);
                     layer = pfx + "/shortcut";
                     gemm(d, 1, false);
+                    if (in_s2d && !rc) {
+                        if (memset_groups(d.stats, (size_t)2 * d.N * sizeof(double)) != hipSuccess) rc = fail(SAGEN_ERR_HIP, "autotune: memset failed");
+                        shortcut_s2d();
+                    }
                     shortcut = c->p("rsc" + sfx);
                 }
-                conv_bn(x_fp32_valid ? xin : nullptr, H, W, cin, pfx + "/conv_1", 3, stride, cout, BnRef(), c->p("ry1" + sfx), Ho, Wo, li, "", in_planes, x_ai);
+                conv_bn(x_fp32_valid ? xin : nullptr, H, W, cin, pfx + "/conv_1", 3, stride, cout, BnRef(), c->p("ry1" + sfx), Ho, Wo, li, "", in_planes, x_ai, in_s2d);
                 const BnRef bn1 = bn_ref(li, pfx + "/conv_1", (long)B * Ho * Wo);
                 ++li;
                 int H2, W2;
@@ -738,7 +769,19 @@
                         if (res_planes) { hs2.res_planes = xplanes; hs2.res_a_inv = h2_a_inv_x(xb_par); }
                     }
                     xb_par ^= 1;
-                    timed("p3_pack_kernel", 0.0, [&] { return p3_pack_launch(c->p("ry2" + sfx), nullptr, nullptr, bn2, res_planes ? nullptr : shortcut, 1, y_fp32 ? xout : nullptr, next_p3 ? xplanes : nullptr, B, Ho, Wo, cout, s, p3_fmt(), &hs2); });
+                    bool s2d_out = false, rows_out = true;
+                    const std::string next_c1 = scope + "/conv" + std::to_string(st + 3) + "_1/conv_1";
+                    if (lean && to_next_stage && c->use_s2d && !(Ho & 1) && !(Wo & 1) && c->h2_slot.count(next_c1) != 0 &&
+                        c->h2_slot.count(scope + "/conv" + std::to_string(st + 3) + "_1/shortcut") != 0) {
+                        auto it = c->plan.find(next_c1);
+                        s2d_out = c->tuning || (it != c->plan.end() && igemm_tile_s2d((IgemmTile)it->second.tile));
+                        rows_out = c->tuning || !s2d_out;
+                    }
+                    if (s2d_out)
+                        timed("p3_pack_kernel", 0.0, [&] { return p3_pack_launch(c->p("ry2" + sfx), nullptr, nullptr, bn2, res_planes ? nullptr : shortcut, 1, nullptr, c->p("p3b" + sfx), B, Ho, Wo, cout, s, p3_fmt(), &hs2, 1); });
+                    if (rows_out)
+                        timed("p3_pack_kernel", 0.0, [&] { return p3_pack_launch(c->p("ry2" + sfx), nullptr, nullptr, bn2, res_planes ? nullptr : shortcut, 1, y_fp32 ? xout : nullptr, next_p3 ? xplanes : nullptr, B, Ho, Wo, cout, s, p3_fmt(), &hs2); });
+                    x_in_s2d = s2d_out; x_in_rows = rows_out;
                     x_in_planes = next_p3;
                     x_fp32_valid = y_fp32;
                     ++li;
diff --git a/spatialaudiogen_amd/csrc/model.hip b/spatialaudiogen_amd/csrc/model.hip
--- a/spatialaudiogen_amd/csrc/model.hip
+++ b/spatialaudiogen_amd/csrc/model.hip
@@ -53,6 +53,7 @@
     c->train_rawpool = getenv("SAGEN_TRAIN_NO_RAWPOOL") == nullptr;
     c->no_d1_planes = getenv("SAGEN_NO_DECONV1_PLANES") != nullptr;
     c->no_lean_trunk = getenv("SAGEN_NO_LEAN_TRUNK") != nullptr;
+    c->use_s2d = getenv("SAGEN_NO_S2D") == nullptr;
     if (getenv("SAGEN_NO_DECODER_PLANES") != nullptr) c->dec_planes_min_batch = 1 << 30;
     if (getenv("SAGEN_P3_FROM_STAGE") == nullptr) c->p3_from_stage = (c->use_h2 && c->use_p3) ? 2 : 3;
     c->use_p3g = c->use_p3 && (getenv("SAGEN_P3G") != nullptr || (c->use_h2 && getenv("SAGEN_NO_P3G") == nullptr));
@@ -226,7 +227,7 @@
         const size_t stage = (size_t)B * 56 * 112 * 64;
         for (const char* nm : {"rx0", "rx1", "ry1", "ry2", "rsc", "ry1n"}) c->alloc(nm + x, stage);
         c->alloc("p3" + x, (p3_bytes(B, 56, 112, 64) + 3) / 4 + 64);
-        c->alloc("p3b" + x, (p3h_bytes(B, 56, 112, 64) + 3) / 4 + 64);
+        c->alloc("p3b" + x, (std::max(p3h_bytes(B, 56, 112, 64), p3s_bytes(B, 56, 112, 64)) + 3) / 4 + 64);
         c->alloc("bnacc" + x, (size_t)24 * 2 * 512 * 2);
         c->alloc("fcred" + x, (size_t)B * 98 * 128);
         const std::string enc = (set == 1 || !c->has_video) ? "flow_encoder" : "video_encoder";
@@ -852,6 +853,7 @@
     if (n == "planes_from_stage") { if (value < 2 || value > 6) return fail(SAGEN_ERR_SHAPE, "planes_from_stage in 2..6"); c->p3_from_stage = value; return SAGEN_OK; }
     if (n == "decoder_planes") { c->dec_planes_min_batch = value ? 1 : (1 << 30); return SAGEN_OK; }
     if (n == "plane_gather") { c->use_p3g = c->use_p3 && value != 0; return SAGEN_OK; }
+    if (n == "plane_s2d") { c->use_s2d = value != 0; return SAGEN_OK; }
     return fail(SAGEN_ERR_UNSUPPORTED, "sagen_set_option: unknown option %s", name);
 }
 
diff --git a/spatialaudiogen_amd/csrc/p3.hip b/spatialaudiogen_amd/csrc/p3.hip
--- a/spatialaudiogen_amd/csrc/p3.hip
+++ b/spatialaudiogen_amd/csrc/p3.hip
@@ -43,6 +43,7 @@
 }
 
 size_t p3h_bytes(int B, int H, int W, int C) { return (size_t)(C / 16) * B * H * (W + 1) * 64; }
+size_t p3s_bytes(int B, int H, int W, int C) { return (size_t)4 * (C / 16) * B * (H / 2) * (W / 2 + 1) * 64; }
 
 
 template <bool H2>
@@ -115,7 +116,7 @@
 __global__ __launch_bounds__(256) void p3_pack_kernel(const float* __restrict__ x_, const float* __restrict__ scale_,
                                                       const float* __restrict__ shift_, const BnRef bn_,
                                                       const float* __restrict__ res_, int relu, float* __restrict__ y_,
-                                                      char* p3_, long nrows, int W, int C, const P3hScale h2_, const GroupInfo gi) {
+                                                      char* p3_, long nrows, int W, int C, const P3hScale h2_, const GroupInfo gi, int s2d) {
     const float* __restrict__ x = SAGEN_GRP(x_);
     const float* __restrict__ scale = SAGEN_GRP(scale_);
     const float* __restrict__ shift = SAGEN_GRP(shift_);
@@ -180,7 +181,14 @@
             for (int k = 0; k < 8; ++k) v[k] = 0.f;
         }
         if (p3) {
-            if (H2) {
+            if (H2 && s2d) {
+                const int Wo = W >> 1;
+                const long cs = (nrows >> 1) * (Wo + 1) * 64, phs = (long)(C >> 4) * cs;
+                const long ps = (row >> 1) * (Wo + 1) + (w < W ? (w >> 1) : Wo);
+                char* const img = p3 + ((row & 1) * 2 + (w < W ? (w & 1) : 0)) * phs;
+                p3h_store(img, cs, ps, c8, v, sa, h2.sat_count);
+                if (w == W) p3h_store(img + phs, cs, ps, c8, v, sa, h2.sat_count);
+            } else if (H2) {
                 p3h_store(p3, cstride, pp, c8, v, sa, h2.sat_count);
             } else {
                 u32x4 hi, mid, lo;
@@ -201,22 +209,24 @@
 }
 
 int p3_pack_launch(const float* x, const float* scale, const float* shift, const BnRef& bn, const float* residual, int relu,
-                   float* y, void* p3, int B, int H, int W, int C, hipStream_t s, int fmt, const P3hScale* h2) {
+                   float* y, void* p3, int B, int H, int W, int C, hipStream_t s, int fmt, const P3hScale* h2, int s2d) {
     if (C % 16 || C > P3_MAX_C) return fail(SAGEN_ERR_UNSUPPORTED, "p3_pack: C=%d must be a multiple of 16, at most %d", C, P3_MAX_C);
     if (!y && !p3) return fail(SAGEN_ERR_NULL, "p3_pack: no output");
     const long nrows = (long)B * H;
     if (p3_bytes(B, H, W, C) >= (1UL << 31)) return fail(SAGEN_ERR_UNSUPPORTED, "p3_pack: tensor exceeds 2 GiB buffer addressing");
     const long total = nrows * (W + 1) * (C / 8);
     if (fmt == 1 && p3 && !(h2 && h2->a_inv)) return fail(SAGEN_ERR_NULL, "p3_pack: the fp16x2 format needs a slot for its scale");
+    if (s2d && (fmt != 1 || !p3 || (H & 1) || (W & 1) || p3 == (h2 ? h2->res_planes : nullptr)))
+        return fail(SAGEN_ERR_UNSUPPORTED, "p3_pack: the space-to-depth form needs fp16x2 planes of an even-sized tensor, not in place");
     static const int amort_env = getenv("SAGEN_P3_AMORT") ? atoi(getenv("SAGEN_P3_AMORT")) : 0;
     const int amort = amort_env > 0 ? amort_env : 4;
     const GroupInfo gi = cur_group();
     if (fmt == 1)
         hipLaunchKernelGGL(p3_pack_kernel<true>, dim3(aligned_grid(total, C / 8, amort), 1, gi.G), dim3(256), 0, s, x, scale, shift, bn, residual, relu, y,
-                           (char*)p3, nrows, W, C, *h2, gi);
+                           (char*)p3, nrows, W, C, *h2, gi, s2d);
     else
         hipLaunchKernelGGL(p3_pack_kernel<false>, dim3(aligned_grid(total, C / 8, amort), 1, gi.G), dim3(256), 0, s, x, scale, shift, bn, residual, relu, y,
-                           (char*)p3, nrows, W, C, P3hScale(), gi);
+                           (char*)p3, nrows, W, C, P3hScale(), gi, 0);
     SAGEN_LAUNCH_CHECK();
     return SAGEN_OK;
 }
```

After: 3299 (median of 6 runs). 1.5% higher.
